# WilliamVenner/squad-mortar-helper

Measured on AMD Instinct MI355X. Metric: map frames/sec (1920x1080 full CV pipeline), whole job, higher is better.
Workload: dtype u8/f32

## Files before the change

include/smh_vision_hip_debug.h:

```cpp
#ifndef SMH_VISION_HIP_DEBUG_H
#define SMH_VISION_HIP_DEBUG_H

#include "smh_vision_hip.h"

#ifdef __cplusplus
extern "C" {
#endif

SMHV_API int smhv_debug_lsd_classic(int on);
SMHV_API int smhv_debug_lsd_tile_cap(uint32_t cap);
SMHV_API int smhv_debug_lsd_threads(uint32_t threads);
SMHV_API int smhv_debug_pattern_copy(smhv_batch *b, const void *d_frames, uint32_t n, uint32_t rows_in_flight, void *stream);
SMHV_API int smhv_debug_heightmap_color_map_device(smhv_heightmap *hm, void *d_rgba, float *ms);
SMHV_API int smhv_debug_skip_line_search(int on);
SMHV_API int smhv_debug_lsd_spin_limit(uint32_t polls);
SMHV_API int smhv_debug_no_host_atomics(int on);
SMHV_API int smhv_debug_side_kernel(smhv_ctx *ctx, uint32_t workgroups, void *stream);

SMHV_API int smhv_debug_pipeline_stats(smhv_pipeline *p, uint64_t out[32]);
SMHV_API int smhv_debug_pipeline_peek(smhv_pipeline *p, uint64_t out[16]);

SMHV_API int smhv_debug_marker_table(smhv_ctx *ctx, uint32_t *bits);

SMHV_API int smhv_debug_crc32_host_level(const void *data, uint64_t nbytes, int level, uint32_t *crc);
SMHV_API int smhv_debug_band_rows(uint32_t frame_w, uint32_t frame_h, uint32_t n, int fused, uint32_t *rows, uint32_t *bands, int *tiles);
SMHV_API int smhv_debug_map_band_rows(uint32_t rows);
SMHV_API int smhv_debug_render_form(uint32_t form);
SMHV_API int smhv_debug_render_rule(uint32_t map_w, uint32_t map_h, float sw, float sh, uint32_t hm_w, uint32_t hm_h, float *ratio, float *switch_ratio,
                                    uint32_t *lds_texels, uint32_t *form);
SMHV_API int smhv_debug_feed_rows(uint32_t rows);
SMHV_API int smhv_debug_feed_gray_form(uint32_t form);
SMHV_API int smhv_debug_batch_mask_state(smhv_batch *b, uint32_t *stale_frames, int *eager);
SMHV_API int smhv_debug_batch_ui_state(smhv_batch *b, uint32_t *stale_frames, int *eager);
SMHV_API int smhv_debug_batch_materialize_ui(smhv_batch *b, void *stream);
SMHV_API int smhv_debug_mask_expand(smhv_batch *b, uint32_t n, void *stream);
SMHV_API int smhv_debug_ingest_feed(smhv_ingest *q, uint32_t n, uint32_t *counter);
SMHV_API int smhv_debug_ingest_feed_pixels(smhv_ingest *q, uint32_t n, uint32_t *counter, uint32_t pixels);

#ifdef __cplusplus
}
#endif

#endif
```

squad-mortar-helper_amd/_lib.py:

```python
import ctypes as C
import os

_HERE = os.path.dirname(os.path.abspath(__file__))
LIB_PATH = os.environ.get("SMH_VISION_HIP_LIB") or os.path.join(_HERE, "libsmh_vision_hip.so")

MAX_LINES = 32
MAX_SCALES = 3

STAGE_MARKERS, STAGE_UI_MAP, STAGE_OCR, STAGE_SCALES, STAGE_ALL = 0x1, 0x2, 0x4, 0x8, 0xF
STAGE_MINIMAP = 0x10
STAGE_EXACT_STATS = 0x20
STAGE_LSD_HELPERS = 0x40
STAGE_FIRING = 0x80
STAGE_HEIGHTMAP_OVERLAY = 0x100
FIRING_BOUNDS_OFFSET = 1
FIRING_NONE, FIRING_SCALES, FIRING_HEIGHTMAP = 0, 1, 2
VIEW_NONE, VIEW_OCR_INPUT, VIEW_FIND_SCALES_INPUT, VIEW_LSD_PREPROCESS, VIEW_LSD_INPUT, VIEW_CROPPED_BRQ = range(6)
IMAGE_UI_MAP = 100
IMAGE_HEIGHTMAP_OVERLAY = 101
RENDER_HEIGHTMAP, RENDER_MARKERS, RENDER_BOUNDS_OFFSET = 1, 2, 4
RENDER_MAX_LINES = 256
PRIM_LINE, PRIM_RECT, PRIM_FOREGROUND, PRIM_SHIFT1 = 0, 1, 0x100, 0x200
RENDER_MAX_PRIMS = 256
LAYER_MINIMAP_BOUNDS = 1
# ... 117 lines not shown

class FeedHeader(C.Structure):
    _fields_ = [("n_entries", C.c_uint32), ("frames_done", C.c_uint32), ("n_maps", C.c_uint32), ("has_last_crc", C.c_uint32),
                ("last_crc", C.c_uint32), ("reserved", C.c_uint32), ("bytes_used", C.c_uint64)]


PIXELS_NV12, PIXELS_I420 = 5, 6
YUV_ROI_ONLY = 1


class YuvLayout(C.Structure):
    _fields_ = [("y_pitch", C.c_uint64), ("uv_pitch", C.c_uint64), ("u_offset", C.c_uint64), ("v_offset", C.c_uint64), ("frame_stride", C.c_uint64)]


LOG_FN = C.CFUNCTYPE(None, C.c_int, C.c_char_p)

SIGNATURES = {
    "smhv_init": (C.c_int, [C.c_int, LOG_FN, C.POINTER(C.c_void_p)]),
    "smhv_shutdown": (None, [C.c_void_p]),
    "smhv_thread_ctx": (C.c_int, [C.c_void_p]),
    "smhv_set_ray_table": (C.c_int, [C.c_void_p, C.POINTER(C.c_float), C.POINTER(C.c_float)]),
    "smhv_last_error": (C.c_char_p, []),
    "smhv_map_bounds": (C.c_int, [C.c_uint32, C.c_uint32, C.POINTER(C.c_uint32)]),
    "smhv_button_bounds": (C.c_int, [C.c_uint32, C.c_uint32, C.POINTER(C.c_uint32)]),
    "smhv_load_frame": (C.c_int, [C.c_void_p, C.c_void_p, C.c_uint32, C.c_uint32]),
    "smhv_load_frame_view": (C.c_int, [C.c_void_p, C.c_void_p] + [C.c_uint32] * 6),
    "smhv_load_frame_device": (C.c_int, [C.c_void_p, C.c_void_p, C.c_uint32, C.c_uint32]),
    "smhv_crop_to_map": (C.c_int, [C.c_void_p, C.c_int, C.POINTER(C.c_int), C.POINTER(C.c_uint32), C.c_void_p]),
    "smhv_red_pixels": (C.c_int, [C.c_void_p, C.POINTER(C.c_uint32)]),
    "smhv_ocr_preprocess": (C.c_int, [C.c_void_p, C.POINTER(C.c_void_p), C.POINTER(C.c_size_t)]),
    "smhv_find_scales_preprocess": (C.c_int, [C.c_void_p, C.c_uint32, C.POINTER(C.c_void_p), C.POINTER(C.c_uint32), C.POINTER(C.c_uint32)]),
    "smhv_isolate_map_markers": (C.c_int, [C.c_void_p]),
    "smhv_mask_marker_lines": (C.c_int, [C.c_void_p]),
    "smhv_get_lsd_image": (C.c_int, [C.c_void_p, C.c_void_p, C.POINTER(C.c_uint32), C.POINTER(C.c_uint32)]),
    "smhv_find_longest_line": (C.c_int, [C.c_void_p, C.c_float, C.c_float, C.c_float, C.POINTER(Line), C.POINTER(C.c_float)]),
    "smhv_find_marker_lines": (C.c_int, [C.c_void_p, C.c_uint32, C.POINTER(Line), C.POINTER(C.c_uint32)]),
    "smhv_lsd_stats": (C.c_int, [C.c_void_p, C.c_uint32, C.c_int, C.POINTER(C.c_uint32), C.POINTER(C.c_uint64)]),
    "smhv_calc_meters_to_px_ratio": (C.c_int, [C.c_void_p, C.POINTER(C.c_uint32), C.c_uint32, C.POINTER(C.c_double), C.POINTER(C.c_int), C.POINTER(C.c_uint32)]),
    "smhv_find_minimap": (C.c_int, [C.c_void_p, C.POINTER(C.c_uint32), C.POINTER(C.c_int)]),
    "smhv_get_debug_view": (C.c_int, [C.c_void_p, C.c_int, C.c_void_p, C.POINTER(C.c_uint32), C.POINTER(C.c_uint32)]),
    "smhv_batch_create": (C.c_int, [C.c_void_p, C.c_uint32, C.c_uint32, C.c_uint32, C.POINTER(C.c_void_p)]),
    "smhv_batch_destroy": (None, [C.c_void_p]),
    "smhv_batch_layout_get": (C.c_int, [C.c_void_p, C.POINTER(BatchLayout)]),
    "smhv_batch_run": (C.c_int, [C.c_void_p, C.c_void_p, C.c_uint32, C.c_uint32, C.c_int, C.c_uint32, C.c_void_p, C.c_void_p]),
    "smhv_batch_device_ptrs": (C.c_int, [C.c_void_p] + [C.POINTER(C.c_void_p)] * 6),
    "smhv_batch_tile_mask": (C.c_int, [C.c_void_p, C.POINTER(C.c_void_p), C.POINTER(C.c_void_p), C.POINTER(C.c_uint32)]),
    "smhv_batch_read_tile_mask": (C.c_int, [C.c_void_p, C.c_uint32, C.c_void_p, C.c_void_p, C.c_void_p, C.POINTER(C.c_int)]),
    "smhv_batch_read_results": (C.c_int, [C.c_void_p, C.c_uint32, C.c_uint32, C.POINTER(FrameResult)]),
    "smhv_batch_read_image": (C.c_int, [C.c_void_p, C.c_int, C.c_uint32, C.c_void_p]),
    "smhv_batch_set_scales_stream": (C.c_int, [C.c_void_p, C.c_void_p]),
    "smhv_batch_wait_map_pass": (C.c_int, [C.c_void_p, C.c_void_p]),
    "smhv_batch_enable_timing": (C.c_int, [C.c_void_p, C.c_int]),
    "smhv_batch_lsd_coop_stats": (C.c_int, [C.c_void_p, C.c_uint32, C.c_uint32, C.POINTER(C.c_uint32)]),
    "smhv_batch_stage_ms": (C.c_int, [C.c_void_p, C.POINTER(C.c_float)]),
    "smhv_pipeline_create": (C.c_int, [C.c_void_p, C.c_uint32, C.c_uint32, C.c_uint32, C.c_uint32, C.POINTER(C.c_void_p)]),
    "smhv_pipeline_create_ex": (C.c_int, [C.c_void_p, C.c_uint32, C.c_uint32, C.c_uint32, C.c_uint32, C.c_void_p, C.POINTER(C.c_void_p)]),
    "smhv_pipeline_hold": (C.c_int, [C.c_void_p, C.c_uint32, C.c_void_p]),
    "smhv_debug_pipeline_stats": (C.c_int, [C.c_void_p, C.POINTER(C.c_uint64)]),
    "smhv_debug_pipeline_peek": (C.c_int, [C.c_void_p, C.POINTER(C.c_uint64)]),
    "smhv_pipeline_destroy": (None, [C.c_void_p]),
    "smhv_pipeline_submit": (C.c_int, [C.c_void_p, C.c_void_p, C.c_uint32, C.c_uint32, C.c_int, C.c_uint32, C.c_void_p, C.c_void_p, C.POINTER(C.c_uint32)]),
    "smhv_pipeline_wait": (C.c_int, [C.c_void_p, C.c_uint32]),
    "smhv_pipeline_wait_all": (C.c_int, [C.c_void_p]),
    "smhv_pipeline_slot": (C.c_int, [C.c_void_p, C.c_uint32, C.POINTER(C.c_void_p), C.POINTER(C.c_void_p)]),
    "smhv_shard_range": (None, [C.c_uint64, C.c_uint32, C.c_uint32, C.POINTER(C.c_uint64), C.POINTER(C.c_uint64)]),
    "smhv_node_create": (C.c_int, [C.POINTER(C.c_int), C.c_uint32, C.c_uint32, C.c_uint32, C.c_uint32, C.c_uint32, LOG_FN, C.POINTER(C.c_void_p)]),
    "smhv_node_destroy": (None, [C.c_void_p]),
    "smhv_node_ctx": (C.c_int, [C.c_void_p, C.c_uint32, C.POINTER(C.c_void_p), C.POINTER(C.c_void_p)]),
    "smhv_node_run": (C.c_int, [C.c_void_p, C.POINTER(C.c_void_p), C.POINTER(C.c_uint32), C.c_uint32, C.c_int, C.c_uint32, C.POINTER(C.c_void_p)]),
    "smhv_node_gather": (C.c_int, [C.c_void_p, C.POINTER(FrameResult), C.POINTER(C.c_uint32)]),
    "smhv_debug_lsd_classic": (C.c_int, [C.c_int]),
    "smhv_debug_lsd_tile_cap": (C.c_int, [C.c_uint32]),
    "smhv_debug_lsd_spin_limit": (C.c_int, [C.c_uint32]),
    "smhv_debug_lsd_threads": (C.c_int, [C.c_uint32]),
    "smhv_debug_skip_line_search": (C.c_int, [C.c_int]),
    "smhv_debug_no_host_atomics": (C.c_int, [C.c_int]),
    "smhv_debug_side_kernel": (C.c_int, [C.c_void_p, C.c_uint32, C.c_void_p]),
    "smhv_trait_times": (C.c_int, [C.c_void_p, C.POINTER(C.c_uint64), C.POINTER(C.c_uint64), C.c_int]),
    "smhv_ui_map": (C.c_int, [C.c_void_p, C.POINTER(C.c_void_p), C.POINTER(C.c_uint32), C.POINTER(C.c_uint32)]),
    "smhv_debug_pattern_copy": (C.c_int, [C.c_void_p, C.c_void_p, C.c_uint32, C.c_uint32, C.c_void_p]),
    "smhv_debug_batch_mask_state": (C.c_int, [C.c_void_p, C.POINTER(C.c_uint32), C.POINTER(C.c_int)]),
    "smhv_debug_batch_ui_state": (C.c_int, [C.c_void_p, C.POINTER(C.c_uint32), C.POINTER(C.c_int)]),
    "smhv_debug_batch_materialize_ui": (C.c_int, [C.c_void_p, C.c_void_p]),
    "smhv_debug_mask_expand": (C.c_int, [C.c_void_p, C.c_uint32, C.c_void_p]),
    "smhv_debug_marker_table": (C.c_int, [C.c_void_p, C.c_void_p]),
    "smhv_ingest_create": (C.c_int, [C.c_void_p, C.c_uint32, C.c_uint32, C.c_uint32, C.c_uint32, C.POINTER(C.c_void_p)]),
    "smhv_ingest_create_ex": (C.c_int, [C.c_void_p, C.c_uint32, C.c_uint32, C.c_uint32, C.c_uint32, C.c_uint32, C.POINTER(C.c_void_p)]),
    "smhv_crc32_host": (C.c_uint32, [C.c_void_p, C.c_uint64]),
    "smhv_debug_map_band_rows": (C.c_int, [C.c_uint32]),
    "smhv_debug_band_rows": (C.c_int, [C.c_uint32, C.c_uint32, C.c_uint32, C.c_int, C.POINTER(C.c_uint32), C.POINTER(C.c_uint32), C.POINTER(C.c_int)]),
    "smhv_debug_ingest_feed": (C.c_int, [C.c_void_p, C.c_uint32, C.POINTER(C.c_uint32)]),
    "smhv_debug_ingest_feed_pixels": (C.c_int, [C.c_void_p, C.c_uint32, C.POINTER(C.c_uint32), C.c_uint32]),
    "smhv_debug_crc32_host_level": (C.c_int, [C.c_void_p, C.c_uint64, C.c_int, C.POINTER(C.c_uint32)]),
    "smhv_ingest_destroy": (None, [C.c_void_p]),
    "smhv_ingest_local_cpus": (C.c_int, [C.c_void_p, C.c_char_p, C.c_size_t]),
    "smhv_ingest_bind_thread": (C.c_int, [C.c_void_p]),
    "smhv_ingest_acquire": (C.c_int, [C.c_void_p, C.POINTER(C.c_void_p)]),
    "smhv_ingest_commit": (C.c_int, [C.c_void_p]),
    "smhv_ingest_push": (C.c_int, [C.c_void_p, C.c_void_p]),
    "smhv_ingest_commit_pixels": (C.c_int, [C.c_void_p, C.c_uint32]),
    "smhv_ingest_push_pixels": (C.c_int, [C.c_void_p, C.c_void_p, C.c_uint32]),
    "smhv_ingest_staging_bytes": (C.c_uint64, [C.c_uint32, C.c_uint32, C.c_uint32]),
    "smhv_yuv_to_bgra_device": (C.c_int, [C.c_void_p, C.c_void_p, C.POINTER(YuvLayout), C.c_uint32, C.c_uint32, C.c_uint32, C.c_uint32, C.c_void_p, C.c_uint64,
                                          C.c_uint32, C.c_void_p]),
    "smhv_ingest_batch": (C.c_int, [C.c_void_p, C.POINTER(C.c_void_p), C.POINTER(C.c_uint32), C.POINTER(C.c_uint32)]),
    "smhv_ingest_reset": (C.c_int, [C.c_void_p]),
    "smhv_ingest_counts": (C.c_int, [C.c_void_p, C.POINTER(C.c_uint64), C.POINTER(C.c_uint64)]),
    "smhv_crc32_device": (C.c_int, [C.c_void_p, C.c_void_p, C.c_uint64, C.POINTER(C.c_uint32)]),
    "smhv_heightmap_create": (C.c_int, [C.c_void_p, C.c_void_p, C.c_uint32, C.c_uint32, C.POINTER(C.c_int32), C.POINTER(C.c_float), C.POINTER(C.c_void_p)]),
    "smhv_heightmap_destroy": (None, [C.c_void_p]),
    "smhv_heightmap_color_map": (C.c_int, [C.c_void_p, C.c_void_p]),
    "smhv_debug_heightmap_color_map_device": (C.c_int, [C.c_void_p, C.c_void_p, C.POINTER(C.c_float)]),
    "smhv_batch_set_firing": (C.c_int, [C.c_void_p, C.c_void_p, C.POINTER(FiringOptions)]),
    "smhv_pipeline_set_firing": (C.c_int, [C.c_void_p, C.c_void_p, C.POINTER(FiringOptions)]),
    "smhv_batch_read_firing": (C.c_int, [C.c_void_p, C.c_uint32, C.c_uint32, C.POINTER(FiringResult)]),
    "smhv_batch_firing_ptr": (C.c_int, [C.c_void_p, C.POINTER(C.c_void_p)]),
    "smhv_firing_solutions": (C.c_int, [C.c_void_p, C.c_void_p, C.c_uint32, C.POINTER(C.c_double), C.POINTER(C.c_uint32), C.c_void_p,
                                        C.POINTER(FiringOptions), C.POINTER(Firing)]),
    "smhv_batch_overlay_ptr": (C.c_int, [C.c_void_p, C.POINTER(C.c_void_p)]),
    "smhv_heightmap_overlay": (C.c_int, [C.c_void_p, C.c_void_p, C.POINTER(FiringOptions), C.c_void_p]),
    "smhv_map_viewport_calc": (C.c_int, [C.c_float, C.c_float, C.c_float, C.c_float, C.c_uint32, C.POINTER(C.c_float), C.POINTER(C.c_float),
                                         C.POINTER(RenderOptions)]),
    "smhv_batch_render": (C.c_int, [C.c_void_p, C.c_uint32, C.c_uint32, C.c_void_p, C.POINTER(RenderOptions), C.c_void_p]),
    "smhv_batch_render_ptr": (C.c_int, [C.c_void_p, C.POINTER(C.c_void_p), C.POINTER(C.c_uint64)]),
    "smhv_batch_render_size": (C.c_int, [C.c_void_p, C.POINTER(C.c_uint32), C.POINTER(C.c_uint32)]),
    "smhv_batch_read_render": (C.c_int, [C.c_void_p, C.c_uint32, C.c_void_p]),
    "smhv_batch_render_layers": (C.c_int, [C.c_void_p, C.c_uint32, C.c_uint32, C.c_void_p, C.POINTER(RenderOptions), C.POINTER(RenderLayersStruct), C.c_void_p]),
    "smhv_render_map_layers": (C.c_int, [C.c_void_p, C.c_void_p, C.POINTER(RenderOptions), C.POINTER(RenderLayersStruct), C.c_void_p, C.c_uint32, C.c_void_p]),
    "smhv_render_map": (C.c_int, [C.c_void_p, C.c_void_p, C.POINTER(RenderOptions), C.c_void_p, C.c_uint32, C.c_void_p]),
    "smhv_label_font": (C.c_int, [C.c_uint8, C.POINTER(C.c_uint8)]),
    "smhv_batch_render_labels": (C.c_int, [C.c_void_p, C.c_uint32, C.c_uint32, C.c_void_p, C.POINTER(RenderOptions), C.POINTER(LabelOptionsStruct), C.c_void_p]),
    "smhv_batch_read_labels": (C.c_int, [C.c_void_p, C.c_uint32, C.c_uint32, C.POINTER(LabelResult)]),
    "smhv_batch_labels_ptr": (C.c_int, [C.c_void_p, C.POINTER(C.c_void_p)]),
    "smhv_render_map_labeled": (C.c_int, [C.c_void_p, C.c_void_p, C.POINTER(RenderOptions), C.POINTER(RenderLayersStruct), C.c_void_p, C.c_uint32,
                                          C.POINTER(LabelOptionsStruct), C.c_void_p, C.POINTER(LabelResult)]),
    "smhv_text_font": (C.c_int, [C.c_uint8, C.POINTER(C.c_uint8)]),
    "smhv_probe_text": (C.c_int, [C.POINTER(Probe), C.c_char_p, C.c_size_t]),
    "smhv_batch_probe": (C.c_int, [C.c_void_p, C.c_uint32, C.c_uint32, C.POINTER(RenderOptions), C.POINTER(ProbePoint), C.c_uint32, C.c_void_p]),
    "smhv_batch_read_probes": (C.c_int, [C.c_void_p, C.c_uint32, C.c_uint32, C.POINTER(Probe)]),
    "smhv_batch_probes_ptr": (C.c_int, [C.c_void_p, C.POINTER(C.c_void_p)]),
    "smhv_batch_render_debug": (C.c_int, [C.c_void_p, C.c_uint32, C.c_uint32, C.POINTER(RenderOptions), C.POINTER(DebugOptionsStruct), C.c_void_p]),
    "smhv_render_map_debug": (C.c_int, [C.c_void_p, C.c_void_p, C.POINTER(RenderOptions), C.POINTER(RenderLayersStruct), C.c_void_p, C.c_uint32,
                                        C.POINTER(LabelOptionsStruct), C.POINTER(DebugOptionsStruct), C.c_void_p, C.POINTER(LabelResult), C.POINTER(Probe)]),
    "smhv_feed_create": (C.c_int, [C.c_void_p, C.c_uint64, C.c_uint32, C.POINTER(C.c_void_p)]),
    "smhv_feed_destroy": (None, [C.c_void_p]),
    "smhv_feed_reset": (C.c_int, [C.c_void_p]),
    "smhv_batch_feed": (C.c_int, [C.c_void_p, C.c_void_p, C.c_uint32, C.c_uint32, C.c_uint32, C.c_void_p]),
    "smhv_feed_read": (C.c_int, [C.c_void_p, C.POINTER(FeedHeader), C.POINTER(FeedEntry), C.c_uint32, C.c_void_p, C.c_uint64]),
    "smhv_feed_ptrs": (C.c_int, [C.c_void_p, C.POINTER(C.c_void_p), C.POINTER(C.c_void_p), C.POINTER(C.c_void_p)]),
    "smhv_feed_frame": (C.c_int, [C.c_void_p, C.c_void_p, C.c_void_p, C.c_uint32, C.POINTER(C.c_double), C.POINTER(C.c_uint32), C.c_uint32]),
    "smhv_web_event_markers": (C.c_int, [C.c_void_p, C.c_uint32, C.c_int, C.c_void_p, C.c_uint64, C.POINTER(C.c_uint64)]),
    "smhv_web_event_heightmap": (C.c_int, [C.c_void_p, C.c_uint32, C.c_uint32, C.POINTER(C.c_int32), C.POINTER(C.c_float), C.c_void_p, C.c_uint64,
                                           C.POINTER(C.c_uint64)]),
    "smhv_web_event_fit": (C.c_int, [C.c_int, C.c_void_p, C.c_uint64, C.POINTER(C.c_uint64)]),
    "smhv_web_interaction_parse": (C.c_int, [C.c_void_p, C.c_uint64, C.POINTER(C.c_uint32), C.POINTER(C.c_float), C.POINTER(C.c_uint32)]),
    "smhv_debug_feed_rows": (C.c_int, [C.c_uint32]),
    "smhv_debug_feed_gray_form": (C.c_int, [C.c_uint32]),
    "smhv_batch_feed_view": (C.c_int, [C.c_void_p, C.c_void_p, C.c_uint32, C.c_uint32, C.c_uint32, C.c_uint32, C.c_void_p]),
    "smhv_feed_frame_view": (C.c_int, [C.c_void_p, C.c_void_p, C.c_void_p, C.c_uint32, C.POINTER(C.c_double), C.POINTER(C.c_uint32), C.c_uint32, C.c_uint32]),
    "smhv_debug_render_form": (C.c_int, [C.c_uint32]),
    "smhv_debug_render_rule": (C.c_int, [C.c_uint32, C.c_uint32, C.c_float, C.c_float, C.c_uint32, C.c_uint32, C.POINTER(C.c_float), C.POINTER(C.c_float),
                                         C.POINTER(C.c_uint32), C.POINTER(C.c_uint32)]),
}


def firing_options(fit_to_minimap=True, viewport=None):
# ... 67 lines not shown
```

squad-mortar-helper_amd/batch.py:

```python
import ctypes as C
from collections.abc import Mapping

import numpy as np

from . import _lib as L

STAGE_NAMES = ("button", "map_pass", "brq_pass", "lsd", "scale_ratio")


def make_anchors(per_frame):
    arr = (L.Anchors * len(per_frame))()
    for i, (start_y, scales) in enumerate(per_frame):
        arr[i].n = min(len(scales), L.MAX_SCALES)
        arr[i].scales_start_y = start_y
        for j, (m, x, y) in enumerate(scales[:L.MAX_SCALES]):
            arr[i].scales[j][0], arr[i].scales[j][1], arr[i].scales[j][2] = m, x, y
    return arr


def results_to_dicts(recs):
    out = []
    for r in recs:
        n = r.n_lines
        out.append(dict(
            map_open=int(r.map_open), n_lines=int(n),
            lines=np.array([[r.lines[i].x0, r.lines[i].y0, r.lines[i].x1, r.lines[i].y1] for i in range(n)], np.float32).reshape(-1, 4),
            mpx=(r.mpx if r.has_mpx else None), n_mask_px=int(r.n_mask_px), red_pixels=int(r.red_pixels),
            rounds=int(r.rounds), ray_steps=int(r.ray_steps),
            length_px=np.array(r.length_px[:n], np.float64), meters=np.array(r.meters[:n], np.float64),
            angle=np.array(r.angle[:n], np.float32),
            minimap=(tuple(r.minimap) if r.has_minimap else None),
            status=int(r.status), error=(None if r.status == L.FRAME_OK else "line search gave the frame up (SMHV_FRAME_LSD_STUCK)" if r.status == L.FRAME_LSD_STUCK
                                         else "status %d" % r.status)))
    return out


_PTR_KEYS = ("results", "ui", "mask", "ocr", "scales", "bits")


class _DevicePtrs(Mapping):

    def __init__(self, batch, ptrs):
        self._batch, self._ptrs = batch, ptrs

    def __getitem__(self, key):
        if key == "mask" and self._ptrs["mask"] is None:
            self._ptrs["mask"] = self._batch._mask_ptr()
        if key == "ui" and self._ptrs["ui"] is None:
            self._ptrs["ui"] = self._batch._ui_ptr()
        return self._ptrs[key]

    def __iter__(self):
        return iter(_PTR_KEYS)

    def __len__(self):
        return len(_PTR_KEYS)


class FrameBatch:

    def __init__(self, vision, frame_w, frame_h, max_frames, _handle=None):
        self._lib = L.load()
        self._vision = vision
        self._owned = _handle is None
        if _handle is None:
            b = C.c_void_p()
            L.check(self._lib.smhv_batch_create(vision._ctx, frame_w, frame_h, max_frames, C.byref(b)))
        else:
            b = _handle
        self._b = b
        self.max_frames = max_frames
        self.frame_w, self.frame_h = frame_w, frame_h
        self.layout = L.BatchLayout()
        L.check(self._lib.smhv_batch_layout_get(self._b, C.byref(self.layout)))

    def close(self):
        if self._b:
            if self._owned:
                self._lib.smhv_batch_destroy(self._b)
            self._b = None

    def __del__(self):
        try:
            self.close()
        except Exception:
            pass

    @property
    def roi(self):
        return tuple(self.layout.roi)

    def enable_timing(self, on=True):
        L.check(self._lib.smhv_batch_enable_timing(self._b, int(on)))

    def run(self, frames_ptr, n, stages=L.STAGE_ALL, grayscale=True, max_gap=15, anchors=None, stream=0):
        if anchors is not None and len(anchors) < n:
            raise ValueError("anchors holds %d entries, the run covers %d frames" % (len(anchors), n))
        a = C.cast(anchors, C.c_void_p) if anchors is not None else None
        L.check(self._lib.smhv_batch_run(self._b, C.c_void_p(frames_ptr), n, stages, int(bool(grayscale)), max_gap, a, C.c_void_p(stream)))

    def set_scales_stream(self, stream=0):
        L.check(self._lib.smhv_batch_set_scales_stream(self._b, C.c_void_p(stream)))

    def wait_map_pass(self, stream=0):
        L.check(self._lib.smhv_batch_wait_map_pass(self._b, C.c_void_p(stream)))

    def stage_ms(self):
        ms = (C.c_float * 5)()
        L.check(self._lib.smhv_batch_stage_ms(self._b, ms))
        return dict(zip(STAGE_NAMES, [float(v) for v in ms]))

    def lsd_coop_stats(self, first=0, n=None):
        n = self.max_frames - first if n is None else n
        out = np.zeros((n, 4), np.uint32)
        L.check(self._lib.smhv_batch_lsd_coop_stats(self._b, first, n, out.ctypes.data_as(C.POINTER(C.c_uint32))))
        return out

    def device_ptrs(self):
        p = [C.c_void_p() for _ in range(6)]
        args = [C.byref(x) for x in p]
        args[1] = args[2] = None
        L.check(self._lib.smhv_batch_device_ptrs(self._b, *args))
        return _DevicePtrs(self, dict(zip(_PTR_KEYS, [x.value for x in p])))

    def _mask_ptr(self):
        m = C.c_void_p()
        L.check(self._lib.smhv_batch_device_ptrs(self._b, None, None, C.byref(m), None, None, None))
        return m.value

    def _ui_ptr(self):
        u = C.c_void_p()
        L.check(self._lib.smhv_batch_device_ptrs(self._b, None, C.byref(u), None, None, None, None))
        return u.value

    def ui_state(self):
        stale, eager = C.c_uint32(0), C.c_int(0)
        L.check(self._lib.smhv_debug_batch_ui_state(self._b, C.byref(stale), C.byref(eager)))
        return int(stale.value), bool(eager.value)

    def materialize_ui(self, stream=0):
        L.check(self._lib.smhv_debug_batch_materialize_ui(self._b, C.c_void_p(stream)))

    def mask_state(self):
        stale, eager = C.c_uint32(0), C.c_int(0)
        L.check(self._lib.smhv_debug_batch_mask_state(self._b, C.byref(stale), C.byref(eager)))
        return int(stale.value), bool(eager.value)

    def tile_mask(self, frame=0):
        geo = (C.c_uint32 * 4)()
        L.check(self._lib.smhv_batch_tile_mask(self._b, None, None, geo))
        trows, wcols, opitch, xoff = [int(v) for v in geo]
        tiled = np.zeros((trows, wcols, 8), np.uint32)
        occ = np.zeros((trows, opitch), np.uint8)
        bits = np.zeros((self.roi[3], wcols), np.uint32)
        written = C.c_int(0)
        L.check(self._lib.smhv_batch_read_tile_mask(self._b, frame, tiled.ctypes.data, occ.ctypes.data, bits.ctypes.data, C.byref(written)))
        return (tiled if written.value else None), (occ if written.value else None), bits, xoff

    def read_results(self, first=0, n=None, check=True):
        n = self.max_frames - first if n is None else n
        recs = (L.FrameResult * n)()
        rc = self._lib.smhv_batch_read_results(self._b, first, n, recs)
        if rc != 0 and not (rc == L.E_STATE and not check):
            try:
                L.check(rc)
            except L.VisionError as e:
                e.records = recs if rc == L.E_STATE else None
                raise
        return recs

    def set_firing(self, heightmap=None, fit_to_minimap=True, viewport=None):
        opt = L.firing_options(fit_to_minimap, viewport)
        L.check(self._lib.smhv_batch_set_firing(self._b, heightmap._hm if heightmap is not None else None, C.byref(opt)))

    def read_firing(self, first=0, n=None):
        n = self.max_frames - first if n is None else n
        out = (L.FiringResult * n)()
        L.check(self._lib.smhv_batch_read_firing(self._b, first, n, out))
        raw = np.frombuffer(out, np.uint8).reshape(n, C.sizeof(L.FiringResult))
        n_lines = raw[:, :4].copy().view(np.uint32).reshape(n)
        lines = raw[:, 8:].copy().view(L.firing_dtype()).reshape(n, L.MAX_LINES)
        return n_lines, lines

    def firing_ptr(self):
        d = C.c_void_p()
        L.check(self._lib.smhv_batch_firing_ptr(self._b, C.byref(d)))
        return d.value or 0

    def read_overlay(self, frame):
        return self.read_image(L.IMAGE_HEIGHTMAP_OVERLAY, frame)

    def overlay_ptr(self):
        d = C.c_void_p()
        L.check(self._lib.smhv_batch_overlay_ptr(self._b, C.byref(d)))
        return d.value or 0

    def render(self, viewport, out_w, out_h, first=0, n=None, heightmap=None, markers=False, fit_to_minimap=True, background=(0, 0, 0, 255),
               stream=None, options=None, layers=None):
        from .render import render_options
        n = self.max_frames - first if n is None else n
        opt = options if options is not None else render_options(viewport, out_w, out_h, heightmap is not None, markers, fit_to_minimap, background)
        if layers is not None:
            ly, keep = layers.struct()
            L.check(self._lib.smhv_batch_render_layers(self._b, first, n, heightmap._hm if heightmap is not None else None, C.byref(opt), C.byref(ly), stream))
            del keep
            return
        L.check(self._lib.smhv_batch_render(self._b, first, n, heightmap._hm if heightmap is not None else None, C.byref(opt), stream))

    def render_size(self):
        w, h = C.c_uint32(), C.c_uint32()
        L.check(self._lib.smhv_batch_render_size(self._b, C.byref(w), C.byref(h)))
        return int(w.value), int(h.value)

    def read_render(self, frame):
        w, h = self.render_size()
        out = np.empty((h, w, 4), np.uint8)
# ... 162 lines not shown
```

squad-mortar-helper_amd/csrc/smh_feed.inc:

```

struct smhv_feed {
	smhv_ctx *ctx = nullptr;
	uint64_t capacity = 0;
	uint32_t max_frames = 0;
	uint8_t *d_bytes = nullptr;
	smhv_feed_header *d_header = nullptr;
	smhv_feed_entry *d_entries = nullptr;
	uint32_t *d_state = nullptr, *d_raw = nullptr, *d_tab = nullptr;
	FeedMap *d_maps = nullptr;
	uint32_t tab_w = 0, tab_h = 0, tab_xoff = 0, tab_ppg = 0;
	uint8_t *d_view = nullptr;
	size_t view_cap = 0;
	hipEvent_t ev_last = nullptr;
	bool used = false;
	smhv_frame_result *d_rec = nullptr, *h_rec = nullptr;
};

extern "C" SMHV_API void smhv_feed_destroy(smhv_feed *f) {
	if (!f) return;
	if (f->ctx) (void)hipSetDevice(f->ctx->device);
	(void)hipDeviceSynchronize();
	void *ptrs[] = {f->d_bytes, f->d_header, f->d_entries, f->d_state, f->d_raw, f->d_tab, f->d_maps, f->d_rec, f->d_view};
	for (void *p : ptrs)
		if (p) (void)hipFree(p);
// ... 81 lines not shown
		f->tab_w = cw; f->tab_h = ch; f->tab_xoff = cxoff; f->tab_ppg = v.ppg;
	}
	FeedRun r;
	memset(&r, 0, sizeof r);
	r.ui = v.base; r.res = res;
	r.ui_stride = v.stride; r.ui_pitch = v.pitch;
	r.w = v.w; r.h = v.h; r.xoff = v.xoff; r.quads = v.quads;
	r.n = n; r.first = first; r.flags = flags;
	r.len_term = crc32_mul(crc32_xpow(32ull * v.w * v.h), 0xFFFFFFFFu) ^ 0xFFFFFFFFu;
	r.rows_per_wave = feed_rows_per_wave(ch, n);
	r.capacity = f->capacity;
	r.raw = f->d_raw; r.tab = f->d_tab; r.state = f->d_state;
	r.header = f->d_header; r.entries = f->d_entries; r.bytes = f->d_bytes; r.maps = f->d_maps;
	if (v.mode == SMH_RND_SRC_UI) HIPCHK(launch_feed(r, s));
	else if (!image) HIPCHK(launch_feed_view(r, v.mode, s));
	else {
		FeedRun c = r;
		c.ui = v.base - 4ull * v.lead; c.ui_pitch = 4ull * SMH_FEED_IMAGE_ROW; c.ui_stride = 0;
		c.w = cw; c.h = ch; c.xoff = 0u; c.quads = cquads;
		HIPCHK(launch_feed_image(c, r, s));
	}
	HIPCHK(hipEventRecord(f->ev_last, s));
	f->used = true;
	return SMHV_OK;
}

static int feed_batch_source(const smhv_batch *b, uint32_t first, uint32_t map_source, bool resolve, FeedSrc *v) {
	const Geom &g = b->g;
	if (map_source > (uint32_t)SMHV_VIEW_CROPPED_BRQ) return fail(SMHV_E_INVALID, "batch_feed_view: unknown map source %u", map_source);
	if (resolve && !b->ui_written) return fail(SMHV_E_STATE, "batch_feed: no run of this batch has produced a ui_map (SMHV_STAGE_UI_MAP)");
	*v = feed_src_ui(g, b->d_ui + (size_t)first * g.ui_stride);
	switch ((int)map_source) {
	case SMHV_VIEW_NONE: break;
	case SMHV_VIEW_OCR_INPUT:
	case SMHV_VIEW_FIND_SCALES_INPUT: {
		const bool ocr = map_source == (uint32_t)SMHV_VIEW_OCR_INPUT;
		if (resolve && !(ocr ? b->ocr_written : b->scales_written))
			return fail(SMHV_E_STATE, "batch_feed_view: no run of this batch has produced the %s image", ocr ? "OCR input (SMHV_STAGE_OCR)" : "scales input (SMHV_STAGE_SCALES with anchors)");
		v->mode = SMH_RND_SRC_GRAY; v->ppg = 16u;
		v->base = (ocr ? b->d_ocr : b->d_scales) + (size_t)first * g.ocr_stride;
		v->pitch = g.ocr_pitch; v->stride = g.ocr_stride; v->xoff = g.q_xoff; v->w = g.qw; v->h = g.qh;
		v->quads = (v->w + v->xoff + 15u) / 16u;
		break;
	}
	case SMHV_VIEW_LSD_INPUT:
		if (resolve && !b->mask_written) return fail(SMHV_E_STATE, "batch_feed_view: no run of this batch has produced the marker mask (SMHV_STAGE_MARKERS)");
		v->mode = SMH_RND_SRC_GRAY; v->ppg = 16u;
		v->base = b->d_mask + (size_t)first * g.mask_stride;
		v->pitch = g.mask_pitch; v->stride = g.mask_stride;
		v->quads = (v->w + v->xoff + 15u) / 16u;
		break;
	default:
		if (resolve && b->ui_gray) return fail(SMHV_E_STATE, "batch_feed_view: the batch's ui_map is grayscale, map source %u needs the colour one", map_source);
		if (map_source == (uint32_t)SMHV_VIEW_CROPPED_BRQ) {
			const uint32_t x0 = g.m_xoff + g.rw / 2u;
			v->mode = SMH_RND_SRC_CROPPED; v->w = g.rw / 2u; v->h = g.rh / 2u;
			if (resolve && (v->w == 0u || v->h == 0u)) return fail(SMHV_E_STATE, "batch_feed_view: the map has no bottom right quarter");
			v->base += (size_t)(g.rh / 2u) * g.ui_pitch + 16ull * (x0 / 4u);
			v->xoff = x0 & 3u; v->quads = (v->w + v->xoff + 3u) / 4u;
		} else v->mode = SMH_RND_SRC_PREPROCESS;
		break;
	}
	return SMHV_OK;
}

extern "C" SMHV_API int smhv_batch_feed_view(smhv_batch *b, smhv_feed *f, uint32_t first, uint32_t n, uint32_t flags, uint32_t map_source, void *stream) {
	if (!b || !f) return fail(SMHV_E_INVALID, "batch_feed: null argument");
	CTX_OPEN(b->ctx);
	CTX_OPEN(f->ctx);
	if (f->ctx->device != b->ctx->device) return fail(SMHV_E_INVALID, "batch_feed: the feed lives on device %d, the batch on %d", f->ctx->device, b->ctx->device);
	if (n == 0u || (uint64_t)first + n > b->max_frames) return fail(SMHV_E_INVALID, "batch_feed: frames [%u, %u + %u) of a batch of %u", first, first, n, b->max_frames);
	FeedSrc v;
	int rc = feed_batch_source(b, first, map_source, false, &v);
	if (rc) return rc;
	rc = feed_check(f, v.w, v.h, n, flags, "batch_feed");
	if (rc) return rc;
	rc = feed_batch_source(b, first, map_source, true, &v);
	if (rc) return rc;
	HIPCHK(hipSetDevice(b->ctx->device));
	if (map_source == (uint32_t)SMHV_VIEW_LSD_INPUT) {
		rc = batch_materialize_mask(b, (hipStream_t)stream);
		if (rc) return rc;
	}
	rc = batch_materialize_ui(b, (hipStream_t)stream);
	if (rc) return rc;
	return feed_enqueue(f, v, b->d_results + first, first, n, flags, (hipStream_t)stream);
}

extern "C" SMHV_API int smhv_batch_feed(smhv_batch *b, smhv_feed *f, uint32_t first, uint32_t n, uint32_t flags, void *stream) {
	return smhv_batch_feed_view(b, f, first, n, flags, (uint32_t)SMHV_VIEW_NONE, stream);
}

extern "C" SMHV_API int smhv_feed_read(smhv_feed *f, smhv_feed_header *header, smhv_feed_entry *entries, uint32_t max_entries, uint8_t *bytes, uint64_t cap) {
	if (!f || !header) return fail(SMHV_E_INVALID, "feed_read: null argument");
	CTX_OPEN(f->ctx);
	HIPCHK(hipSetDevice(f->ctx->device));
	if (f->used) HIPCHK(wait_event(f->ev_last));
	HIPCHK(hipMemcpy(header, f->d_header, sizeof *header, hipMemcpyDeviceToHost));
	if (entries && header->n_entries > max_entries) return fail(SMHV_E_INVALID, "feed_read: %u entries, room for %u", header->n_entries, max_entries);
	if (bytes && header->bytes_used > cap) return fail(SMHV_E_INVALID, "feed_read: %llu bytes, room for %llu", (unsigned long long)header->bytes_used, (unsigned long long)cap);
	if (entries && header->n_entries) HIPCHK(hipMemcpy(entries, f->d_entries, sizeof(smhv_feed_entry) * header->n_entries, hipMemcpyDeviceToHost));
	if (bytes && header->bytes_used) HIPCHK(hipMemcpy(bytes, f->d_bytes, (size_t)header->bytes_used, hipMemcpyDeviceToHost));
	return SMHV_OK;
}

extern "C" SMHV_API int smhv_feed_ptrs(smhv_feed *f, void **d_header, void **d_entries, void **d_bytes) {
	if (!f) return fail(SMHV_E_INVALID, "feed_ptrs: null feed");
	if (d_header) *d_header = f->d_header;
	if (d_entries) *d_entries = f->d_entries;
	if (d_bytes) *d_bytes = f->d_bytes;
	return SMHV_OK;
}

extern "C" SMHV_API int smhv_debug_feed_gray_form(uint32_t form) {
	if (form != 0u && form != 4u) return fail(SMHV_E_INVALID, "feed gray form %u (0 = the rule, 4 = four lookups per message dword)", form);
	feed_set_gray_form(form);
	return SMHV_OK;
}

extern "C" SMHV_API int smhv_debug_feed_rows(uint32_t rows) {
	if (rows > 64u) return fail(SMHV_E_INVALID, "feed rows per wave %u (0 = the rule, 1 .. 64)", rows);
	feed_set_rows(rows);
	return SMHV_OK;
}

extern "C" SMHV_API int smhv_feed_frame_view(smhv_ctx *c, smhv_feed *f, const smhv_line *lines, uint32_t n_lines, const double *mpx, const uint32_t minimap[4],
                                             uint32_t flags, uint32_t map_source) {
	int rc = require_open(c, "feed_frame");
	if (rc) return rc;
	CTX_OPEN(c);
	if (!f || (n_lines && !lines)) return fail(SMHV_E_INVALID, "feed_frame: null argument");
	CTX_OPEN(f->ctx);
	if (f->ctx->device != c->device) return fail(SMHV_E_INVALID, "feed_frame: the feed lives on device %d, the context on %d", f->ctx->device, c->device);
	if (n_lines > SMHV_MAX_LINES) return fail(SMHV_E_INVALID, "feed_frame: %u lines (at most %u)", n_lines, (unsigned)SMHV_MAX_LINES);
	if (map_source > (uint32_t)SMHV_VIEW_CROPPED_BRQ) return fail(SMHV_E_INVALID, "feed_frame_view: unknown map source %u", map_source);
	smhv_batch *b = c->fb;
	const Geom &g = b->g;
	rc = batch_materialize_ui(b, c->s_main);
	if (rc) return rc;
	FeedSrc v = feed_src_ui(g, b->d_ui);
	if (map_source != (uint32_t)SMHV_VIEW_NONE) {
		const int which = (int)map_source;
		const bool brq = which == SMHV_VIEW_OCR_INPUT || which == SMHV_VIEW_FIND_SCALES_INPUT || which == SMHV_VIEW_CROPPED_BRQ;
		v.mode = SMH_RND_SRC_RGBA; v.w = brq ? g.qw : g.rw; v.h = brq ? g.qh : g.rh;
		v.xoff = 0u; v.quads = 0u; v.pitch = 4ull * v.w; v.stride = 0;
	}
	rc = feed_check(f, v.w, v.h, 1, flags, "feed_frame");
	if (rc) return rc;
	HIPCHK(hipSetDevice(c->device));
	if (f->used) HIPCHK(wait_event(f->ev_last));
	if (v.mode == SMH_RND_SRC_RGBA) {
		const uint64_t dw = (uint64_t)v.w * v.h, rows = (dw + SMH_FEED_IMAGE_ROW - 1u) / SMH_FEED_IMAGE_ROW;
		const size_t need = (size_t)rows * SMH_FEED_IMAGE_ROW * 4u;
		if (rows > SMH_FEED_MAX_ROWS) return fail(SMHV_E_INVALID, "feed_frame_view: a view of %u x %u pixels", v.w, v.h);
		if (f->view_cap < need) {
			if (f->d_view) (void)hipFree(f->d_view);
			f->d_view = nullptr; f->view_cap = 0;
			HIPCHK(hipMalloc((void **)&f->d_view, need));
			f->view_cap = need;
		}
		v.lead = (uint32_t)(rows * SMH_FEED_IMAGE_ROW - dw);
		v.base = f->d_view + 4ull * v.lead;
		if (v.lead) HIPCHK(hipMemsetAsync(f->d_view, 0, 4ull * v.lead, c->s_main));
		Buffers bf = make_buffers(b, c->frame_ptr, 0);
		HIPCHK(launch_debug_view(g, bf, 0, (int)map_source, c->isolated ? 1 : 0, f->d_view + 4ull * v.lead, c->s_main));
	}
// ... 87 lines not shown
```

squad-mortar-helper_amd/csrc/smh_kernels.h:

```cpp
#pragma once
#include <hip/hip_runtime.h>
#include <stdint.h>

#include "../../include/smh_vision_hip.h"
#include "../../include/smh_vision_hip_debug.h"

namespace smh {

struct Geom {
	uint32_t W, H;
	uint32_t rx, ry, rw, rh;
	uint32_t bx, by, bw, bh;
	uint32_t qx, qy, qw, qh;
	uint32_t m_ax, m_xoff, m_quads, m_block;
	uint32_t q_ax, q_xoff, q_quads, q_block;
	uint64_t frame_bytes;
	uint64_t ui_pitch, ui_stride;
	uint64_t mask_pitch, mask_stride;
	uint32_t bits_pitch_w; uint64_t bits_stride_w;
	uint64_t ocr_pitch, ocr_stride;
};

struct FrameAux {
	uint32_t open;
// ... 207 lines not shown
#define SMH_CULL_TAB_WORDS (SMH_CULL_CELLS + (SMH_SECTOR_ENTRIES + 3) / 4)

#define SVC_MAX_SLOTS 32u
struct SvcSlot {
	Buffers b;
	uint32_t n;
	uint32_t seq;
	uint32_t done;
	uint32_t pad;
	unsigned long long t_pub;
};
#define SVC_REMOTE_RING 12u
#define SVC_REMOTE_OPEN 0x80000000ull
struct SvcRemoteEntry {
	unsigned long long post;
	unsigned long long claim;
	uint32_t res_a[4];
	uint32_t res_b[4];
	unsigned long long pad[2];
};
struct SvcRemote {
	unsigned long long state;
	unsigned long long info;
	unsigned long long pad[6];
	SvcRemoteEntry ring[SVC_REMOTE_RING];
};
#define SVC_HELP_RING 256u
struct SvcCtl {
	int32_t avail;
	uint32_t closing;
	int32_t help_avail;
	uint32_t help_head, help_reserve;
	uint32_t stat_remote;
	uint32_t head;
	uint32_t reserve;
	uint32_t completed;
	uint32_t busy;
	uint32_t stat_items, stat_waves;
	unsigned long long stat_busy, stat_life;
	unsigned long long stat_phase[4];
	unsigned long long stat_help;
	uint32_t stat_requests, stat_attached;
	unsigned long long stat_t_wait, stat_t_sub, stat_t_last;
	uint32_t stat_h_polls, stat_h_empty, stat_h_lost, stat_h_idle_exit, stat_h_closed_exit, stat_h_pad;
	unsigned long long stat_h_cycles, stat_h_cast_cycles;
	unsigned long long help_ring[SVC_HELP_RING];
};
struct SvcHost {
	unsigned long long state;
	uint32_t launches;
	uint32_t pad0;
	uint32_t done_seq[SVC_MAX_SLOTS];
	uint32_t pad[12];
};
struct SvcParams {
	SvcCtl *ctl;
	unsigned long long *ring;
	SvcSlot *slots;
	SvcHost *host;
	const uint32_t *cull_tab;
	const float *ray_off;
	float max_gap;
	uint32_t tile_cap, list_cap;
	uint32_t part_words;
	uint32_t ring_log2;
	uint32_t epoch;
	uint32_t idle_short, idle_long;
	uint32_t flags;
	SvcRemote *remote;
	uint32_t *remote_store;
	uint32_t remote_store_words;
	uint32_t remote_after;
	uint32_t remote_tickets;
	uint32_t remote_last_div;
	uint32_t compact;
};
uint32_t svc_waves_for(const Geom &g, uint32_t tile_limit, uint32_t *part_words, uint32_t *tile_cap, uint32_t *list_cap, uint32_t *lds_bytes, uint32_t *compact = nullptr);
uint32_t svc_store_words_for(const Geom &g, uint32_t tile_cap, uint32_t compact);
hipError_t svc_probe_host_atomics(SvcHost *h, SvcHost *d_h, bool *ok);
hipError_t launch_svc_publish(SvcCtl *ctl, unsigned long long *ring, SvcSlot *slots, uint32_t slot, const Buffers &b, uint32_t n, uint32_t seq, uint32_t ring_log2, hipStream_t s);
hipError_t launch_lsd_service(const Geom &g, const SvcParams &p, uint32_t workgroups, uint32_t waves, uint32_t lds_bytes, hipStream_t s);

enum : uint32_t { MAP_UI = 1u, MAP_MASK = 2u, MAP_BYTES = 4u, MAP_PRIO = 0x100u, MAP_BAND_MAJOR = 0x200u };
enum : uint32_t { BRQ_OCR = 1u, BRQ_SCALES = 2u };

enum : uint32_t { UI_FORM_RGBA = 0u, UI_FORM_LUMA = 1u, UI_FORM_KEEP = 2u };
hipError_t launch_button(const Geom &g, const Buffers &b, uint32_t n, int force_open, hipStream_t s, uint8_t *ui_form = nullptr, uint32_t ui_luma = UI_FORM_KEEP);
hipError_t launch_ui_expand(const Geom &g, const uint8_t *d_luma, uint8_t *d_ui, uint8_t *ui_form, uint32_t n, hipStream_t s);
hipError_t launch_map_pass(const Geom &g, const Buffers &b, uint32_t n, uint32_t flags, int grayscale, hipStream_t s, bool tiles_wanted = false, bool overlapped = false);
struct LaunchTuning {
	uint32_t map_lds_total;
	uint32_t map_grid_cap;
	uint32_t lsd_tile_limit;
	uint32_t map_prio;
	uint32_t map_deep;
	uint32_t map_overlapped;
};
uint32_t map_brq_lds_bytes(const Geom &g);
uint32_t lsd_tile_lds_bytes(const Geom &g, uint32_t tile_limit);
hipError_t launch_map_brq_pass(const Geom &g, const Buffers &b, uint32_t n, uint32_t flags, uint32_t qflags, int grayscale, uint32_t fixed_start_y, int use_anchor_start, hipStream_t s,
                               const LaunchTuning *tune = nullptr);
hipError_t launch_pattern_copy(const Geom &g, const Buffers &b, uint32_t n, uint32_t rows_in_flight, hipStream_t s);
void map_band_rows(uint32_t rh, uint32_t n, int fused, uint32_t *rows, int *tiles);
hipError_t launch_brq_pass(const Geom &g, const Buffers &b, uint32_t n, uint32_t flags, uint32_t fixed_start_y, int use_anchor_start, hipStream_t s);
struct LsdFork { hipStream_t s1, s2; hipEvent_t fork, join1, join2; };
bool lsd_rows_only(const Geom &g);
hipError_t launch_lsd(const Geom &g, const Buffers &b, uint32_t n, float max_gap, int mode, float px, float py, hipStream_t s, const LsdFork *fk, uint32_t tile_bs = 0,
                      bool prefer_classic = false, uint32_t tile_limit = 0, bool *record_fused = nullptr);
size_t lsd_coop_ctl_bytes(uint32_t n);
hipError_t launch_scale_ratio(const Geom &g, const Buffers &b, uint32_t n, uint32_t *d_bars, hipStream_t s);
hipError_t launch_find_minimap(const Geom &g, const Buffers &b, uint32_t n, hipStream_t s);
hipError_t launch_finalize(const Geom &g, const Buffers &b, uint32_t n, uint32_t stages, hipStream_t s);
hipError_t launch_scales_finalize(const Geom &g, const Buffers &b, uint32_t n, uint32_t stages, uint32_t *d_bars, hipStream_t s);
hipError_t launch_firing_lines(const FiringRun &r, const smhv_line *lines, uint32_t n, uint32_t has_mpx, double mpx, uint32_t has_minimap,
                               const uint32_t minimap[4], smhv_firing *out, hipStream_t s);
hipError_t launch_heightmap_color_map(const uint16_t *hm, uint64_t n, uint32_t *mm, uint32_t *rgba, hipStream_t s);
#define SMH_HM_LUT_ENTRIES 65536u
hipError_t launch_heightmap_lut(const uint16_t *hm, uint64_t n, uint32_t *mm, uint32_t *lut, hipStream_t s);
hipError_t launch_hm_overlay(const Geom &g, const OverlayRun &r, uint32_t n, hipStream_t s);
hipError_t launch_render_map(const Geom &g, const RenderRun &r, uint32_t n, hipStream_t s);
hipError_t launch_render_map_layers(const Geom &g, const RenderRun &r, const RenderLayersRun &y, uint32_t n, hipStream_t s);
hipError_t launch_heightmap_lut16(const uint32_t *lut, uint16_t *lut16, uint32_t *vr, hipStream_t s);
#define SMH_HM_LUT_WORDS (SMH_HM_LUT_ENTRIES + 4u + SMH_HM_LUT_ENTRIES / 2u)
hipError_t launch_labels(const LabelRun &r, uint32_t n, hipStream_t s);
hipError_t launch_debug_text(const Geom &g, const DebugRun &r, uint32_t n, hipStream_t s);
void render_set_form(uint32_t form);
uint32_t render_rule(const Geom &g, const RenderRun &r, uint32_t *texels, float *ratio);
float render_switch_ratio();
hipError_t launch_debug_view(const Geom &g, const Buffers &b, uint32_t frame, int which, int isolated, uint8_t *d_rgba, hipStream_t s);
hipError_t launch_marker_table(uint32_t *d_bits, hipStream_t s);
hipError_t launch_mask_expand(const Geom &g, const uint32_t *d_bits, uint8_t *d_mask, uint32_t n, hipStream_t s);
hipError_t launch_pack_rows(const void *d_src, uint32_t src_pitch_bytes, void *d_dst, uint32_t row_bytes, uint32_t rows, hipStream_t s);
hipError_t launch_side_probe(uint32_t *d_out, uint32_t workgroups, uint32_t spin, hipStream_t s);
hipError_t launch_build_sector_table(unsigned long long *d_tab, uint32_t T, hipStream_t s);
hipError_t launch_build_ray_offsets(float *d_off, hipStream_t s);
size_t lsd_lds_bytes();
void lsd_set_classic(bool on);
void lsd_set_tile_cap(uint32_t cap);
void lsd_set_threads(uint32_t threads);
void lsd_set_spin_limit(uint32_t polls);
hipError_t set_ray_table(const float *dx, const float *dy);
#define SMH_CRC_BS 1024
hipError_t launch_to_bgra(const void *d_src, void *d_bgra, uint64_t n_px, uint32_t layout, hipStream_t s);
#define SMH_YUV_NV12 5
#define SMH_YUV_I420 6
#define SMH_YUV_BAND_PAIRS 4u
struct YuvCoef { int cy, yoff, rv, gu, gv, bu; };
struct YuvRect {
	uint32_t x0, y0, w, h;
	uint64_t y_off, u_off, v_off;
	uint32_t y_pitch, uv_pitch, y_x0, y_y0, c_x0, c_y0;
};
struct YuvRun {
	const uint8_t *src; uint8_t *dst;
	uint64_t src_stride, dst_stride;
	uint32_t W, H, n;
	uint32_t bands0, bands_total;
	YuvCoef k;
	YuvRect r[2];
};
hipError_t launch_yuv_to_bgra(YuvRun run, uint32_t n_rects, uint32_t layout, uint32_t bilinear, hipStream_t s);
hipError_t launch_unpack_rows(const void *d_pack, void *d_frame, uint32_t pitch_px, uint32_t roi_x, uint32_t roi_y, uint32_t roi_w, uint32_t roi_h, uint32_t btn_x,
                              uint32_t btn_y, uint32_t btn_w, uint32_t btn_h, hipStream_t s);
hipError_t launch_crc32(const void *d_msg, uint64_t n_dwords, uint32_t wgs, uint32_t rounds, uint32_t x_skip, const uint32_t *d_x_local,
                        const uint32_t *d_x_wg, uint32_t *d_acc, hipStream_t s);
uint32_t crc32_xpow(uint64_t n);
uint32_t crc32_mul(uint32_t a, uint32_t b);

struct FeedMap { uint64_t dst; uint32_t frame, pad; };
struct FeedRun {
	const uint8_t *ui;
	const smhv_frame_result *res;
	uint64_t ui_stride, ui_pitch;
	uint32_t w, h, xoff, quads;
	uint32_t n, first, flags;
	uint32_t len_term;
	uint32_t rows_per_wave;
	uint64_t capacity;
	uint32_t *raw;
	const uint32_t *tab;
	uint32_t *state;
	smhv_feed_header *header;
// ... 17 lines not shown
```

squad-mortar-helper_amd/csrc/smh_misc.hip:

```cpp
#include "smh_device.h"
#include "smh_record.inc"

namespace smh {

__global__ void __launch_bounds__(64 * SMHV_MAX_SCALES) k_scale_ratio(Geom g, Buffers b, uint32_t *bars) { scale_ratio_body(g, b, blockIdx.x, bars); }

__device__ __forceinline__ bool flat_pixel(const uint8_t *roi0, uint32_t W, uint32_t x, uint32_t y) {
	const uint32_t *p = (const uint32_t *)(roi0 + ((size_t)y * W + x) * 4);
	const int Wi = (int)W;
	const uint32_t c = p[0] & 0x00FFFFFFu;
	uint32_t mx = 0;
#pragma unroll
	for (int dy = -1; dy <= 1; ++dy)
#pragma unroll
		for (int dx = -1; dx <= 1; ++dx)
			if (dx != 0 || dy != 0) mx = max(mx, (uint32_t)__builtin_amdgcn_sad_u8(c, p[dy * Wi + dx] & 0x00FFFFFFu, 0u));
	return (float)mx / 765.0f <= 0.01f;
}

__device__ uint32_t find_edge(const uint8_t *roi0, uint32_t W, uint32_t w, uint32_t h, uint32_t x0, uint32_t y0, int dir) {
	const uint32_t lane = threadIdx.x & 63u;
	const bool vertical = dir < 2;
	uint32_t c_max = vertical ? h : w, oc_max = vertical ? w : h;
	const int cod = (dir == 0 || dir == 2) ? -1 : 1;
// ... 302 lines not shown
hipError_t launch_scale_ratio(const Geom &g, const Buffers &b, uint32_t n, uint32_t *d_bars, hipStream_t s) {
	hipLaunchKernelGGL(k_scale_ratio, dim3(n), dim3(64 * SMHV_MAX_SCALES), 0, s, g, b, d_bars);
	return hipGetLastError();
}

hipError_t launch_find_minimap(const Geom &g, const Buffers &b, uint32_t n, hipStream_t s) {
	hipLaunchKernelGGL(k_find_minimap, dim3(n), dim3(256), 0, s, g, b);
	return hipGetLastError();
}

hipError_t launch_finalize(const Geom &g, const Buffers &b, uint32_t n, uint32_t stages, hipStream_t s) {
	if (stages & SMHV_STAGE_FIRING) hipLaunchKernelGGL(k_finalize_firing, dim3(n), dim3(64), 0, s, g, b, stages);
	else hipLaunchKernelGGL(k_finalize, dim3(n), dim3(64), 0, s, g, b, stages);
	return hipGetLastError();
}

hipError_t launch_scales_finalize(const Geom &g, const Buffers &b, uint32_t n, uint32_t stages, uint32_t *d_bars, hipStream_t s) {
	if (stages & SMHV_STAGE_FIRING) hipLaunchKernelGGL(k_scales_finalize_firing, dim3(n), dim3(64 * SMHV_MAX_SCALES), 0, s, g, b, stages, d_bars);
	else hipLaunchKernelGGL(k_scales_finalize, dim3(n), dim3(64 * SMHV_MAX_SCALES), 0, s, g, b, stages, d_bars);
	return hipGetLastError();
}

__global__ void __launch_bounds__(256) k_pack_rows(const uint32_t *__restrict__ src, uint32_t src_pitch_w, uint32_t *__restrict__ dst, uint32_t row_w, uint32_t rows) {
	const uint32_t r = blockIdx.y;
	const uint32_t *s = src + (size_t)r * src_pitch_w;
	uint32_t *d = dst + (size_t)r * row_w;
	for (uint32_t x = blockIdx.x * blockDim.x + threadIdx.x; x < row_w; x += gridDim.x * blockDim.x) d[x] = s[x];
}
hipError_t launch_pack_rows(const void *d_src, uint32_t src_pitch_bytes, void *d_dst, uint32_t row_bytes, uint32_t rows, hipStream_t s) {
	if ((src_pitch_bytes | row_bytes) & 3u) return hipErrorInvalidValue;
	const uint32_t row_w = row_bytes / 4u;
	hipLaunchKernelGGL(k_pack_rows, dim3((row_w + 255u) / 256u, rows), dim3(256), 0, s, (const uint32_t *)d_src, src_pitch_bytes / 4u, (uint32_t *)d_dst, row_w, rows);
	return hipGetLastError();
}

__global__ void __launch_bounds__(256) k_mask_expand(const uint16_t *__restrict__ bits, uint4 *__restrict__ mask, uint64_t groups) {
	const uint64_t i = (uint64_t)blockIdx.x * 256u + threadIdx.x;
	if (i >= groups) return;
	const uint32_t v = bits[i];
	uint4 o;
	o.x = (((v & 15u) * 0x00204081u) & 0x01010101u) * 0xFFu;
	o.y = ((((v >> 4) & 15u) * 0x00204081u) & 0x01010101u) * 0xFFu;
	o.z = ((((v >> 8) & 15u) * 0x00204081u) & 0x01010101u) * 0xFFu;
	o.w = ((((v >> 12) & 15u) * 0x00204081u) & 0x01010101u) * 0xFFu;
	mask[i] = o;
}
hipError_t launch_mask_expand(const Geom &g, const uint32_t *d_bits, uint8_t *d_mask, uint32_t n, hipStream_t s) {
	if (g.mask_pitch != (uint64_t)g.bits_pitch_w * 32u || (g.mask_stride & 15u)) return hipErrorInvalidValue;
	const uint64_t groups = g.mask_stride / 16u * n, blocks = (groups + 255u) / 256u;
	if (blocks == 0 || blocks > 0x7FFFFFFFull) return hipErrorInvalidValue;
	hipLaunchKernelGGL(k_mask_expand, dim3((uint32_t)blocks), dim3(256), 0, s, (const uint16_t *)d_bits, (uint4 *)d_mask, groups);
	return hipGetLastError();
}

__global__ void __launch_bounds__(256) k_ui_expand(const uint32_t *__restrict__ luma, uint4 *__restrict__ ui, const uint8_t *__restrict__ form, uint32_t groups,
                                                   uint32_t pitch_q, uint32_t quads) {
	const uint32_t f = blockIdx.y;
	if (form[f] != UI_FORM_LUMA) return;
	const uint32_t i = blockIdx.x * 256u + threadIdx.x;
	if (i >= groups || i % pitch_q >= quads) return;
	const size_t j = (size_t)f * groups + i;
	const uint32_t v = luma[j];
	uint4 o;
	o.x = __builtin_amdgcn_perm(0u, v, 0x0D000000u);
	o.y = __builtin_amdgcn_perm(0u, v, 0x0D010101u);
	o.z = __builtin_amdgcn_perm(0u, v, 0x0D020202u);
	o.w = __builtin_amdgcn_perm(0u, v, 0x0D030303u);
	ui[j] = o;
}
hipError_t launch_ui_expand(const Geom &g, const uint8_t *d_luma, uint8_t *d_ui, uint8_t *ui_form, uint32_t n, hipStream_t s) {
	if ((g.ui_stride & 15u) || g.ui_stride / 16u > 0xFFFFFF00ull || n == 0) return hipErrorInvalidValue;
	const uint32_t groups = (uint32_t)(g.ui_stride / 16u);
	hipError_t e = hipSuccess;
	for (uint32_t done = 0; done < n && e == hipSuccess; done += 65535u) {
		const uint32_t k = std::min(n - done, 65535u);
		hipLaunchKernelGGL(k_ui_expand, dim3((groups + 255u) / 256u, k), dim3(256), 0, s, (const uint32_t *)d_luma + (size_t)done * groups, (uint4 *)d_ui + (size_t)done * groups,
		                   (const uint8_t *)ui_form + done, groups, (uint32_t)(g.ui_pitch / 16u), g.m_quads);
		e = hipGetLastError();
	}
	if (e == hipSuccess) e = hipMemsetAsync(ui_form, 0, n, s);
	return e;
}

hipError_t launch_debug_view(const Geom &g, const Buffers &b, uint32_t frame, int which, int isolated, uint8_t *d_rgba, hipStream_t s) {
	const bool brq = which == SMHV_VIEW_OCR_INPUT || which == SMHV_VIEW_FIND_SCALES_INPUT || which == SMHV_VIEW_CROPPED_BRQ;
	const uint32_t npx = brq ? g.qw * g.qh : g.rw * g.rh;
	hipLaunchKernelGGL(k_debug_view, dim3((npx + 255) / 256), dim3(256), 0, s, g, b, frame, which, isolated, d_rgba);
	return hipGetLastError();
}

hipError_t launch_marker_table(uint32_t *d_bits, hipStream_t s) {
	hipLaunchKernelGGL(k_marker_table, dim3(((1u << 24) / 32u + 255) / 256), dim3(256), 0, s, d_bits);
	return hipGetLastError();
}

#define CRC_POLY SMH_CRC_POLY
#define CRC_BS 1024

__global__ void __launch_bounds__(CRC_BS) k_crc32(const uint32_t *msg, uint64_t n_dwords, uint32_t rounds, uint32_t x_skip,
                                                 const uint32_t *x_local, const uint32_t *x_wg, uint32_t *acc) {
	__shared__ uint32_t tab[4][256];
	__shared__ uint32_t wsum[CRC_BS / 64];
	const uint32_t tid = threadIdx.x;
	if (tid < 256u) {
		uint32_t c = tid;
		for (int k = 0; k < 8; ++k) c = (c >> 1) ^ ((c & 1u) ? CRC_POLY : 0u);
		tab[0][tid] = c;
	}
	__syncthreads();
	if (tid < 256u) {
		uint32_t c = tab[0][tid];
		for (int k = 1; k < 4; ++k) { c = (c >> 8) ^ tab[0][c & 255u]; tab[k][tid] = c; }
	}
	__syncthreads();
	const uint64_t G = (uint64_t)gridDim.x * CRC_BS, T = (uint64_t)blockIdx.x * CRC_BS + tid;
	const uint64_t pad = (uint64_t)rounds * G * 4u - n_dwords;
	uint32_t v = 0;
	for (uint32_t r = 0; r < rounds; ++r) {
		const uint64_t vi = ((uint64_t)r * G + T) * 4u;
		uint32_t d[4] = {0u, 0u, 0u, 0u};
		if (vi >= pad && ((vi - pad) & 3u) == 0u && (((uintptr_t)msg) & 15u) == 0u) {
			const uint4 q = *(const uint4 *)(msg + (vi - pad));
			d[0] = q.x; d[1] = q.y; d[2] = q.z; d[3] = q.w;
		} else {
#pragma unroll
			for (int j = 0; j < 4; ++j) if (vi + j >= pad) d[j] = msg[vi + j - pad];
		}
		if (r) v = gf2_mulmod(v, x_skip);
#pragma unroll
		for (int j = 0; j < 4; ++j) {
			const uint32_t c = v ^ d[j];
			v = tab[3][c & 255u] ^ tab[2][(c >> 8) & 255u] ^ tab[1][(c >> 16) & 255u] ^ tab[0][c >> 24];
		}
	}
	v = gf2_mulmod(v, x_local[tid]);
	v = wave_xor32_dpp(v);
	if ((tid & 63u) == 0u) wsum[tid >> 6] = v;
	__syncthreads();
	if (tid == 0) {
		uint32_t w = 0;
		for (int k = 0; k < CRC_BS / 64; ++k) w ^= wsum[k];
		atomicXor(acc, gf2_mulmod(w, x_wg[blockIdx.x]));
	}
}

uint32_t crc32_xpow(uint64_t n) {
	uint32_t r = 0x80000000u, b = 0x40000000u;
	for (; n; n >>= 1) { if (n & 1u) r = gf2_mulmod(r, b); b = gf2_mulmod(b, b); }
	return r;
}
uint32_t crc32_mul(uint32_t a, uint32_t b) { return gf2_mulmod(a, b); }

hipError_t launch_crc32(const void *d_msg, uint64_t n_dwords, uint32_t wgs, uint32_t rounds, uint32_t x_skip, const uint32_t *d_x_local,
                        const uint32_t *d_x_wg, uint32_t *d_acc, hipStream_t s) {
	hipLaunchKernelGGL(k_crc32, dim3(wgs), dim3(CRC_BS), 0, s, (const uint32_t *)d_msg, n_dwords, rounds, x_skip, d_x_local, d_x_wg, d_acc);
	return hipGetLastError();
}

template <int BPP>
__global__ void __launch_bounds__(256) k_to_bgra(const uint32_t *__restrict__ src, uint4 *__restrict__ dst, uint64_t n_groups, uint64_t n_px) {
	for (uint64_t gidx = (uint64_t)blockIdx.x * 256u + threadIdx.x; gidx < n_groups; gidx += (uint64_t)gridDim.x * 256u) {
		uint32_t w[4] = {0u, 0u, 0u, 0u}, px[4];
		const uint64_t n_src_dwords = (n_px * BPP + 3u) / 4u;
#pragma unroll
		for (int k = 0; k < BPP; ++k) { const uint64_t i = gidx * BPP + k; if (i < n_src_dwords) w[k] = src[i]; }
		if (BPP == 4) {
// ... 60 lines not shown
```

squad-mortar-helper_amd/csrc/smh_runtime.cpp:

```cpp
#include <hip/hip_runtime.h>

#include <atomic>
#include <condition_variable>
#include <deque>
#include <thread>
#include <cmath>
#include <cstdarg>
#include <cstdio>
#include <cstdlib>
#include <cstring>
#include <ctime>
#include <sched.h>
#include <pthread.h>
#include <cctype>
#include <mutex>
#include <vector>
#include <new>
#include <string>

#include "smh_consts.h"
#include "smh_kernels.h"

using namespace smh;

// ... 99 lines not shown
	if (rc) return rc;
	rc = smhv_button_bounds(W, H, bt);
	if (rc) return rc;
	memset(g, 0, sizeof *g);
	g->W = W; g->H = H;
	g->rx = m[0]; g->ry = m[1]; g->rw = m[2]; g->rh = m[3];
	g->bx = bt[0]; g->by = bt[1]; g->bw = bt[2]; g->bh = bt[3];
	g->qw = g->rw / 2; g->qh = g->rh / 2;
	g->qx = g->rx + g->qw; g->qy = g->ry + g->qh;
	if (g->qw < SMH_OCR_DILATE_RADIUS || g->qh < SMH_OCR_DILATE_RADIUS) return fail(SMHV_E_GEOMETRY, "frame %ux%u too small", W, H);
	g->m_ax = g->rx & ~3u; g->m_xoff = g->rx - g->m_ax;
	g->m_quads = (g->rw + g->m_xoff + 3u) / 4u;
	g->m_block = (g->m_quads + 63u) & ~63u;
	g->q_ax = g->qx & ~3u; g->q_xoff = g->qx - g->q_ax;
	g->q_quads = (g->qw + g->q_xoff + 3u) / 4u;
	g->q_block = (g->q_quads + 63u) & ~63u;
	if (g->m_block > 1024u) return fail(SMHV_E_GEOMETRY, "frame %ux%u: map ROI wider than 4096 px is not supported", W, H);
	const uint32_t mq = (g->m_quads + 15u) & ~15u, qq = (g->q_quads + 15u) & ~15u;
	g->frame_bytes = (uint64_t)W * H * 4;
	g->ui_pitch = (uint64_t)mq * 16; g->ui_stride = g->ui_pitch * g->rh;
	g->mask_pitch = (uint64_t)mq * 4; g->mask_stride = g->mask_pitch * g->rh;
	g->bits_pitch_w = mq / 8; g->bits_stride_w = (uint64_t)g->bits_pitch_w * g->rh;
	g->ocr_pitch = (uint64_t)qq * 4; g->ocr_stride = g->ocr_pitch * g->qh;
	return SMHV_OK;
}

struct smhv_batch {
	smhv_ctx *ctx = nullptr;
	Geom g{};
	uint32_t max_frames = 0;
	uint8_t *d_ui = nullptr, *d_mask = nullptr, *d_ocr = nullptr, *d_scales = nullptr;
	uint32_t *d_bits = nullptr, *d_bars = nullptr, *d_tiled = nullptr;
	uint8_t *d_occ = nullptr;
	FrameAux *d_aux = nullptr;
	smhv_frame_result *d_results = nullptr;
	smhv_anchors *d_anchors = nullptr;
	BatchError *h_err = nullptr, *d_err = nullptr;
	FarmFrame *d_farm = nullptr;
	uint8_t *d_lsd_ctl = nullptr;
	uint32_t *d_lsd_req = nullptr;
	LsdCacheEntry *d_lsd_cache = nullptr;
	uint32_t lsd_epoch = 0;
	struct AnchorStage { smhv_anchors *h = nullptr; hipEvent_t done = nullptr; };
	std::vector<AnchorStage> anchor_stage;
	static constexpr int TIMING_RING = 64;
	static constexpr int TIMING_EVENTS = 10;
	bool timing = false;
	hipEvent_t (*ev)[TIMING_EVENTS] = nullptr;
	uint64_t timed_runs = 0;
	hipStream_t s_scales = nullptr;
	hipStream_t s_scales_ext = nullptr;
	hipEvent_t ev_map_done = nullptr;
	hipEvent_t ev_fork = nullptr, ev_join = nullptr;
	LsdFork lsd_fork{};
	uint32_t lsd_late_kc = 0;
	uint32_t lsd_bs = 1024;
	bool lsd_prefer_classic = false;
	LaunchTuning tune{0u, 0u, 0u, 0u};
	hipEvent_t ev_probe[3] = {nullptr, nullptr, nullptr};
	bool probe = false, probe_valid = false;
	smhv_heightmap *fire_hm = nullptr;
	smhv_firing_options fire_opt{};
	smhv_firing_result *d_firing = nullptr;
	FiringRun *d_fire_run = nullptr;
	struct FireStage { FiringRun *h = nullptr; hipEvent_t done = nullptr; };
	std::vector<FireStage> fire_stage;
	uint8_t *d_overlay = nullptr;
	uint8_t *d_render = nullptr;
	size_t render_cap = 0;
	uint32_t render_w = 0, render_h = 0;
	smhv_heightmap *render_hm = nullptr;
	hipEvent_t ev_render = nullptr;
	bool ui_written = false;
	bool ui_gray = false, mask_written = false, ocr_written = false, scales_written = false;
	std::mutex mask_mu;
	uint32_t mask_stale = 0;
	bool mask_eager = false;
	hipEvent_t ev_mask = nullptr;
	uint8_t *d_ui_luma = nullptr, *d_ui_form = nullptr;
	std::mutex ui_mu;
	uint32_t ui_stale = 0;
	bool ui_eager = false;
	hipEvent_t ev_ui = nullptr;
	smhv_render_prim *h_prims = nullptr, *d_prims = nullptr;
	hipEvent_t ev_prims = nullptr;
	smhv_label_result *d_labels = nullptr;
	LabelCull *d_label_cull = nullptr;
	smhv_label_line *h_label_extra = nullptr, *d_label_extra = nullptr;
	hipEvent_t ev_label_extra = nullptr;
	smhv_heightmap *label_hm = nullptr;
	smhv_probe *d_probes = nullptr;
	DebugItem *d_dbg_items = nullptr;
	uint8_t *d_dbg_pool = nullptr, *h_dbg_stage = nullptr, *d_dbg_stage = nullptr;
	hipEvent_t ev_dbg_stage = nullptr, ev_dbg = nullptr;
	bool probed = false;
};

struct smhv_heightmap {
	smhv_ctx *ctx = nullptr;
	uint16_t *d = nullptr;
	uint32_t w = 0, h = 0;
	int32_t bounds[4] = {0, 0, 0, 0};
	float scale[3] = {0.0f, 0.0f, 0.0f};
	std::atomic<int> refs{1};
	mutable std::mutex lut_mu;
	mutable std::atomic<uint32_t *> d_lut{nullptr};
};
static void hm_retain(smhv_heightmap *hm) { if (hm) hm->refs.fetch_add(1, std::memory_order_relaxed); }
static void hm_release(smhv_heightmap *hm);

struct smhv_ctx {
	int device = 0;
	smhv_log_fn log = nullptr;
	hipStream_t s_main = nullptr, s_markers = nullptr, s_scales = nullptr;
	hipStream_t s_ui = nullptr;
	hipEvent_t ev_map = nullptr, ev_ui[2] = {nullptr, nullptr};
	hipEvent_t ev_ui_part[3] = {nullptr, nullptr, nullptr};
	uint8_t *h_ui[2] = {nullptr, nullptr};
	size_t h_ui_cap[2] = {0, 0};
	uint8_t *d_ui_tight = nullptr;
	size_t d_ui_tight_cap = 0;
	uint8_t *d_fire = nullptr, *h_fire = nullptr;
	size_t fire_cap = 0;
	std::mutex fire_mu;
	uint32_t ui_turn = 0;
	bool ui_pending = false, minimap_cached = false;
	uint32_t W = 0, H = 0;
	bool have_frame = false;
	uint8_t *d_frame = nullptr;
	size_t d_frame_cap = 0;
	const uint8_t *frame_ptr = nullptr;
	smhv_batch *fb = nullptr;
	uint8_t *h_ocr = nullptr, *h_scales = nullptr;
	uint8_t *h_stage[3] = {nullptr, nullptr, nullptr};
	size_t h_stage_cap[3] = {0, 0, 0};
	smhv_frame_result *h_res = nullptr;
	FrameAux *h_aux = nullptr;
	uint32_t *h_bars = nullptr;
	bool cropped = false, map_open = false, isolated = false, mask_valid = false, scales_valid = false;
	static constexpr int SECTOR_CACHE = 8;
	uint32_t sector_T[SECTOR_CACHE] = {};
	uint32_t *sector_tab[SECTOR_CACHE] = {};
	int sector_n = 0;
	float *d_ray_off = nullptr;
	uint32_t *d_side = nullptr;
	std::atomic<uint64_t> tt_ns[SMHV_TRAIT_CALLS] = {}, tt_calls[SMHV_TRAIT_CALLS] = {};
	std::mutex mu;
	std::atomic<int> refs{1};
	std::atomic<bool> closed{false};
};

static std::mutex g_ctx_mu;
static std::vector<smhv_ctx *> g_ctx_open;

static void ctx_release(smhv_ctx *c) {
	if (c && c->refs.fetch_sub(1, std::memory_order_acq_rel) == 1) delete c;
}
#define CTX_OPEN(c)                                                                                          \
	do {                                                                                                     \
		if (!(c) || (c)->closed.load(std::memory_order_acquire)) return fail(SMHV_E_INVALID, "the context was shut down"); \
	} while (0)

static void logf(smhv_ctx *c, int lvl, const char *fmt, ...) {
	if (!c || !c->log) return;
	char buf[512];
	va_list ap;
// ... 169 lines not shown
extern "C" SMHV_API int smhv_debug_lsd_tile_cap(uint32_t cap) {
	lsd_set_tile_cap(cap);
	return SMHV_OK;
}

extern "C" SMHV_API int smhv_debug_skip_line_search(int on) {
	g_skip_lsd.store(on != 0, std::memory_order_relaxed);
	return SMHV_OK;
}

static std::atomic<bool> g_no_host_atomics{false};
extern "C" SMHV_API int smhv_debug_no_host_atomics(int on) {
	g_no_host_atomics.store(on != 0, std::memory_order_relaxed);
	return SMHV_OK;
}
extern "C" SMHV_API int smhv_debug_side_kernel(smhv_ctx *c, uint32_t workgroups, void *stream) {
	if (!c || workgroups == 0 || workgroups > 1024u) return fail(SMHV_E_INVALID, "side_kernel: 1..1024 workgroups");
	CTX_OPEN(c);
	HIPCHK(hipSetDevice(c->device));
	if (!c->d_side) HIPCHK(hipMalloc((void **)&c->d_side, 1024u * sizeof(uint32_t)));
	HIPCHK(launch_side_probe(c->d_side, workgroups, 64u, (hipStream_t)stream));
	return SMHV_OK;
}
extern "C" SMHV_API int smhv_debug_lsd_threads(uint32_t threads) {
	if (threads != 0 && (threads < 128 || threads > 1024 || threads % 64)) return fail(SMHV_E_INVALID, "lsd_threads: 0 or a multiple of 64 from 128 to 1024");
	lsd_set_threads(threads);
	return SMHV_OK;
}

extern "C" SMHV_API int smhv_debug_lsd_spin_limit(uint32_t polls) {
	lsd_set_spin_limit(polls);
	return SMHV_OK;
}

extern "C" SMHV_API int smhv_set_ray_table(smhv_ctx *c, const float *dx, const float *dy) {
	if (!c || !dx || !dy) return fail(SMHV_E_INVALID, "bad arguments");
	CTX_OPEN(c);
	for (int i = 0; i < SMH_LSD_RAYS; ++i) {
		const double a = (double)i / 10.0 * 3.14159265358979323846 / 180.0;
		if (!(std::fabs((double)dx[i] - std::cos(a)) < 1e-5 && std::fabs((double)dy[i] - std::sin(a)) < 1e-5))
			return fail(SMHV_E_INVALID, "ray table entry %d is not (cos, sin) of %.1f degrees", i, i / 10.0);
	}
	std::lock_guard<std::mutex> lk(g_ctx_mu);
	HIPCHK(hipSetDevice(c->device));
	HIPCHK(hipDeviceSynchronize());
	HIPCHK(set_ray_table(dx, dy));
	for (smhv_ctx *o : g_ctx_open)
		if (o->device == c->device && o->d_ray_off) HIPCHK(launch_build_ray_offsets(o->d_ray_off, c->s_main));
	HIPCHK(hipStreamSynchronize(c->s_main));
	return SMHV_OK;
}

static hipError_t create_stream(hipStream_t *st, const uint32_t *cu_mask) {
	return cu_mask ? hipExtStreamCreateWithCUMask(st, 8, cu_mask) : hipStreamCreateWithFlags(st, hipStreamNonBlocking);
}

extern "C" SMHV_API int smhv_batch_create(smhv_ctx *c, uint32_t W, uint32_t H, uint32_t max_frames, smhv_batch **out) {
	if (!c || !out || max_frames == 0) return fail(SMHV_E_INVALID, "bad arguments");
	*out = nullptr;
	CTX_OPEN(c);
	Geom g;
	int rc = compute_geom(W, H, &g);
	if (rc) return rc;
	HIPCHK(hipSetDevice(c->device));
	smhv_batch *b = new (std::nothrow) smhv_batch();
	if (!b) return fail(SMHV_E_INVALID, "out of host memory");
	c->refs.fetch_add(1, std::memory_order_relaxed);
	b->ctx = c; b->g = g; b->max_frames = max_frames;
	const size_t n = max_frames;
#define ALLOC0(ptr, bytes)                                          \
	do {                                                            \
		hipError_t _e = hipMalloc((void **)&(ptr), (bytes));        \
		if (_e == hipSuccess) _e = hipMemset((ptr), 0, (bytes));    \
		if (_e != hipSuccess) { smhv_batch_destroy(b); return fail(SMHV_E_HIP, "allocating %zu bytes: %s", (size_t)(bytes), hipGetErrorString(_e)); } \
	} while (0)
	ALLOC0(b->d_ui, g.ui_stride * n);
	ALLOC0(b->d_ui_luma, g.ui_stride / 4 * n);
	ALLOC0(b->d_ui_form, n);
	ALLOC0(b->d_mask, g.mask_stride * n);
	ALLOC0(b->d_bits, g.bits_stride_w * 4 * n);
	ALLOC0(b->d_tiled, tiled_stride_w(g) * 4 * n);
	ALLOC0(b->d_occ, occ_stride(g) * n);
	ALLOC0(b->d_ocr, g.ocr_stride * n);
	ALLOC0(b->d_scales, g.ocr_stride * n);
	ALLOC0(b->d_aux, sizeof(FrameAux) * n);
	ALLOC0(b->d_results, sizeof(smhv_frame_result) * (n + 3));
	ALLOC0(b->d_anchors, sizeof(smhv_anchors) * n);
	ALLOC0(b->d_bars, sizeof(uint32_t) * SMHV_MAX_SCALES * 4 * n);
	ALLOC0(b->d_lsd_ctl, lsd_coop_ctl_bytes(max_frames));
	ALLOC0(b->d_lsd_req, sizeof(uint32_t) * SMH_LSD_REQ_CAP * n);
	ALLOC0(b->d_farm, sizeof(FarmFrame) * n);
	ALLOC0(b->d_lsd_cache, sizeof(LsdCacheEntry) * SMH_LSD_CACHE_SLOTS * n);
#undef ALLOC0
	{
		hipError_t e = hipHostMalloc((void **)&b->h_err, sizeof(BatchError), hipHostMallocMapped | hipHostMallocCoherent);
		if (e == hipSuccess) { memset(b->h_err, 0, sizeof(BatchError)); e = hipHostGetDevicePointer((void **)&b->d_err, b->h_err, 0); }
		if (e == hipSuccess) e = hipEventCreateWithFlags(&b->ev_map_done, hipEventDisableTiming);
		if (e == hipSuccess) e = hipEventCreateWithFlags(&b->ev_mask, hipEventDisableTiming);
		if (e == hipSuccess) e = hipEventCreateWithFlags(&b->ev_ui, hipEventDisableTiming);
		if (max_frames > 1 && !lsd_rows_only(b->g)) {
			if (e == hipSuccess) e = create_stream(&b->lsd_fork.s1, nullptr);
			if (e == hipSuccess) e = create_stream(&b->lsd_fork.s2, nullptr);
			if (e == hipSuccess) e = hipEventCreateWithFlags(&b->lsd_fork.fork, hipEventDisableTiming);
			if (e == hipSuccess) e = hipEventCreateWithFlags(&b->lsd_fork.join1, hipEventDisableTiming);
			if (e == hipSuccess) e = hipEventCreateWithFlags(&b->lsd_fork.join2, hipEventDisableTiming);
		}
		if (e != hipSuccess) { smhv_batch_destroy(b); return fail(SMHV_E_HIP, "branch streams: %s", hipGetErrorString(e)); }
	}
	*out = b;
	return SMHV_OK;
}

extern "C" SMHV_API void smhv_batch_destroy(smhv_batch *b) {
	if (!b) return;
	if (b->ctx) (void)hipSetDevice(b->ctx->device);
	(void)hipDeviceSynchronize();
	void *ptrs[] = {b->d_ui, b->d_ui_luma, b->d_ui_form, b->d_mask, b->d_bits, b->d_tiled, b->d_occ, b->d_ocr, b->d_scales, b->d_aux, b->d_results, b->d_anchors, b->d_bars, b->d_farm,
	                b->d_lsd_ctl, b->d_lsd_req, b->d_lsd_cache, b->d_firing, b->d_fire_run, b->d_overlay, b->d_render, b->d_prims, b->d_labels,
	                b->d_label_cull, b->d_label_extra, b->d_probes, b->d_dbg_items, b->d_dbg_pool, b->d_dbg_stage};
	for (void *p : ptrs)
		if (p) (void)hipFree(p);
	if (b->h_prims) (void)hipHostFree(b->h_prims);
	if (b->ev_prims) (void)hipEventDestroy(b->ev_prims);
	if (b->h_label_extra) (void)hipHostFree(b->h_label_extra);
	if (b->ev_label_extra) (void)hipEventDestroy(b->ev_label_extra);
	if (b->h_dbg_stage) (void)hipHostFree(b->h_dbg_stage);
	if (b->ev_dbg_stage) (void)hipEventDestroy(b->ev_dbg_stage);
	if (b->ev_dbg) (void)hipEventDestroy(b->ev_dbg);
	if (b->h_err) (void)hipHostFree(b->h_err);
	for (auto &a : b->anchor_stage) {
		if (a.h) (void)hipHostFree(a.h);
		if (a.done) (void)hipEventDestroy(a.done);
	}
	for (auto &a : b->fire_stage) {
		if (a.h) (void)hipHostFree(a.h);
		if (a.done) (void)hipEventDestroy(a.done);
	}
	hm_release(b->fire_hm);
	hm_release(b->render_hm);
	hm_release(b->label_hm);
	if (b->ev_render) (void)hipEventDestroy(b->ev_render);
	if (b->ev) {
		for (int r = 0; r < smhv_batch::TIMING_RING; ++r)
			for (int i = 0; i < smhv_batch::TIMING_EVENTS; ++i) if (b->ev[r][i]) (void)hipEventDestroy(b->ev[r][i]);
		delete[] b->ev;
	}
	if (b->s_scales) (void)hipStreamDestroy(b->s_scales);
	if (b->ev_fork) (void)hipEventDestroy(b->ev_fork);
	if (b->ev_join) (void)hipEventDestroy(b->ev_join);
	if (b->ev_map_done) (void)hipEventDestroy(b->ev_map_done);
	if (b->ev_mask) (void)hipEventDestroy(b->ev_mask);
	if (b->ev_ui) (void)hipEventDestroy(b->ev_ui);
	for (auto e : b->ev_probe) if (e) (void)hipEventDestroy(e);
	if (b->lsd_fork.s1) (void)hipStreamDestroy(b->lsd_fork.s1);
	if (b->lsd_fork.s2) (void)hipStreamDestroy(b->lsd_fork.s2);
	if (b->lsd_fork.fork) (void)hipEventDestroy(b->lsd_fork.fork);
	if (b->lsd_fork.join1) (void)hipEventDestroy(b->lsd_fork.join1);
	if (b->lsd_fork.join2) (void)hipEventDestroy(b->lsd_fork.join2);
	ctx_release(b->ctx);
	delete b;
}

static int batch_check_errors(smhv_batch *b, const char *what) {
	BatchError *e = b->h_err;
	if (!e) return SMHV_OK;
	const uint32_t count = __atomic_load_n(&e->count, __ATOMIC_ACQUIRE);
	if (count == 0) return SMHV_OK;
	const BatchError snap = *e;
	memset(e, 0, sizeof *e);
	logf(b->ctx, 1, "%s: %u frame(s) failed, first: frame %u status %u", what, count, snap.frame, snap.status);
	if (snap.status == SMHV_FRAME_LSD_STUCK)
		return fail(SMHV_E_STATE, "%s: %u frame(s) without marker lines (status != 0 in their records); first: frame %u, line search gave up "
		            "(SMHV_FRAME_LSD_STUCK: head %u tail %u list %u/%u lines %u rounds %u spec %u head-state %u)", what, count, snap.frame,
		            snap.info[0], snap.info[1], snap.info[2], snap.info[3], snap.info[4], snap.info[5], snap.info[6], snap.info[7]);
	return fail(SMHV_E_STATE, "%s: %u frame(s) failed; first: frame %u, status %u", what, count, snap.frame, snap.status);
}
extern "C" int smhv_internal_batch_check(smhv_batch *b, const char *what) { return b ? batch_check_errors(b, what) : SMHV_OK; }

extern "C" SMHV_API int smhv_batch_layout_get(smhv_batch *b, smhv_batch_layout *o) {
	if (!b || !o) return fail(SMHV_E_INVALID, "bad arguments");
	const Geom &g = b->g;
	memset(o, 0, sizeof *o);
	o->frame_w = g.W; o->frame_h = g.H;
	o->roi[0] = g.rx; o->roi[1] = g.ry; o->roi[2] = g.rw; o->roi[3] = g.rh;
	o->button[0] = g.bx; o->button[1] = g.by; o->button[2] = g.bw; o->button[3] = g.bh;
	o->brq_w = g.qw; o->brq_h = g.qh;
	o->ui_pitch = g.ui_pitch; o->ui_stride = g.ui_stride; o->ui_offset = (uint64_t)g.m_xoff * 4;
	o->mask_pitch = g.mask_pitch; o->mask_stride = g.mask_stride; o->mask_offset = g.m_xoff;
	o->ocr_pitch = g.ocr_pitch; o->ocr_stride = g.ocr_stride; o->ocr_offset = g.q_xoff;
	o->scales_pitch = g.ocr_pitch; o->scales_stride = g.ocr_stride; o->scales_offset = g.q_xoff;
	o->bits_pitch_words = g.bits_pitch_w; o->bits_stride = g.bits_stride_w * 4; o->bits_xoff = g.m_xoff;
	return SMHV_OK;
}

extern "C" SMHV_API int smhv_batch_enable_timing(smhv_batch *b, int enable) {
	if (!b) return fail(SMHV_E_INVALID, "null batch");
	if (enable && !b->ev) {
		HIPCHK(hipSetDevice(b->ctx->device));
		b->ev = new hipEvent_t[smhv_batch::TIMING_RING][smhv_batch::TIMING_EVENTS]();
		for (int r = 0; r < smhv_batch::TIMING_RING; ++r)
			for (int i = 0; i < smhv_batch::TIMING_EVENTS; ++i) HIPCHK(hipEventCreate(&b->ev[r][i]));
	}
	b->timing = enable != 0;
	b->timed_runs = 0;
	return SMHV_OK;
}

static void hm_release(smhv_heightmap *hm) {
	if (!hm || hm->refs.fetch_sub(1, std::memory_order_acq_rel) != 1) return;
	(void)hipSetDevice(hm->ctx->device);
	(void)hipDeviceSynchronize();
	if (hm->d) (void)hipFree(hm->d);
	if (uint32_t *l = hm->d_lut.load(std::memory_order_acquire)) (void)hipFree(l);
	ctx_release(hm->ctx);
	delete hm;
}

static smhv_firing_options firing_opts(const smhv_firing_options *opt) {
	smhv_firing_options o{};
	o.size = sizeof o;
	if (opt) { o.flags = opt->flags; o.viewport_scale[0] = opt->viewport_scale[0]; o.viewport_scale[1] = opt->viewport_scale[1];
	           o.viewport_top_left[0] = opt->viewport_top_left[0]; o.viewport_top_left[1] = opt->viewport_top_left[1]; }
	if (o.viewport_scale[0] == 0.0f) o.viewport_scale[0] = 1.0f;
	if (o.viewport_scale[1] == 0.0f) o.viewport_scale[1] = 1.0f;
	return o;
}

static void firing_run_params(const smhv_heightmap *hm, const smhv_firing_options *o, FiringRun *r) {
	memset(r, 0, sizeof *r);
	if (hm) {
		r->hm = hm->d; r->hm_w = hm->w; r->hm_h = hm->h;
		r->b0x = (float)hm->bounds[0]; r->b0y = (float)hm->bounds[1];
		r->zscale = (double)hm->scale[2] / 0.1953125;
	}
	r->flags = o->flags;
// ... 42 lines not shown
	}
	firing_run_params(b->fire_hm, &b->fire_opt, st->h);
	st->h->out = b->d_firing;
	HIPCHK(hipMemcpyAsync(b->d_fire_run, st->h, sizeof(FiringRun), hipMemcpyHostToDevice, sb));
	HIPCHK(hipEventRecord(st->done, sb));
	return SMHV_OK;
}

static int hm_lut(const smhv_heightmap *hm, const uint32_t **lut) {
	uint32_t *l = hm->d_lut.load(std::memory_order_acquire);
	if (!l) {
		std::lock_guard<std::mutex> lk(hm->lut_mu);
		l = hm->d_lut.load(std::memory_order_relaxed);
		if (!l) {
			HIPCHK(hipSetDevice(hm->ctx->device));
			hipStream_t s = nullptr;
			hipError_t e = hipMalloc((void **)&l, sizeof(uint32_t) * SMH_HM_LUT_WORDS);
			if (e == hipSuccess) e = hipStreamCreateWithFlags(&s, hipStreamNonBlocking);
			if (e == hipSuccess) e = launch_heightmap_lut(hm->d, (uint64_t)hm->w * hm->h, l + SMH_HM_LUT_ENTRIES, l, s);
			if (e == hipSuccess) e = launch_heightmap_lut16(l, (uint16_t *)(l + SMH_HM_LUT_ENTRIES + 4u), l + SMH_HM_LUT_ENTRIES + 2u, s);
			if (e == hipSuccess) e = hipStreamSynchronize(s);
			if (s) (void)hipStreamDestroy(s);
			if (e != hipSuccess) {
				if (l) (void)hipFree(l);
				return fail(SMHV_E_HIP, "heightmap overlay colour table: %s", hipGetErrorString(e));
			}
			hm->d_lut.store(l, std::memory_order_release);
		}
	}
	*lut = l;
	return SMHV_OK;
}

static int overlay_prepare(smhv_batch *b, const smhv_heightmap *hm, uint32_t flags, const smhv_frame_result *res, hipStream_t s, OverlayRun *r) {
	const uint32_t *lut = nullptr;
	int rc = hm_lut(hm, &lut);
	if (rc) return rc;
	if (!b->d_overlay) {
		const size_t bytes = b->g.ui_stride * (size_t)b->max_frames;
		hipError_t e = hipMalloc((void **)&b->d_overlay, bytes);
		if (e == hipSuccess) e = hipMemsetAsync(b->d_overlay, 0, bytes, s);
		if (e != hipSuccess) {
			if (b->d_overlay) (void)hipFree(b->d_overlay);
			b->d_overlay = nullptr;
			return fail(SMHV_E_HIP, "overlay slab: %s", hipGetErrorString(e));
		}
	}
	memset(r, 0, sizeof *r);
	r->ui = b->d_ui; r->out = b->d_overlay; r->aux = b->d_aux; r->res = res;
	r->hm = hm->d; r->lut = lut; r->hm_w = hm->w; r->hm_h = hm->h;
	r->b0x = (float)hm->bounds[0]; r->b0y = (float)hm->bounds[1];
	r->flags = flags;
	return SMHV_OK;
}

static int check_overlay_stages(uint32_t stages, const smhv_heightmap *hm) {
	if (!(stages & SMHV_STAGE_HEIGHTMAP_OVERLAY)) return SMHV_OK;
	if ((stages & (SMHV_STAGE_UI_MAP | SMHV_STAGE_MINIMAP)) != (SMHV_STAGE_UI_MAP | SMHV_STAGE_MINIMAP))
		return fail(SMHV_E_INVALID, "SMHV_STAGE_HEIGHTMAP_OVERLAY needs SMHV_STAGE_UI_MAP and SMHV_STAGE_MINIMAP");
	if (!hm) return fail(SMHV_E_INVALID, "SMHV_STAGE_HEIGHTMAP_OVERLAY needs a heightmap (smhv_batch_set_firing / smhv_pipeline_set_firing)");
	return SMHV_OK;
}

static int batch_materialize_mask(smhv_batch *b, hipStream_t stream) {
	std::lock_guard<std::mutex> lk(b->mask_mu);
	if (b->mask_stale) {
		HIPCHK(launch_mask_expand(b->g, b->d_bits, b->d_mask, std::min(b->mask_stale, b->max_frames), stream));
		HIPCHK(hipEventRecord(b->ev_mask, stream));
		b->mask_stale = 0;
	} else HIPCHK(hipStreamWaitEvent(stream, b->ev_mask, 0));
	return SMHV_OK;
}

static int batch_materialize_ui(smhv_batch *b, hipStream_t stream) {
	std::lock_guard<std::mutex> lk(b->ui_mu);
	if (b->ui_stale) {
		HIPCHK(launch_ui_expand(b->g, b->d_ui_luma, b->d_ui, b->d_ui_form, std::min(b->ui_stale, b->max_frames), stream));
		HIPCHK(hipEventRecord(b->ev_ui, stream));
		b->ui_stale = 0;
	} else HIPCHK(hipStreamWaitEvent(stream, b->ev_ui, 0));
	return SMHV_OK;
}

struct SvcPublish { SvcCtl *ctl; unsigned long long *ring; SvcSlot *slots; uint32_t slot, seq, ring_log2; const uint32_t *cull_tab; bool have_cull; hipStream_t s_pro; hipEvent_t ev_pro;
                    bool *published; };
static int batch_run_impl(smhv_batch *b, const void *d_frames, uint32_t n, uint32_t stages, int grayscale, uint32_t max_gap,
                          const smhv_anchors *anchors, hipStream_t s, hipStream_t sl, const SvcPublish *svc = nullptr) {
	if (!b || !d_frames || n == 0 || n > b->max_frames) return fail(SMHV_E_INVALID, "bad arguments (n=%u, capacity %u)", n, b ? b->max_frames : 0);
	if ((uintptr_t)d_frames & 3u) return fail(SMHV_E_INVALID, "d_frames is not aligned to a pixel (4 bytes)");
	CTX_OPEN(b->ctx);
	if ((stages & (SMHV_STAGE_ALL | SMHV_STAGE_MINIMAP)) == 0) return fail(SMHV_E_INVALID, "no stage selected");
	if ((stages & SMHV_STAGE_FIRING) && !(stages & SMHV_STAGE_MARKERS)) return fail(SMHV_E_INVALID, "SMHV_STAGE_FIRING needs SMHV_STAGE_MARKERS");
	{ int rc = check_overlay_stages(stages, b->fire_hm); if (rc) return rc; }
	stages &= SMHV_STAGE_ALL | SMHV_STAGE_MINIMAP | SMHV_STAGE_EXACT_STATS | SMHV_STAGE_LSD_HELPERS | SMHV_STAGE_FIRING | SMHV_STAGE_HEIGHTMAP_OVERLAY;
	HIPCHK(hipSetDevice(b->ctx->device));
	const Geom &g = b->g;
	Buffers bf = make_buffers(b, (const uint8_t *)d_frames, 0);
	OverlayRun orun{};
	if (stages & SMHV_STAGE_HEIGHTMAP_OVERLAY) {
		int rc = batch_materialize_ui(b, s);
		if (rc) return rc;
		rc = overlay_prepare(b, b->fire_hm, b->fire_opt.flags, bf.results, s, &orun);
		if (rc) return rc;
	}
	if ((bf.co.epoch & 0xFFFFu) == 0u && b->d_farm) HIPCHK(hipMemsetAsync(b->d_farm, 0, sizeof(FarmFrame) * (size_t)b->max_frames, s));
	if (stages & SMHV_STAGE_LSD_HELPERS) bf.co.ctl = (LsdCtl *)b->d_lsd_ctl;
	if (svc && svc->have_cull) bf.cull_tab = svc->cull_tab;
	else if ((stages & SMHV_STAGE_MARKERS) && !(stages & SMHV_STAGE_EXACT_STATS)) {
		int rc = sector_table_for(b->ctx, max_gap, s, &bf);
		if (rc) return rc;
	}
	const bool scales = (stages & SMHV_STAGE_SCALES) && anchors;
	const hipStream_t sb = (svc && svc->s_pro) ? svc->s_pro : s;
	if (scales) {
		smhv_batch::AnchorStage *st = nullptr;
		for (auto &a : b->anchor_stage)
			if (hipEventQuery(a.done) == hipSuccess) { st = &a; break; }
		if (!st) {
			smhv_batch::AnchorStage a;
			hipError_t e = hipHostMalloc((void **)&a.h, sizeof(smhv_anchors) * b->max_frames);
			if (e == hipSuccess) e = hipEventCreateWithFlags(&a.done, hipEventDisableTiming);
			if (e != hipSuccess) { if (a.h) (void)hipHostFree(a.h); return fail(SMHV_E_HIP, "anchor staging: %s", hipGetErrorString(e)); }
			b->anchor_stage.push_back(a);
			st = &b->anchor_stage.back();
		}
		memcpy(st->h, anchors, sizeof(smhv_anchors) * n);
		HIPCHK(hipMemcpyAsync(b->d_anchors, st->h, sizeof(smhv_anchors) * n, hipMemcpyHostToDevice, sb));
		HIPCHK(hipEventRecord(st->done, sb));
	}
	if (stages & SMHV_STAGE_FIRING) {
		int rc = firing_upload(b, sb);
		if (rc) return rc;
		bf.firing = b->d_fire_run;
	}
	const bool t = b->timing;
	hipEvent_t *ev = t ? b->ev[b->timed_runs % smhv_batch::TIMING_RING] : nullptr;
#define STAGE_BEGIN(i, st) do { if (t) HIPCHK(hipEventRecord(ev[2 * (i)], (st))); } while (0)
#define STAGE_END(i, st) do { if (t) HIPCHK(hipEventRecord(ev[2 * (i) + 1], (st))); } while (0)
	const bool ui_stage = (stages & SMHV_STAGE_UI_MAP) != 0u;
	bool ui_lazy = false;
	if (ui_stage) {
		std::lock_guard<std::mutex> lk(b->ui_mu);
		ui_lazy = grayscale && !(stages & SMHV_STAGE_HEIGHTMAP_OVERLAY) && !b->ui_eager;
		if (ui_lazy) { b->ui_stale = std::max(b->ui_stale, n); bf.ui = b->d_ui_luma; }
	}
	const int pass_gray = ui_lazy ? 2 : (grayscale ? 1 : 0);
	STAGE_BEGIN(0, sb);
	HIPCHK(launch_button(g, bf, n, 0, sb, b->d_ui_form, ui_stage ? (ui_lazy ? UI_FORM_LUMA : UI_FORM_RGBA) : UI_FORM_KEEP));
	STAGE_END(0, sb);
	if (sb != s) {
		HIPCHK(hipEventRecord(svc->ev_pro, sb));
		HIPCHK(hipStreamWaitEvent(s, svc->ev_pro, 0));
	}
	uint32_t mflags = 0, qflags = 0;
	if (stages & SMHV_STAGE_MARKERS) mflags |= MAP_MASK;
	if (stages & SMHV_STAGE_UI_MAP) mflags |= MAP_UI;
	if (stages & SMHV_STAGE_OCR) qflags |= BRQ_OCR;
	if (scales) qflags |= BRQ_SCALES;
	if (b->probe) HIPCHK(hipEventRecord(b->ev_probe[0], s));
	STAGE_BEGIN(1, s);
	if (mflags && qflags) HIPCHK(launch_map_brq_pass(g, bf, n, mflags, qflags, pass_gray, 0, 1, s, &b->tune));
	else if (mflags) HIPCHK(launch_map_pass(g, bf, n, mflags, pass_gray, s, true, b->tune.map_overlapped != 0u));
	if (mflags & MAP_MASK) {
		std::lock_guard<std::mutex> lk(b->mask_mu);
		if (b->mask_eager) HIPCHK(launch_mask_expand(g, b->d_bits, b->d_mask, n, s));
		else b->mask_stale = std::max(b->mask_stale, n);
	}
	STAGE_END(1, s);
	if (mflags & MAP_UI) { b->ui_written = true; b->ui_gray = grayscale != 0; }
	if (mflags & MAP_MASK) b->mask_written = true;
	if (qflags & BRQ_OCR) b->ocr_written = true;
	if (qflags & BRQ_SCALES) b->scales_written = true;
	STAGE_BEGIN(2, s);
	if (qflags && !mflags) HIPCHK(launch_brq_pass(g, bf, n, qflags, 0, 1, s));
	STAGE_END(2, s);
	if (!svc) HIPCHK(hipEventRecord(b->ev_map_done, s));
	if (b->probe) HIPCHK(hipEventRecord(b->ev_probe[1], s));
	if (sl != s) HIPCHK(hipStreamWaitEvent(sl, b->ev_map_done, 0));
	const bool skip_lsd = g_skip_lsd.load(std::memory_order_relaxed);
	if (svc) {
		if (stages & SMHV_STAGE_MINIMAP) HIPCHK(launch_find_minimap(g, bf, n, s));
		if (stages & SMHV_STAGE_HEIGHTMAP_OVERLAY) HIPCHK(launch_hm_overlay(g, orun, n, s));
		bf.rec_stages = SMH_REC_ON | (scales ? stages : (stages & ~SMHV_STAGE_SCALES));
		bf.rec_bars = b->d_bars;
		STAGE_BEGIN(3, s);
		HIPCHK(launch_svc_publish(svc->ctl, svc->ring, svc->slots, svc->slot, bf, n, svc->seq, svc->ring_log2, s));
		if (svc->published) *svc->published = true;
		STAGE_END(3, s);
		STAGE_BEGIN(4, s);
		STAGE_END(4, s);
		if (t) b->timed_runs++;
		return SMHV_OK;
	}
	STAGE_BEGIN(3, sl);
	const uint32_t late_kc = b->lsd_late_kc;
	if (late_kc > 0u) { bf.lsd_flags |= SMH_LSD_LATE_HELP; bf.lsd_late_kc = late_kc; }
	bool record_fused = false;
	if (!(stages & SMHV_STAGE_MINIMAP)) {
		bf.rec_stages = SMH_REC_ON | (scales ? stages : (stages & ~SMHV_STAGE_SCALES));
		bf.rec_bars = b->d_bars;
	}
	if ((stages & SMHV_STAGE_MARKERS) && !skip_lsd) HIPCHK(launch_lsd(g, bf, n, (float)max_gap, 0, 0.0f, 0.0f, sl, b->lsd_fork.s1 ? &b->lsd_fork : nullptr, b->lsd_bs, b->lsd_prefer_classic,
	                                                      (mflags && qflags) ? b->tune.lsd_tile_limit : 0u,
	                                                      &record_fused));
	STAGE_END(3, sl);
	if (b->probe) { HIPCHK(hipEventRecord(b->ev_probe[2], sl)); b->probe_valid = (stages & SMHV_STAGE_MARKERS) && mflags; }
	if (stages & SMHV_STAGE_MINIMAP) HIPCHK(launch_find_minimap(g, bf, n, sl));
	if (stages & SMHV_STAGE_HEIGHTMAP_OVERLAY) HIPCHK(launch_hm_overlay(g, orun, n, sl));
	STAGE_BEGIN(4, sl);
	if (record_fused) {  }
	else if (scales) HIPCHK(launch_scales_finalize(g, bf, n, stages, b->d_bars, sl));
	else HIPCHK(launch_finalize(g, bf, n, stages & ~SMHV_STAGE_SCALES, sl));
	STAGE_END(4, sl);
#undef STAGE_BEGIN
#undef STAGE_END
	if (t) b->timed_runs++;
	return SMHV_OK;
}

extern "C" SMHV_API int smhv_batch_run(smhv_batch *b, const void *d_frames, uint32_t n, uint32_t stages, int grayscale, uint32_t max_gap,
                                       const smhv_anchors *anchors, void *stream) {
	return batch_run_impl(b, d_frames, n, stages, grayscale, max_gap, anchors, (hipStream_t)stream, (hipStream_t)stream);
}

extern "C" SMHV_API int smhv_debug_pattern_copy(smhv_batch *b, const void *d_frames, uint32_t n, uint32_t rows_in_flight, void *stream) {
	if (!b || !d_frames || n == 0 || n > b->max_frames || (rows_in_flight != 0u && rows_in_flight != 4u && rows_in_flight != 8u && rows_in_flight != 12u))
		return fail(SMHV_E_INVALID, "bad arguments (rows in flight: 0 = 4, 4, 8, 12)");
	CTX_OPEN(b->ctx);
	HIPCHK(hipSetDevice(b->ctx->device));
	const Buffers bf = make_buffers(b, (const uint8_t *)d_frames, 0);
	HIPCHK(launch_pattern_copy(b->g, bf, n, rows_in_flight, (hipStream_t)stream));
	return SMHV_OK;
}

extern "C" SMHV_API int smhv_batch_wait_map_pass(smhv_batch *b, void *stream) {
	if (!b) return fail(SMHV_E_INVALID, "null batch");
	HIPCHK(hipSetDevice(b->ctx->device));
	HIPCHK(hipStreamWaitEvent((hipStream_t)stream, b->ev_map_done, 0));
	return SMHV_OK;
}

extern "C" SMHV_API int smhv_batch_set_scales_stream(smhv_batch *b, void *stream) {
	if (!b) return fail(SMHV_E_INVALID, "null batch");
	(void)stream;
	return SMHV_OK;
}

extern "C" SMHV_API int smhv_batch_stage_ms(smhv_batch *b, float ms[5]) {
	if (!b || !ms) return fail(SMHV_E_INVALID, "bad arguments");
	if (!b->ev || b->timed_runs == 0) return fail(SMHV_E_STATE, "no timed smhv_batch_run since timing was enabled");
	const uint64_t runs = b->timed_runs < (uint64_t)smhv_batch::TIMING_RING ? b->timed_runs : (uint64_t)smhv_batch::TIMING_RING;
	double acc[5] = {0, 0, 0, 0, 0};
	for (uint64_t r = 0; r < runs; ++r) {
		hipEvent_t *ev = b->ev[(b->timed_runs - 1 - r) % smhv_batch::TIMING_RING];
		for (int i = 0; i < 5; ++i) {
			float m = 0;
			HIPCHK(hipEventSynchronize(ev[2 * i + 1]));
			HIPCHK(hipEventElapsedTime(&m, ev[2 * i], ev[2 * i + 1]));
			acc[i] += m;
		}
	}
	for (int i = 0; i < 5; ++i) ms[i] = (float)(acc[i] / (double)runs);
	b->timed_runs = 0;
	return SMHV_OK;
}

extern "C" SMHV_API int smhv_batch_lsd_coop_stats(smhv_batch *b, uint32_t first, uint32_t n, uint32_t *out) {
	if (!b || !out || (uint64_t)first + n > b->max_frames) return fail(SMHV_E_INVALID, "bad arguments");
	HIPCHK(hipSetDevice(b->ctx->device));
	HIPCHK(hipDeviceSynchronize());
	std::vector<LsdCoop> h(n);
	HIPCHK(hipMemcpy(h.data(), b->d_lsd_ctl + sizeof(LsdCtl) + sizeof(LsdCoop) * (size_t)first, sizeof(LsdCoop) * n, hipMemcpyDeviceToHost));
	for (uint32_t i = 0; i < n; ++i) { out[4 * i] = h[i].stat_groups; out[4 * i + 1] = h[i].stat_hits; out[4 * i + 2] = h[i].stat_casts; out[4 * i + 3] = h[i].req_tail; }
	return SMHV_OK;
}

extern "C" SMHV_API int smhv_batch_device_ptrs(smhv_batch *b, void **r, void **ui, void **mask, void **ocr, void **scales, void **bits) {
	if (!b) return fail(SMHV_E_INVALID, "null batch");
	if (r) *r = b->d_results;
	if (ui) {
		CTX_OPEN(b->ctx);
		HIPCHK(hipSetDevice(b->ctx->device));
		{ std::lock_guard<std::mutex> lk(b->ui_mu); b->ui_eager = true; }
		HIPCHK(hipDeviceSynchronize());
		int rc = batch_materialize_ui(b, b->ctx->s_main);
		if (rc) return rc;
		HIPCHK(wait_stream(b->ctx->s_main));
		*ui = b->d_ui;
	}
	if (mask) {
		CTX_OPEN(b->ctx);
		HIPCHK(hipSetDevice(b->ctx->device));
		{ std::lock_guard<std::mutex> lk(b->mask_mu); b->mask_eager = true; }
		HIPCHK(hipDeviceSynchronize());
		int rc = batch_materialize_mask(b, b->ctx->s_main);
		if (rc) return rc;
		HIPCHK(wait_stream(b->ctx->s_main));
		*mask = b->d_mask;
	}
	if (ocr) *ocr = b->d_ocr;
	if (scales) *scales = b->d_scales;
	if (bits) *bits = b->d_bits;
	return SMHV_OK;
}

extern "C" SMHV_API int smhv_batch_tile_mask(smhv_batch *b, void **d_tiled, void **d_occ, uint32_t geometry[4]) {
	if (!b) return fail(SMHV_E_INVALID, "null batch");
	if (d_tiled) *d_tiled = b->d_tiled;
	if (d_occ) *d_occ = b->d_occ;
	if (geometry) { geometry[0] = tiled_rows(b->g); geometry[1] = b->g.bits_pitch_w; geometry[2] = occ_pitch(b->g); geometry[3] = b->g.m_xoff; }
	return SMHV_OK;
}

extern "C" SMHV_API int smhv_batch_read_tile_mask(smhv_batch *b, uint32_t frame, uint32_t *tiled, uint8_t *occ, uint32_t *bits, int *written) {
	if (!b || frame >= b->max_frames) return fail(SMHV_E_INVALID, "bad arguments");
	HIPCHK(hipSetDevice(b->ctx->device));
	HIPCHK(hipDeviceSynchronize());
	const Geom &g = b->g;
	if (tiled) HIPCHK(hipMemcpy(tiled, b->d_tiled + (size_t)frame * tiled_stride_w(g), tiled_stride_w(g) * 4, hipMemcpyDeviceToHost));
	if (occ) HIPCHK(hipMemcpy(occ, b->d_occ + (size_t)frame * occ_stride(g), occ_stride(g), hipMemcpyDeviceToHost));
	if (bits) HIPCHK(hipMemcpy(bits, b->d_bits + (size_t)frame * g.bits_stride_w, g.bits_stride_w * 4, hipMemcpyDeviceToHost));
	if (written) {
		FrameAux a;
		HIPCHK(hipMemcpy(&a, b->d_aux + frame, sizeof a, hipMemcpyDeviceToHost));
		*written = a.tiles ? 1 : 0;
	}
	return SMHV_OK;
}

extern "C" SMHV_API int smhv_batch_read_results(smhv_batch *b, uint32_t first, uint32_t n, smhv_frame_result *out) {
	if (!b || !out || (uint64_t)first + n > b->max_frames) return fail(SMHV_E_INVALID, "bad arguments");
	HIPCHK(hipSetDevice(b->ctx->device));
	HIPCHK(hipDeviceSynchronize());
	HIPCHK(hipMemcpy(out, b->d_results + first, sizeof(smhv_frame_result) * n, hipMemcpyDeviceToHost));
	return batch_check_errors(b, "batch_read_results");
}

static int copy_image_d2h(smhv_ctx *c, int slot, uint8_t *dst, const uint8_t *d_rows, size_t pitch, size_t xoff, size_t width, size_t rows, hipStream_t s) {
	const size_t bytes = pitch * rows;
	if (c->h_stage_cap[slot] < bytes) {
		if (c->h_stage[slot]) { (void)hipHostFree(c->h_stage[slot]); c->h_stage[slot] = nullptr; c->h_stage_cap[slot] = 0; }
		HIPCHK(hipHostMalloc((void **)&c->h_stage[slot], bytes, hipHostMallocDefault));
		c->h_stage_cap[slot] = bytes;
	}
	HIPCHK(hipMemcpyAsync(c->h_stage[slot], d_rows, bytes, hipMemcpyDeviceToHost, s));
	HIPCHK(wait_stream(s));
	for (size_t r = 0; r < rows; ++r) memcpy(dst + r * width, c->h_stage[slot] + r * pitch + xoff, width);
	return SMHV_OK;
}

extern "C" SMHV_API int smhv_batch_read_image(smhv_batch *b, int which, uint32_t frame, uint8_t *out) {
	if (!b || !out || frame >= b->max_frames) return fail(SMHV_E_INVALID, "bad arguments");
	CTX_OPEN(b->ctx);
	const Geom &g = b->g;
	HIPCHK(hipSetDevice(b->ctx->device));
	HIPCHK(hipDeviceSynchronize());
	if (which == SMHV_IMAGE_HEIGHTMAP_OVERLAY && !b->d_overlay) return fail(SMHV_E_STATE, "batch_read_image: no run of this batch had SMHV_STAGE_HEIGHTMAP_OVERLAY");
	switch (which) {
	case 100:
	case SMHV_IMAGE_HEIGHTMAP_OVERLAY:
		{
			int rc = batch_materialize_ui(b, b->ctx->s_main);
			if (rc) return rc;
			HIPCHK(wait_stream(b->ctx->s_main));
		}
		HIPCHK(hipMemcpy2D(out, (size_t)g.rw * 4, (which == 100 ? b->d_ui : b->d_overlay) + frame * g.ui_stride + (size_t)g.m_xoff * 4, g.ui_pitch, (size_t)g.rw * 4,
		                   g.rh, hipMemcpyDeviceToHost));
		break;
	case SMHV_VIEW_LSD_INPUT: {
		std::lock_guard<std::mutex> lk(b->ctx->mu);
		int rc = batch_materialize_mask(b, b->ctx->s_main);
		if (rc) return rc;
		return copy_image_d2h(b->ctx, 2, out, b->d_mask + frame * g.mask_stride, g.mask_pitch, g.m_xoff, g.rw, g.rh, b->ctx->s_main);
	}
	case SMHV_VIEW_OCR_INPUT: {
		std::lock_guard<std::mutex> lk(b->ctx->mu);
		return copy_image_d2h(b->ctx, 2, out, b->d_ocr + frame * g.ocr_stride, g.ocr_pitch, g.q_xoff, g.qw, g.qh, b->ctx->s_main);
	}
	case SMHV_VIEW_FIND_SCALES_INPUT: {
		std::lock_guard<std::mutex> lk(b->ctx->mu);
		return copy_image_d2h(b->ctx, 2, out, b->d_scales + frame * g.ocr_stride, g.ocr_pitch, g.q_xoff, g.qw, g.qh, b->ctx->s_main);
	}
	default:
		return fail(SMHV_E_INVALID, "unsupported image id %d", which);
	}
	return SMHV_OK;
}

static std::atomic<int> g_own_queues[64];
struct smhv_pipeline {
	smhv_ctx *ctx = nullptr;
	uint32_t depth = 0;
	smhv_pipeline_options opt{};
	std::vector<smhv_batch *> batch;
	std::vector<hipStream_t> stream;
	std::vector<hipEvent_t> done;
	std::vector<hipEvent_t> hold;
	std::vector<char> held;
	std::vector<hipStream_t> last_sl;
	hipEvent_t ev_after = nullptr;
	LaunchTuning tuning{0u, 0u, 0u, 0u};
	bool adapt = false, tune_on = true;
	float ratio_ema = 0.0f;
	uint64_t submitted = 0;
	uint64_t round_start = 0;
	bool svc = false;
	uint32_t svc_compact = 0;
	uint32_t svc_streams = 0, svc_waves = 0, svc_part_words = 0, svc_tile_cap = 0, svc_list_cap = 0, svc_lds = 0, svc_wgs = 0, svc_ring_log2 = 0;
	SvcCtl *d_svc_ctl = nullptr;
	unsigned long long *d_svc_ring = nullptr;
	SvcSlot *d_svc_slots = nullptr;
	SvcHost *h_svc = nullptr, *d_svc_host = nullptr;
	SvcRemote *d_svc_remote = nullptr;
	uint32_t *d_svc_store = nullptr;
	uint32_t svc_store_words = 0;
	hipStream_t s_search = nullptr, s_pro = nullptr;
	std::mutex peek_mu;
	hipStream_t s_peek = nullptr;
	SvcCtl *h_peek = nullptr;
	smhv_heightmap *fire_hm = nullptr;
	smhv_firing_options fire_opt{};
	std::vector<hipEvent_t> ev_pub;
	std::vector<hipEvent_t> ev_pro;
	std::vector<uint32_t> seq;
	std::vector<hipStream_t> slot_st;
	uint32_t seq_counter = 0, svc_epoch = 0;
	bool svc_key_valid = false;
	const uint32_t *svc_cull = nullptr;
	uint32_t svc_max_gap = 0;
	std::vector<hipStream_t> svc_stream;
	std::vector<uint8_t> slot_frame;
	bool adaptive = false, mode_frame = false;
	uint32_t own_queues = 0;
	struct ModeCtl {
		uint32_t phase = 0, count = 0, settle = 0, key_n = 0, key_stages = 0, key_gap = 0, decisions = 0;
		uint32_t cand_n = 0, cand_stages = 0, cand_gap = 0, cand_count = 0;
		uint32_t remeasured = 0;
		bool window_mixed = false;
		uint64_t frames = 0;
		struct timespec t0{};
		double rate[2] = {0.0, 0.0};
	} mc;
};
static int svc_wait_slot(smhv_pipeline *p, uint32_t slot);
static int slot_wait(smhv_pipeline *p, uint32_t slot) {
	if (p->svc && p->slot_frame[slot]) return svc_wait_slot(p, slot);
	HIPCHK(wait_event(p->done[slot]));
	return SMHV_OK;
}
static int svc_launch(smhv_pipeline *p, uint32_t slot);
static int svc_submit(smhv_pipeline *p, uint32_t slot, const void *d_frames, uint32_t n, uint32_t stages, int grayscale, uint32_t max_gap,
                      const smhv_anchors *anchors, void *after_stream, uint32_t *slot_out);

extern "C" SMHV_API void smhv_pipeline_destroy(smhv_pipeline *p) {
	if (!p) return;
	if (p->ctx) (void)hipSetDevice(p->ctx->device);
	if (p->svc) for (uint32_t i = 0; i < p->depth && i < p->slot_frame.size(); ++i) if (p->slot_frame[i]) (void)svc_wait_slot(p, i);
	(void)hipDeviceSynchronize();
	for (auto b : p->batch) if (b) smhv_batch_destroy(b);
// ... 1370 lines not shown
			q->slot_pixels[slot] = layout;
			q->crc_state[slot] = 1;
			q->jobs.push_back(slot);
		}
		q->cv_job.notify_one();
		q->head++;
		q->acquired = false;
		return SMHV_OK;
	}
	if (layout == SMHV_PIXELS_BGRA8) {
		HIPCHK(hipMemcpyAsync(q->d_stage[slot], q->h_stage[slot], q->frame_bytes, hipMemcpyHostToDevice, q->s));
	} else if (yuv) {
		if (!q->d_raw[slot]) HIPCHK(hipMalloc((void **)&q->d_raw[slot], q->frame_bytes));
		HIPCHK(hipMemcpyAsync(q->d_raw[slot], q->h_stage[slot], yuv_tight_bytes(q->W, q->H), hipMemcpyHostToDevice, q->s));
		YuvRun run{};
		run.src = q->d_raw[slot]; run.dst = q->d_stage[slot]; run.W = q->W; run.H = q->H; run.n = 1; run.k = yuv_coef(yd);
		run.r[0] = yuv_tight_rect(q->W, q->H, yd.layout);
		HIPCHK(launch_yuv_to_bgra(run, 1, yd.layout, yd.bilinear, q->s));
	} else {
		if (!q->d_raw[slot]) HIPCHK(hipMalloc((void **)&q->d_raw[slot], q->frame_bytes));
		HIPCHK(hipMemcpyAsync(q->d_raw[slot], q->h_stage[slot], q->frame_bytes / 4 * bpp, hipMemcpyHostToDevice, q->s));
		HIPCHK(launch_to_bgra(q->d_raw[slot], q->d_stage[slot], (uint64_t)q->W * q->H, layout, q->s));
	}
	HIPCHK(hipMemsetAsync(q->d_acc + slot, 0, sizeof(uint32_t), q->s));
	HIPCHK(launch_crc32(q->d_stage[slot], q->frame_bytes / 4, q->wgs, q->rounds, q->x_skip, q->d_x_local, q->d_x_wg, q->d_acc + slot, q->s));
	HIPCHK(hipMemcpyAsync(q->h_acc + slot, q->d_acc + slot, sizeof(uint32_t), hipMemcpyDeviceToHost, q->s));
	HIPCHK(hipEventRecord(q->done[slot], q->s));
	q->head++;
	q->acquired = false;
	return SMHV_OK;
}

extern "C" SMHV_API int smhv_ingest_commit(smhv_ingest *q) { return smhv_ingest_commit_pixels(q, SMHV_PIXELS_BGRA8); }

extern "C" SMHV_API int smhv_ingest_push_pixels(smhv_ingest *q, const uint8_t *pixels, uint32_t layout) {
	if (!q || !pixels) return fail(SMHV_E_INVALID, "ingest_push: null argument");
	const uint32_t bpp = pixel_layout_bytes(layout);
	YuvDesc yd;
	if (!bpp && !yuv_decode(layout, &yd)) return fail(SMHV_E_INVALID, "ingest_push_pixels: unknown pixel layout 0x%x", layout);
	if (q->roi && bpp && layout != SMHV_PIXELS_BGRA8) return fail(SMHV_E_INVALID, "ingest_push_pixels: a queue created with SMHV_INGEST_ROI_UPLOAD takes BGRA8, NV12 and I420 frames only");
	uint8_t *dst = nullptr;
	int rc = smhv_ingest_acquire(q, &dst);
	if (rc) return rc;
	memcpy(dst, pixels, bpp ? q->frame_bytes / 4 * bpp : (size_t)yuv_tight_bytes(q->W, q->H));
	return smhv_ingest_commit_pixels(q, layout);
}

namespace smh { extern std::atomic<uint32_t> g_map_band_rows, g_map_band_major; }
extern "C" SMHV_API int smhv_debug_map_band_rows(uint32_t rows) {
	g_map_band_major.store((rows >> 31) ? 1u : ((rows >> 30) & 1u) ? 2u : 0u, std::memory_order_relaxed);
	rows &= 0x3FFFFFFFu;
	if (rows & 7u) return fail(SMHV_E_INVALID, "debug_map_band_rows: a multiple of 8 (0: the library's rule)");
	g_map_band_rows.store(rows, std::memory_order_relaxed);
	return SMHV_OK;
}

extern "C" SMHV_API int smhv_debug_band_rows(uint32_t frame_w, uint32_t frame_h, uint32_t n, int fused, uint32_t *rows, uint32_t *bands, int *tiles) {
	Geom g;
	int rc = compute_geom(frame_w, frame_h, &g);
	if (rc) return rc;
	uint32_t rb = 0;
	map_band_rows(g.rh, n ? n : 1u, fused, &rb, tiles);
	if (rows) *rows = rb;
	if (bands) *bands = (g.rh + rb - 1) / rb;
	return SMHV_OK;
}

extern "C" SMHV_API int smhv_debug_batch_mask_state(smhv_batch *b, uint32_t *stale_frames, int *eager) {
	if (!b) return fail(SMHV_E_INVALID, "null batch");
	std::lock_guard<std::mutex> lk(b->mask_mu);
	if (stale_frames) *stale_frames = b->mask_stale;
	if (eager) *eager = b->mask_eager ? 1 : 0;
	return SMHV_OK;
}

extern "C" SMHV_API int smhv_debug_batch_ui_state(smhv_batch *b, uint32_t *stale_frames, int *eager) {
	if (!b) return fail(SMHV_E_INVALID, "null batch");
	std::lock_guard<std::mutex> lk(b->ui_mu);
	if (stale_frames) *stale_frames = b->ui_stale;
	if (eager) *eager = b->ui_eager ? 1 : 0;
	return SMHV_OK;
}

extern "C" SMHV_API int smhv_debug_batch_materialize_ui(smhv_batch *b, void *stream) {
	if (!b) return fail(SMHV_E_INVALID, "null batch");
	CTX_OPEN(b->ctx);
	HIPCHK(hipSetDevice(b->ctx->device));
	return batch_materialize_ui(b, (hipStream_t)stream);
}

extern "C" SMHV_API int smhv_debug_mask_expand(smhv_batch *b, uint32_t n, void *stream) {
	if (!b || n == 0 || n > b->max_frames) return fail(SMHV_E_INVALID, "debug_mask_expand: bad arguments");
	CTX_OPEN(b->ctx);
	HIPCHK(hipSetDevice(b->ctx->device));
	HIPCHK(launch_mask_expand(b->g, b->d_bits, b->d_mask, n, (hipStream_t)stream));
	return SMHV_OK;
}

extern "C" SMHV_API int smhv_debug_ingest_feed(smhv_ingest *q, uint32_t n, uint32_t *counter) { return smhv_debug_ingest_feed_pixels(q, n, counter, SMHV_PIXELS_BGRA8); }

extern "C" SMHV_API int smhv_debug_ingest_feed_pixels(smhv_ingest *q, uint32_t n, uint32_t *counter, uint32_t pixels) {
	if (!q || !counter) return fail(SMHV_E_INVALID, "ingest_feed: null argument");
	for (uint32_t i = 0; i < n; ++i) {
		uint8_t *buf = nullptr;
		int rc = smhv_ingest_acquire(q, &buf);
		if (rc) return rc;
		const uint32_t c = (*counter)++;
		buf[0] = (uint8_t)c; buf[1] = (uint8_t)(c >> 8); buf[2] = (uint8_t)(c >> 16); buf[3] = 255;
		rc = smhv_ingest_commit_pixels(q, pixels);
		if (rc) return rc;
	}
	return SMHV_OK;
}

extern "C" SMHV_API int smhv_ingest_push(smhv_ingest *q, const uint8_t *bgra) { return smhv_ingest_push_pixels(q, bgra, SMHV_PIXELS_BGRA8); }

extern "C" SMHV_API int smhv_ingest_batch(smhv_ingest *q, const void **d_frames, uint32_t *n, uint32_t *last_crc) {
	if (!q || !d_frames || !n) return fail(SMHV_E_INVALID, "ingest_batch: null argument");
	if (q->acquired) return fail(SMHV_E_INVALID, "ingest_batch: a staging buffer is acquired but not committed");
	HIPCHK(hipSetDevice(q->ctx->device));
	while (q->tail < q->head) {
		int rc = ingest_resolve_one(q);
		if (rc == INGEST_FULL) break;
		if (rc) return rc;
	}
	HIPCHK(wait_stream(q->s));
	if (q->roi) HIPCHK(wait_stream(q->s_alt));
	*d_frames = q->d_slab; *n = q->count;
	if (last_crc) *last_crc = q->last_crc;
	return SMHV_OK;
}

extern "C" SMHV_API int smhv_ingest_reset(smhv_ingest *q) {
	if (!q) return fail(SMHV_E_INVALID, "ingest_reset: null argument");
	if (q->acquired) return fail(SMHV_E_INVALID, "ingest_reset: a staging buffer is acquired but not committed");
	q->count = 0;
	return SMHV_OK;
}

extern "C" SMHV_API int smhv_ingest_counts(smhv_ingest *q, uint64_t *n_new, uint64_t *n_dup) {
	if (!q) return fail(SMHV_E_INVALID, "ingest_counts: null argument");
	if (n_new) *n_new = q->n_new;
	if (n_dup) *n_dup = q->n_dup;
	return SMHV_OK;
}

extern "C" SMHV_API int smhv_heightmap_create(smhv_ctx *c, const uint16_t *data, uint32_t w, uint32_t h, const int32_t bounds[4], const float scale[3],
                                              smhv_heightmap **out) {
	if (!c || !data || !bounds || !scale || !out) return fail(SMHV_E_INVALID, "heightmap_create: null argument");
	*out = nullptr;
	CTX_OPEN(c);
	if (w == 0 || h == 0 || (uint64_t)w * h > (1ull << 28)) return fail(SMHV_E_INVALID, "heightmap_create: %u x %u texels (1 .. 2^28)", w, h);
	HIPCHK(hipSetDevice(c->device));
	smhv_heightmap *hm = new (std::nothrow) smhv_heightmap();
	if (!hm) return fail(SMHV_E_INVALID, "out of host memory");
	hm->w = w; hm->h = h;
	memcpy(hm->bounds, bounds, sizeof hm->bounds);
	memcpy(hm->scale, scale, sizeof hm->scale);
	const size_t bytes = (size_t)w * h * sizeof(uint16_t);
	hipError_t e = hipMalloc((void **)&hm->d, bytes);
	if (e == hipSuccess) e = hipMemcpy(hm->d, data, bytes, hipMemcpyHostToDevice);
	if (e != hipSuccess) {
		if (hm->d) (void)hipFree(hm->d);
		delete hm;
		return fail(SMHV_E_HIP, "heightmap_create: %s", hipGetErrorString(e));
	}
// ... 338 lines not shown

static int check_render_layers(const smhv_render_layers *ly, const char *what) {
	if (!ly) return fail(SMHV_E_INVALID, "%s: null layers", what);
	if (ly->size != sizeof(smhv_render_layers)) return fail(SMHV_E_INVALID, "%s: smhv_render_layers.size %u != %zu", what, ly->size, sizeof(smhv_render_layers));
	if (ly->flags & ~SMHV_LAYER_MINIMAP_BOUNDS) return fail(SMHV_E_INVALID, "%s: unknown layer flags 0x%x", what, ly->flags);
	if (ly->map_source > (uint32_t)SMHV_VIEW_CROPPED_BRQ) return fail(SMHV_E_INVALID, "%s: unknown map source %u", what, ly->map_source);
	if (ly->n_prims > SMHV_RENDER_MAX_PRIMS) return fail(SMHV_E_INVALID, "%s: %u prims (at most %u)", what, ly->n_prims, SMHV_RENDER_MAX_PRIMS);
	if (ly->n_prims && !ly->prims) return fail(SMHV_E_INVALID, "%s: %u prims and a null pointer", what, ly->n_prims);
	for (uint32_t i = 0; i < ly->n_prims; ++i) {
		const smhv_render_prim &p = ly->prims[i];
		if ((p.kind & ~(0xFFu | SMHV_PRIM_FOREGROUND | SMHV_PRIM_SHIFT1)) || (p.kind & 0xFFu) > SMHV_PRIM_RECT)
			return fail(SMHV_E_INVALID, "%s: prim %u has the unknown kind 0x%x", what, i, p.kind);
		if (p.rgba[3] != 255u) return fail(SMHV_E_INVALID, "%s: prim %u has alpha %u (255 only)", what, i, p.rgba[3]);
	}
	return SMHV_OK;
}

static int render_upload_prims(smhv_batch *b, const smhv_render_layers *ly, RenderLayersRun *y, hipStream_t s) {
	if (ly->n_prims == 0u) return SMHV_OK;
	const size_t cap = sizeof(smhv_render_prim) * (size_t)SMHV_RENDER_MAX_PRIMS;
	if (!b->h_prims) HIPCHK(hipHostMalloc((void **)&b->h_prims, cap));
	if (!b->d_prims) HIPCHK(hipMalloc((void **)&b->d_prims, cap));
	if (!b->ev_prims) HIPCHK(hipEventCreateWithFlags(&b->ev_prims, hipEventDisableTiming));
	else HIPCHK(wait_event(b->ev_prims));
	uint32_t k = 0;
	for (uint32_t pass = 0; pass < 2u; ++pass) {
		for (uint32_t i = 0; i < ly->n_prims; ++i)
			if (((ly->prims[i].kind & SMHV_PRIM_FOREGROUND) != 0u) == (pass == 1u)) b->h_prims[k++] = ly->prims[i];
		if (pass == 0u) y->n_below = k;
	}
	y->n_fg = k - y->n_below;
	y->prims = b->d_prims;
	HIPCHK(hipMemcpyAsync(b->d_prims, b->h_prims, sizeof(smhv_render_prim) * (size_t)k, hipMemcpyHostToDevice, s));
	HIPCHK(hipEventRecord(b->ev_prims, s));
	return SMHV_OK;
}

extern "C" SMHV_API int smhv_batch_render_layers(smhv_batch *b, uint32_t first, uint32_t n, const smhv_heightmap *hm, const smhv_render_options *opt,
                                                 const smhv_render_layers *layers, void *stream) {
	if (!b) return fail(SMHV_E_INVALID, "batch_render_layers: null batch");
	CTX_OPEN(b->ctx);
	int rc = check_render_options(opt, hm, "batch_render_layers");
	if (rc) return rc;
	rc = check_render_layers(layers, "batch_render_layers");
	if (rc) return rc;
	if (n == 0u || (uint64_t)first + n > b->max_frames) return fail(SMHV_E_INVALID, "batch_render_layers: frames [%u, %u + %u) of a batch of %u", first, first, n, b->max_frames);
	if (!b->ui_written) return fail(SMHV_E_STATE, "batch_render_layers: no run of this batch has produced a ui_map (SMHV_STAGE_UI_MAP)");
	const Geom &g = b->g;
	RenderLayersRun y{};
	y.flags = layers->flags;
	y.src_mode = SMH_RND_SRC_UI; y.src_w = g.rw; y.src_h = g.rh;
	switch ((int)layers->map_source) {
	case SMHV_VIEW_NONE: break;
	case SMHV_VIEW_OCR_INPUT:
	case SMHV_VIEW_FIND_SCALES_INPUT: {
		const bool ocr = layers->map_source == (uint32_t)SMHV_VIEW_OCR_INPUT;
		if (!(ocr ? b->ocr_written : b->scales_written))
			return fail(SMHV_E_STATE, "batch_render_layers: no run of this batch has produced the %s image", ocr ? "OCR input (SMHV_STAGE_OCR)" : "scales input (SMHV_STAGE_SCALES with anchors)");
		y.src_mode = SMH_RND_SRC_GRAY; y.src = (ocr ? b->d_ocr : b->d_scales) + (size_t)first * g.ocr_stride;
		y.src_pitch = g.ocr_pitch; y.src_stride = g.ocr_stride; y.src_xoff = g.q_xoff; y.src_w = g.qw; y.src_h = g.qh;
		break;
	}
	case SMHV_VIEW_LSD_INPUT:
		if (!b->mask_written) return fail(SMHV_E_STATE, "batch_render_layers: no run of this batch has produced the marker mask (SMHV_STAGE_MARKERS)");
		y.src_mode = SMH_RND_SRC_GRAY; y.src = b->d_mask + (size_t)first * g.mask_stride;
		y.src_pitch = g.mask_pitch; y.src_stride = g.mask_stride; y.src_xoff = g.m_xoff;
		break;
	default:
		if (b->ui_gray) return fail(SMHV_E_STATE, "batch_render_layers: the batch's ui_map is grayscale, map source %u needs the colour one", layers->map_source);
		if (layers->map_source == (uint32_t)SMHV_VIEW_CROPPED_BRQ) {
			y.src_mode = SMH_RND_SRC_CROPPED; y.src_w = g.rw / 2u; y.src_h = g.rh / 2u;
			if (y.src_w == 0u || y.src_h == 0u) return fail(SMHV_E_STATE, "batch_render_layers: the map has no bottom right quarter");
		} else y.src_mode = SMH_RND_SRC_PREPROCESS;
		break;
	}
	HIPCHK(hipSetDevice(b->ctx->device));
	const bool use_hm = (opt->flags & SMHV_RENDER_HEIGHTMAP) != 0u;
	RenderRun r;
	rc = render_prepare(b, first, n, b->d_results + first, use_hm ? hm : nullptr, opt, &r);
	if (rc) return rc;
	hipStream_t s = (hipStream_t)stream;
	if (layers->map_source == (uint32_t)SMHV_VIEW_LSD_INPUT) {
		rc = batch_materialize_mask(b, s);
		if (rc) return rc;
	}
	rc = batch_materialize_ui(b, s);
	if (rc) return rc;
	rc = render_upload_prims(b, layers, &y, s);
	if (rc) return rc;
	render_bind(b, use_hm ? hm : nullptr);
	for (uint32_t done = 0; done < n;) {
		const uint32_t k = std::min(n - done, 65535u);
		RenderRun part = r;
		part.ui += (size_t)done * g.ui_stride; part.out += (size_t)done * r.out_stride; part.aux += done; part.res += done;
		RenderLayersRun yp = y;
		if (yp.src) yp.src += (size_t)done * y.src_stride;
		HIPCHK(launch_render_map_layers(g, part, yp, k, s));
		done += k;
	}
	HIPCHK(hipEventRecord(b->ev_render, s));
	return SMHV_OK;
}

extern "C" SMHV_API int smhv_render_map_layers(smhv_ctx *c, const smhv_heightmap *hm, const smhv_render_options *opt, const smhv_render_layers *layers,
                                               const smhv_line *lines, uint32_t n_lines, uint8_t *rgba) {
	int rc = require_open(c, "render_map_layers");
	if (rc) return rc;
	CTX_OPEN(c);
	if (!rgba || (n_lines && !lines)) return fail(SMHV_E_INVALID, "render_map_layers: null argument");
	if (n_lines > SMHV_RENDER_MAX_LINES) return fail(SMHV_E_INVALID, "render_map_layers: %u lines (at most %u)", n_lines, SMHV_RENDER_MAX_LINES);
	rc = check_render_options(opt, hm, "render_map_layers");
	if (rc) return rc;
	rc = check_render_layers(layers, "render_map_layers");
	if (rc) return rc;
	HIPCHK(hipSetDevice(c->device));
	smhv_batch *b = c->fb;
	const Geom &g = b->g;
	const bool use_hm = (opt->flags & SMHV_RENDER_HEIGHTMAP) != 0u;
	std::lock_guard<std::mutex> lk(c->fire_mu);
	RenderRun r;
	rc = render_prepare(b, 0, 1, b->d_results + 3, use_hm ? hm : nullptr, opt, &r);
	if (rc) return rc;
	RenderLayersRun y{};
	y.flags = layers->flags;
	y.src_mode = SMH_RND_SRC_UI; y.src_w = g.rw; y.src_h = g.rh;
	uint8_t *d_view = nullptr;
	if (layers->map_source != (uint32_t)SMHV_VIEW_NONE) {
		const int which = (int)layers->map_source;
		const bool brq = which == SMHV_VIEW_OCR_INPUT || which == SMHV_VIEW_FIND_SCALES_INPUT || which == SMHV_VIEW_CROPPED_BRQ;
		y.src_w = brq ? g.qw : g.rw; y.src_h = brq ? g.qh : g.rh;
		HIPCHK(hipMalloc((void **)&d_view, (size_t)y.src_w * y.src_h * 4u));
		Buffers bf = make_buffers(b, c->frame_ptr, 0);
		hipError_t e = launch_debug_view(g, bf, 0, which, c->isolated ? 1 : 0, d_view, c->s_main);
		if (e != hipSuccess) { (void)hipFree(d_view); return fail(SMHV_E_HIP, "render_map_layers: debug view: %s", hipGetErrorString(e)); }
		y.src_mode = SMH_RND_SRC_RGBA; y.src = d_view; y.src_pitch = (uint64_t)y.src_w * 4u;
	}
	const auto run = [&]() -> int {
		const size_t line_bytes = sizeof(smhv_line) * (size_t)SMHV_RENDER_MAX_LINES;
		if (c->fire_cap < line_bytes) {
			if (c->d_fire) (void)hipFree(c->d_fire);
			if (c->h_fire) (void)hipHostFree(c->h_fire);
			c->d_fire = c->h_fire = nullptr; c->fire_cap = 0;
			HIPCHK(hipMalloc((void **)&c->d_fire, line_bytes));
			HIPCHK(hipHostMalloc((void **)&c->h_fire, line_bytes));
			c->fire_cap = line_bytes;
		}
		if (n_lines && (opt->flags & SMHV_RENDER_MARKERS)) {
			memcpy(c->h_fire, lines, sizeof(smhv_line) * (size_t)n_lines);
			HIPCHK(hipMemcpyAsync(c->d_fire, c->h_fire, sizeof(smhv_line) * (size_t)n_lines, hipMemcpyHostToDevice, c->s_main));
			r.lines = (const smhv_line *)c->d_fire; r.n_lines = n_lines;
		} else
			r.flags &= ~SMHV_RENDER_MARKERS;
		int rc2 = render_upload_prims(b, layers, &y, c->s_main);
		if (rc2) return rc2;
		HIPCHK(launch_render_map_layers(g, r, y, 1, c->s_main));
		HIPCHK(hipEventRecord(b->ev_render, c->s_main));
		std::lock_guard<std::mutex> lk2(c->mu);
		return copy_image_d2h(c, 2, rgba, b->d_render, (size_t)r.out_stride / opt->out_h, 0, (size_t)opt->out_w * 4, opt->out_h, c->s_main);
	};
	rc = run();
	if (d_view) {
		if (rc) (void)hipStreamSynchronize(c->s_main);
		(void)hipFree(d_view);
	}
	return rc;
}
// ... 28 lines not shown
```

squad-mortar-helper_amd/csrc/smh_stream.hip:

```cpp
#include <algorithm>
#include <atomic>
#include <cstdlib>

#include "smh_device.h"

namespace smh {

__device__ __forceinline__ uint32_t tile_occupancy(uint64_t rows_any, uint32_t lane, uint32_t ntr, uint8_t *occp, uint32_t pitch) {
	uint32_t alo = (uint32_t)rows_any, ahi = (uint32_t)(rows_any >> 32);
	alo |= SMH_DPP(alo, 0x101); ahi |= SMH_DPP(ahi, 0x101);
	alo |= SMH_DPP(alo, 0x102); ahi |= SMH_DPP(ahi, 0x102);
	alo |= SMH_DPP(alo, 0x104); ahi |= SMH_DPP(ahi, 0x104);
	uint32_t occ = 0;
#pragma unroll
	for (int t = 0; t < 4; ++t) occ |= (((alo >> (8 * t)) & 255u) ? 1u : 0u) << t;
#pragma unroll
	for (int t = 0; t < 3; ++t) occ |= (((ahi >> (8 * t)) & 255u) ? 1u : 0u) << (4 + t);
	if (lane & 7u) occ = 0u;
	uint32_t mine = 0;
#pragma unroll
	for (int t = 0; t < 7; ++t) {
		const uint64_t bal = __ballot((occ >> t) & 1u) & 0x0101010101010101ull;
		const uint32_t byte = (uint32_t)((bal * 0x0102040810204080ull) >> 56);
		if (lane == (uint32_t)t) mine = byte;
	}
	if (lane < ntr) occp[(size_t)lane * pitch] = (uint8_t)mine;
	return occ;
}

__global__ void __launch_bounds__(256) k_button(Geom g, Buffers b, int force_open, uint8_t *ui_form, uint32_t ui_luma) {
	const uint32_t f = blockIdx.x;
	const uint8_t *fp = b.frames + (size_t)f * g.frame_bytes;
	__shared__ uint32_t s_cnt;
	if (threadIdx.x == 0) s_cnt = 0;
	__syncthreads();
	uint32_t cnt = 0;
	const uint32_t npx = g.bw * g.bh;
	constexpr uint32_t U = 8;
	for (uint32_t i0 = threadIdx.x; i0 < npx; i0 += blockDim.x * U) {
		uint32_t p[U];
#pragma unroll
		for (uint32_t k = 0; k < U; ++k) {
			const uint32_t i = min(i0 + k * blockDim.x, npx - 1u);
			const uint32_t y = i / g.bw, x = i - y * g.bw;
			p[k] = *(const uint32_t *)(fp + ((size_t)(g.by + y) * g.W + g.bx + x) * 4);
		}
#pragma unroll
		for (uint32_t k = 0; k < U; ++k) {
			const uint32_t bb = p[k] & 255u, gg = (p[k] >> 8) & 255u, rr = (p[k] >> 16) & 255u;
			const bool red = absdiff(SMH_BUTTON_R, rr) <= SMH_BUTTON_TOLERANCE && absdiff(SMH_BUTTON_G, gg) <= SMH_BUTTON_TOLERANCE &&
			                 absdiff(SMH_BUTTON_B, bb) <= SMH_BUTTON_TOLERANCE;
			cnt += (red && i0 + k * blockDim.x < npx) ? 1u : 0u;
		}
	}
	cnt = wave_sum32(cnt);
	if ((threadIdx.x & 63) == 0) atomicAdd(&s_cnt, cnt);
	__syncthreads();
	if (threadIdx.x == 0) {
		const uint32_t red = s_cnt;
		const float ratio = (float)red / (float)npx;
		FrameAux a;
		a.open = (force_open || !(ratio < SMH_BUTTON_RED_PIXEL_THRESHOLD)) ? 1u : 0u;
		a.red = red; a.n_mask_px = 0;
		a.y_min = 0xFFFFFFFFu; a.y_max = 0; a.w_min = 0xFFFFFFFFu; a.w_max = 0; a.tiles = 0;
		b.aux[f] = a;
		if (ui_form && ui_luma != UI_FORM_KEEP && a.open) ui_form[f] = (uint8_t)ui_luma;
	}
}

#define MAP_RB_MAX 62

template <bool GRAY, bool TILES>
__global__ void __launch_bounds__(1024) k_map_pass(Geom g, Buffers b, uint32_t flags, uint32_t RB) {
	constexpr int GRAYF = GRAY ? 1 : 0;
#include "smh_map_pass.inc"
}
template <bool TILES>
__global__ void __launch_bounds__(1024) k_map_pass_luma(Geom g, Buffers b, uint32_t flags, uint32_t RB) {
	constexpr int GRAYF = 2;
#include "smh_map_pass.inc"
}

#define BRQ_RB 58

__global__ void __launch_bounds__(1024) k_brq_pass(Geom g, Buffers b, uint32_t flags, uint32_t fixed_start_y, int use_anchor_start) {
	const uint32_t f = blockIdx.y;
	if (!b.aux[f].open) return;
	uint32_t start_y = fixed_start_y;
	bool do_scales = (flags & BRQ_SCALES) != 0;
	if (use_anchor_start) {
		const smhv_anchors an = b.anchors[f];
		start_y = an.scales_start_y;
		if (an.n == 0 || start_y > g.qh) do_scales = false;
	}
	const bool do_ocr = (flags & BRQ_OCR) != 0;
	const uint32_t q = threadIdx.x, lane = q & 63u, wave = q >> 6, nwave = blockDim.x >> 6;
	const int r0 = (int)(blockIdx.x * BRQ_RB);
	const int r1 = min(r0 + BRQ_RB, (int)g.qh);
	const bool qact = q < g.q_quads;
	uint32_t vmask = 0, wmask = 0;
#pragma unroll
	for (int c = 0; c < 4; ++c) {
		const uint32_t x = 4 * q + c - g.q_xoff;
		if (x < g.qw) vmask |= 1u << c;
		if (x + SMH_OCR_DILATE_RADIUS <= g.qw) wmask |= 1u << c;
	}
	if (!qact) { vmask = 0; wmask = 0; }
	wmask &= vmask;

	const uint8_t *fp = b.frames + (size_t)f * g.frame_bytes + ((size_t)g.qy * g.W + g.q_ax + 4 * q) * 4;
	const size_t row_bytes = (size_t)g.W * 4;
	uint8_t *op = b.ocr + (size_t)f * g.ocr_stride + (size_t)q * 4;
	uint8_t *sp = b.scales + (size_t)f * g.ocr_stride + (size_t)q * 4;

	uint64_t Wb[4] = {0, 0, 0, 0}, Eb[4] = {0, 0, 0, 0};
	const int rs = max(r0 - 3, 0), re = min(r1 + 2, (int)g.qh - 1);
	const uint8_t *lp = qact ? fp : fp - (size_t)q * 16;
	uint4 nx[4];
#pragma unroll
	for (int k = 0; k < 4; ++k) nx[k] = *(const uint4 *)(lp + (size_t)min(rs + k, re) * row_bytes);
	for (int r = rs; r <= re; r += 4) {
		uint4 px[4];
#pragma unroll
		for (int k = 0; k < 4; ++k) px[k] = nx[k];
		if (r + 4 <= re) {
#pragma unroll
			for (int k = 0; k < 4; ++k) nx[k] = *(const uint4 *)(lp + (size_t)min(r + 4 + k, re) * row_bytes);
		}
#pragma unroll
		for (int k = 0; k < 4; ++k) {
			const int row = r + k;
			if (row > re) break;
			const int bit = row - (r0 - 3);
			const uint32_t pv[4] = {px[k].x, px[k].y, px[k].z, px[k].w};
			const bool out_row = row >= r0 && row < r1;
			const bool nb_row = (uint32_t)row + SMH_OCR_DILATE_RADIUS <= g.qh;
			uint32_t ocr_w = 0, sc_w = 0;
#pragma unroll
			for (int c = 0; c < 4; ++c) {
				const uint32_t p = pv[c], bb = p & 255u, gg = (p >> 8) & 255u, rr8 = (p >> 16) & 255u;
				const uint32_t mx = max(rr8, max(gg, bb)), mn = min(rr8, min(gg, bb));
				const bool w = (mx == mn) && mn >= SMH_OCR_BRIGHTNESS_THRESHOLD;
				const bool e = (4u * (mx - mn) <= SMH_OCR_SIMILARITY_EDGE_THRESHOLD) && mn >= SMH_OCR_BRIGHTNESS_EDGE_THRESHOLD && !w;
				const bool valid = (vmask >> c) & 1u;
				Wb[c] |= (uint64_t)((w && nb_row && ((wmask >> c) & 1u)) ? 1u : 0u) << bit;
				Eb[c] |= (uint64_t)((e && valid && out_row) ? 1u : 0u) << bit;
				const uint32_t l = luma8(rr8, gg, bb);
				ocr_w |= ((w && valid) ? (255u - l) : 255u) << (8 * c);
				sc_w |= (l != 0u ? 255u : 0u) << (8 * c);
// ... 43 lines not shown
				k &= k - 1;
				const int row = r0 - 3 + bit;
				const uint32_t p = *(const uint32_t *)(fp + (size_t)row * row_bytes + 4 * c);
				const uint32_t l = luma8((p >> 16) & 255u, (p >> 8) & 255u, p & 255u);
				op[(size_t)row * g.ocr_pitch + c] = (uint8_t)(255u - l);
			}
		}
	}
}

#define MAPQ_RB_MAX 58
std::atomic<uint32_t> g_map_band_major{0};
std::atomic<uint32_t> g_map_band_rows{0};
static inline uint32_t band_rows_for(uint32_t rh, uint32_t n, uint32_t rb_cap, bool tiles_wanted = true, bool beside_service = false) {
	const uint32_t rb8 = rb_cap & ~7u, forced = g_map_band_rows.load(std::memory_order_relaxed);
	uint32_t RB = rb_cap;
	if (tiles_wanted && forced) RB = std::min(rb8, forced);
	else if (tiles_wanted && rh <= 900u) RB = beside_service ? rb8 : 24u;
	else if (tiles_wanted && (rh + rb8 - 1) / rb8 == (rh + rb_cap - 1) / rb_cap) RB = rb8;
	const uint64_t fill = RB == 24u ? 768u : 512u;
	while (RB > 8 && (uint64_t)((rh + RB - 1) / RB) * n < fill) RB = (RB & 7u) ? (RB + 1) / 2 : (RB > 32 ? 32 : RB > 16 ? 16 : 8);
	return RB;
}

typedef uint32_t u32x4 __attribute__((ext_vector_type(4)));
#ifdef SMH_TRACKED_LOADS
#define SMH_LD128(dst, voff, sbase) (dst) = *(const u32x4 *)((sbase) + (voff))
#else
#define SMH_LD128(dst, voff, sbase) asm volatile("global_load_dwordx4 %0, %1, %2 ; smh-load" : "=v"(dst) : "v"(voff), "s"(sbase) : "memory")
#endif
#define SMH_ST128(voff, data, sbase) asm volatile("global_store_dwordx4 %0, %1, %2" : : "v"(voff), "v"(data), "s"(sbase) : "memory")
#define SMH_ST32(voff, data, sbase) asm volatile("global_store_dword %0, %1, %2" : : "v"(voff), "v"(data), "s"(sbase) : "memory")
#ifdef SMH_TRACKED_LOADS
#define SMH_WAIT_SET(n, X) ((void)0)
#else
#define SMH_WAIT_SET(n, X) asm volatile("s_waitcnt vmcnt(" #n ") ; smh-release" : "+v"((X)[0]), "+v"((X)[1]), "+v"((X)[2]), "+v"((X)[3]) : : "memory")
#endif
__device__ __forceinline__ uint32_t luma_bgra(uint32_t p) {
	const float l = SMH_LUMA_R * (float)((p >> 16) & 255u) + SMH_LUMA_G * (float)((p >> 8) & 255u) + SMH_LUMA_B * (float)(p & 255u);
	return (uint32_t)l;
}
__device__ __forceinline__ uint32_t bright4(const uint32_t pv[4]) {
	uint32_t acc = 0;
#pragma unroll
	for (int c = 0; c < 4; ++c) acc |= ((pv[c] & 0x007F7F7Fu) + 0x004E4E4Eu) & pv[c];
	return acc & 0x00808080u;
}
__device__ __forceinline__ uint32_t ones_to_bytes(uint32_t ones) { return __builtin_amdgcn_perm(0u, 0u, ones + 0x0C0C0C0Cu); }
__device__ __forceinline__ uint32_t nib_to_bytes(uint32_t nib) {
	return ones_to_bytes((nib * 0x00204081u) & 0x01010101u);
}
__device__ __forceinline__ uint32_t rows_of_col(uint32_t nibbles, int c) {
	const uint32_t y = (nibbles >> c) & 0x1111u;
	return (y | (y >> 3) | (y >> 6) | (y >> 9)) & 0xFu;
}

#ifndef SMH_MAP_ITEM_INLINE
#define SMH_MAP_ITEM_INLINE __forceinline__
#endif
struct MapKernelArgs { Geom g; Buffers b; uint32_t flags, qflags, RB, fixed_start_y; int use_anchor_start; uint32_t nbands, items; };
#ifdef __HIP_DEVICE_COMPILE__
typedef const __attribute__((address_space(4))) MapKernelArgs *MapKernelArgsPtr;
#else
typedef const MapKernelArgs *MapKernelArgsPtr;
#endif
template <int GRAY, int SETS, bool TILES>
__device__ SMH_MAP_ITEM_INLINE void map_brq_item(MapKernelArgsPtr ka, uint32_t f, uint32_t band0) {
	constexpr int GR = 4;
	const Geom g = ka->g;
	const Buffers b = ka->b;
	const uint32_t flags = ka->flags, qflags = ka->qflags, RB = ka->RB, fixed_start_y = ka->fixed_start_y;
	const int use_anchor_start = ka->use_anchor_start;
	if (!b.aux[f].open) return;
	const uint32_t band = band0;
	constexpr bool live = true;
	uint32_t start_y = fixed_start_y;
	bool do_scales = (qflags & BRQ_SCALES) != 0;
	if (use_anchor_start && do_scales) {
		const smhv_anchors an = b.anchors[f];
		start_y = an.scales_start_y;
		if (an.n == 0 || start_y > g.qh) do_scales = false;
	}
	const bool do_ocr = (qflags & BRQ_OCR) != 0;
	const uint32_t q = threadIdx.x, lane = q & 63u, wave = q >> 6;
	const uint32_t nwave = blockDim.x >> 6, gwave = wave;
	const int r0 = live ? (int)(band * RB) : 0;
	const int r1 = live ? min(r0 + (int)RB, (int)g.rh) : 0;
	const bool qact = q < g.m_quads && live;
	uint32_t vmask = 0;
#pragma unroll
	for (int c = 0; c < 4; ++c)
		if ((uint32_t)(4 * q + c - g.m_xoff) < g.rw) vmask |= 1u << c;
	if (!qact) vmask = 0;
	const int qy0 = (int)(g.qy - g.ry);
	const int qq = (int)q - (int)((g.q_ax - g.m_ax) >> 2);
	const bool in_q = qq >= 0 && (uint32_t)qq < g.q_quads && qact;
	uint32_t qv = 0, qw_ = 0;
#pragma unroll
	for (int c = 0; c < 4; ++c) {
		const uint32_t x = (uint32_t)(4 * qq + c) - g.q_xoff;
		if (in_q && x < g.qw) qv |= 1u << c;
		if (in_q && x + SMH_OCR_DILATE_RADIUS <= g.qw) qw_ |= 1u << c;
	}
	qw_ &= qv;
	const int qr0 = max(r0 - qy0, 0), qr1 = min(r1 - qy0, (int)g.qh);
	const bool band_q = qr1 > qr0 && (do_ocr || do_scales);

	const uint8_t *fbase = b.frames + (size_t)f * g.frame_bytes + ((size_t)g.ry * g.W + g.m_ax) * 4;
	const uint32_t loff = qact ? q * 16u : 0u;
	const uint8_t *fp = fbase + (size_t)q * 16;
	uint8_t *uibase = b.ui + (size_t)f * (GRAY == 2 ? g.ui_stride >> 2 : g.ui_stride);
	uint8_t *op = b.ocr + (size_t)f * g.ocr_stride;
	uint8_t *sp = b.scales + (size_t)f * g.ocr_stride;
	const uint32_t qoff = (uint32_t)(in_q ? qq : 0) * 4u;
	const size_t row_bytes = (size_t)g.W * 4;

	uint64_t P[4] = {0, 0, 0, 0}, Wb[4] = {0, 0, 0, 0}, Eb[4] = {0, 0, 0, 0};
	extern __shared__ __attribute__((aligned(16))) uint32_t s_dyn[];
	auto or_w = [&](int c, uint64_t v) { Wb[c] |= v; };
	auto or_e = [&](int c, uint64_t v) { Eb[c] |= v; };
	auto get_w = [&](int c) -> uint64_t { return Wb[c]; };
	auto get_e = [&](int c) -> uint64_t { return Eb[c]; };
	const int rs = max(r0 - 1, 0), re = min(r1, (int)g.rh - 1);
	const bool do_ui = (flags & MAP_UI) != 0, do_mask = (flags & MAP_MASK) != 0;
	const int base = r0 - 3;
	const bool my_q = band_q && in_q;
	const bool wave_q = band_q && __any(in_q);

	if (my_q && do_ocr && live) {
#pragma unroll
		for (int k = 0; k < 4; ++k) {
			const int row = k < 2 ? r0 - 3 + k : r1 + k - 1;
			const int qrow = row - qy0;
			if (qrow < 0 || qrow >= (int)g.qh || row < 0 || row >= (int)g.rh) continue;
			if ((uint32_t)qrow + SMH_OCR_DILATE_RADIUS > g.qh) continue;
			const uint4 v = *(const uint4 *)(fp + (size_t)row * row_bytes);
			const uint32_t pv[4] = {v.x, v.y, v.z, v.w};
#pragma unroll
			for (int c = 0; c < 4; ++c) {
				const uint32_t p = pv[c], bb = p & 255u, gg = (p >> 8) & 255u, rr8 = (p >> 16) & 255u;
				const uint32_t mx = max(rr8, max(gg, bb)), mn = min(rr8, min(gg, bb));
				const bool w = (mx == mn) && mn >= SMH_OCR_BRIGHTNESS_THRESHOLD && ((qw_ >> c) & 1u);
				or_w(c, (uint64_t)(w ? 1u : 0u) << (row - base));
			}
		}
	}

	uint32_t *s_hits = s_dyn;
	auto rare = [](bool c) -> bool { if constexpr (TILES) return __builtin_expect(c, 0); else return c; };
	auto group = [&](const u32x4 (&px)[GR], int r) {
		uint32_t prehits = 0, wrows = 0, erows = 0;
#pragma unroll
		for (int k = 0; k < GR; ++k) {
			const int row = r + k;
			if (row > re) break;
			const uint32_t pv[4] = {px[k].x, px[k].y, px[k].z, px[k].w};
			const bool out_row = row >= r0 && row < r1;
			const int qrow = row - qy0;
			const bool q_row = wave_q && qrow >= 0 && qrow < (int)g.qh;
			uint32_t wnib = 0, enib = 0;
			if (q_row) {
#pragma unroll
				for (int c = 0; c < 4; ++c) {
					const uint32_t p = pv[c], bb = p & 255u, gg = (p >> 8) & 255u, rr8 = (p >> 16) & 255u;
					const uint32_t mx = max(rr8, max(gg, bb)), mn = min(rr8, min(gg, bb));
					const bool w = (mx == mn) && mn >= SMH_OCR_BRIGHTNESS_THRESHOLD;
					const bool e = (4u * (mx - mn) <= SMH_OCR_SIMILARITY_EDGE_THRESHOLD) && mn >= SMH_OCR_BRIGHTNESS_EDGE_THRESHOLD && !w;
					wnib |= (w ? 1u : 0u) << c;
					enib |= (e ? 1u : 0u) << c;
				}
				const bool nb_row = (uint32_t)qrow + SMH_OCR_DILATE_RADIUS <= g.qh;
				if (nb_row) wrows |= (wnib & qw_) << (4 * k);
				if (out_row) erows |= (enib & qv) << (4 * k);
			}
			if (out_row) {
				uint32_t lum[4] = {0, 0, 0, 0};
				if (GRAY || q_row) {
#pragma unroll
					for (int c = 0; c < 4; ++c) lum[c] = luma_bgra(pv[c]);
				}
				if constexpr (GRAY == 2) {
					if (do_ui && qact) SMH_ST32(loff >> 2, lum[0] | (lum[1] << 8) | (lum[2] << 16) | (lum[3] << 24), uibase + (size_t)row * (g.ui_pitch >> 2));
				} else if (do_ui && qact) {
					u32x4 o;
					uint32_t ov[4];
#pragma unroll
					for (int c = 0; c < 4; ++c) {
						const uint32_t p = pv[c], bb = p & 255u, gg = (p >> 8) & 255u, rr8 = (p >> 16) & 255u;
						if (GRAY) ov[c] = __builtin_amdgcn_perm(0u, lum[c], 0x0D000000u);
						else ov[c] = rr8 | (gg << 8) | (bb << 16) | 0xFF000000u;
					}
					o.x = ov[0]; o.y = ov[1]; o.z = ov[2]; o.w = ov[3];
					SMH_ST128(loff, o, uibase + (size_t)row * g.ui_pitch);
				}
				if (q_row && in_q) {
					const uint32_t l4 = lum[0] | (lum[1] << 8) | (lum[2] << 16) | (lum[3] << 24);
					if (do_ocr) SMH_ST32(qoff, ~(l4 & nib_to_bytes(wnib & qv)), op + (size_t)qrow * g.ocr_pitch);
					if (do_scales && (uint32_t)qrow >= start_y) {
						const uint32_t nz = ((((l4 & 0x7F7F7F7Fu) + 0x7F7F7F7Fu) | l4) >> 7) & 0x01010101u;
						SMH_ST32(qoff, ones_to_bytes(nz), sp + (size_t)qrow * g.ocr_pitch);
					}
				}
			}
			if (rare(do_mask && __any(bright4(pv) != 0u))) {
				uint32_t pre = 0;
#pragma unroll
				for (int c = 0; c < 4; ++c) pre |= marker_prefilter(pv[c]) ? (1u << c) : 0u;
				prehits |= (pre & vmask) << (4 * k);
			}
		}
		if (rare(wave_q && __any((wrows | erows) != 0u))) {
			const int sh = r - base;
#pragma unroll
			for (int c = 0; c < 4; ++c) { or_w(c, (uint64_t)rows_of_col(wrows, c) << sh); or_e(c, (uint64_t)rows_of_col(erows, c) << sh); }
		}
		if (rare(do_mask && __any(prehits != 0u))) {
			uint32_t *hpx = s_hits + gwave * 160u;
			uint32_t *hres = hpx + 64;
			unsigned short *hid = (unsigned short *)(hres + 64);
			const uint32_t cnt = (uint32_t)__popc(prehits);
			uint32_t incl = cnt;
			for (int o = 1; o < 64; o <<= 1) { const uint32_t t = __shfl_up(incl, o); if (lane >= (uint32_t)o) incl += t; }
			const uint32_t total = __shfl(incl, 63);
			const uint32_t off = incl - cnt;
			hres[lane] = 0u;
			for (uint32_t hb = 0; hb < total; hb += 64u) {
				uint32_t o = off - hb;
#pragma unroll
				for (int k = 0; k < GR; ++k) {
					const uint32_t pk[4] = {px[k].x, px[k].y, px[k].z, px[k].w};
#pragma unroll
					for (int c = 0; c < 4; ++c)
						if ((prehits >> (4 * k + c)) & 1u) {
							if (o < 64u) { hpx[o] = pk[c]; hid[o] = (unsigned short)((lane << 4) | (uint32_t)(4 * k + c)); }
							++o;
						}
				}
				__builtin_amdgcn_wave_barrier();
				const uint32_t e = hb + lane;
				if (e < total) {
					const uint32_t p = hpx[lane];
					if (marker_exact((p >> 16) & 255u, (p >> 8) & 255u, p & 255u)) {
						const uint32_t id = hid[lane];
						atomicOr(&hres[id >> 4], 1u << (id & 15u));
					}
				}
				__builtin_amdgcn_wave_barrier();
			}
			const uint32_t res = hres[lane];
			if (res) {
				const int sh = r - base;
#pragma unroll
				for (int c = 0; c < 4; ++c) P[c] |= (uint64_t)rows_of_col(res, c) << sh;
			}
		}
	};

	{
		const uint8_t *dummy = (const uint8_t *)&b.aux[f];
		auto load4 = [&](u32x4 (&dst)[GR], int r) {
#pragma unroll
			for (int k = 0; k < GR; ++k) {
				const bool inside = r + k <= re;
				const uint8_t *rowp = inside ? fbase + (size_t)(r + k) * row_bytes : dummy;
				SMH_LD128(dst[k], inside ? loff : 0u, rowp);
			}
		};
		if constexpr (SETS == 2) {
			u32x4 S0[GR], S1[GR];
			load4(S0, rs);
			for (int r = rs; ; r += 8) {
				load4(S1, r + 4);
				SMH_WAIT_SET(4, S0);
				group(S0, r);
				if (r + 4 > re) break;
				load4(S0, r + 8);
				SMH_WAIT_SET(4, S1);
				group(S1, r + 4);
				if (r + 8 > re) break;
			}
			asm volatile("s_waitcnt vmcnt(0) ; smh-drain" : "+v"(S0[0]), "+v"(S0[1]), "+v"(S0[2]), "+v"(S0[3]), "+v"(S1[0]), "+v"(S1[1]), "+v"(S1[2]), "+v"(S1[3]) : : "memory");
		} else {
			u32x4 S0[GR], S1[GR], S2[GR];
			load4(S0, rs);
			load4(S1, rs + 4);
			for (int r = rs; ; r += 12) {
				load4(S2, r + 8);
				SMH_WAIT_SET(8, S0);
				group(S0, r);
				if (r + 4 > re) break;
				load4(S0, r + 12);
				SMH_WAIT_SET(8, S1);
				group(S1, r + 4);
				if (r + 8 > re) break;
				load4(S1, r + 16);
				SMH_WAIT_SET(8, S2);
				group(S2, r + 8);
				if (r + 12 > re) break;
			}
			asm volatile("s_waitcnt vmcnt(0) ; smh-drain" : "+v"(S0[0]), "+v"(S0[1]), "+v"(S0[2]), "+v"(S0[3]), "+v"(S1[0]), "+v"(S1[1]), "+v"(S1[2]), "+v"(S1[3]),
			             "+v"(S2[0]), "+v"(S2[1]), "+v"(S2[2]), "+v"(S2[3]) : : "memory");
		}
	}

	uint64_t V[4];
#pragma unroll
	for (int c = 0; c < 4; ++c) {
		const uint64_t w = get_w(c);
		V[c] = w | (w << 1) | (w << 2) | (w << 3) | (w >> 1) | (w >> 2) | (w >> 3);
	}
	__shared__ uint64_t s_edge_first[16], s_edge_last[16], s_first[16][4], s_last[16][4];
	if (lane == 0) { s_edge_first[gwave] = P[0]; s_first[gwave][0] = V[0]; s_first[gwave][1] = V[1]; s_first[gwave][2] = V[2]; s_first[gwave][3] = V[3]; }
	if (lane == 63) { s_edge_last[gwave] = P[3]; s_last[gwave][0] = V[0]; s_last[gwave][1] = V[1]; s_last[gwave][2] = V[2]; s_last[gwave][3] = V[3]; }
	__syncthreads();
	if (do_mask) {
		uint64_t left = __shfl_up(P[3], 1), right = __shfl_down(P[0], 1);
		if (lane == 0) left = wave > 0 ? s_edge_last[gwave - 1] : 0ull;
		if (lane == 63) right = wave + 1 < nwave ? s_edge_first[gwave + 1] : 0ull;
		const int nrows = r1 - r0;
		const uint64_t rowmask = ((nrows >= 61 ? ~0ull : ((1ull << nrows) - 1ull)) << 3);
		uint64_t D[4];
#define SMH_VERT(p) ((p) | ((p) << 1) | ((p) >> 1))
		D[0] = SMH_VERT(P[0]) | left | P[1];
		D[1] = SMH_VERT(P[1]) | P[0] | P[2];
		D[2] = SMH_VERT(P[2]) | P[1] | P[3];
		D[3] = SMH_VERT(P[3]) | P[2] | right;
#undef SMH_VERT
#pragma unroll
		for (int c = 0; c < 4; ++c) D[c] = ((vmask >> c) & 1u) ? (D[c] & rowmask) : 0ull;
		const uint32_t quads_padded = (g.m_quads + 15u) & ~15u;
		const uint64_t any = D[0] | D[1] | D[2] | D[3];
		const uint64_t lanes_set = __ballot(any != 0ull);
		uint32_t occ7 = 0;
		uint32_t *tiled_out = nullptr;
		if constexpr (TILES) {
			MapKernelArgsPtr kb = ka;
			asm volatile("" : "+s"(kb));
			tiled_out = kb->b.tiled;
			uint8_t *const occ_out = kb->b.occ;
			const uint32_t ntr = ((uint32_t)nrows + 7u) >> 3, opitch = occ_pitch(g);
			uint8_t *occp = occ_out + (size_t)f * occ_stride(g) + (size_t)((uint32_t)r0 >> 3) * opitch + wave;
			if (lanes_set) occ7 = tile_occupancy(any >> 3, lane, ntr, occp, opitch);
			else if (lane < ntr) occp[(size_t)lane * opitch] = 0;
			if (band == 0u && q == 0u) b.aux[f].tiles = 1u;
		}
		if (q < quads_padded && !lanes_set) {
			uint32_t *bbase = b.bits + (size_t)f * g.bits_stride_w;
			const uint32_t boff = (q >> 3) * 4u;
			const bool bit_lane = (lane & 7u) == 0;
			if (bit_lane)
				for (int row = r0; row < r1; ++row) *(uint32_t *)((uint8_t *)bbase + (size_t)row * g.bits_pitch_w * 4u + boff) = 0u;
		} else if (q < quads_padded) {
			uint32_t *bbase = b.bits + (size_t)f * g.bits_stride_w;
			const uint32_t boff = (q >> 3) * 4u;
			const bool bit_lane = (lane & 7u) == 0;
			uint32_t *tp = nullptr;
			uint32_t tpitch = 0;
			if constexpr (TILES) { tp = tiled_out + (size_t)f * tiled_stride_w(g) + ((size_t)((uint32_t)r0 >> 3) * g.bits_pitch_w + (q >> 3)) * 8u; tpitch = g.bits_pitch_w * 8u; }
#pragma unroll
			for (int half = 0; half < 2; ++half) {
				const uint32_t d0 = (uint32_t)(D[0] >> (32 * half)), d1 = (uint32_t)(D[1] >> (32 * half)), d2 = (uint32_t)(D[2] >> (32 * half)), d3 = (uint32_t)(D[3] >> (32 * half));
				const int row_lo = max(r0, base + 32 * half), row_hi = min(r1, base + 32 * half + 32);
				for (int row = row_lo; row < row_hi; ++row) {
					const uint32_t bit = (uint32_t)(row - base) & 31u;
					const uint32_t nib = ((d0 >> bit) & 1u) | (((d1 >> bit) & 1u) << 1) | (((d2 >> bit) & 1u) << 2) | (((d3 >> bit) & 1u) << 3);
					uint32_t v = nib;
					v |= SMH_DPP(v, 0x101) << 4;
					v |= SMH_DPP(v, 0x102) << 8;
					v |= SMH_DPP(v, 0x104) << 16;
					if (bit_lane) *(uint32_t *)((uint8_t *)bbase + (size_t)row * g.bits_pitch_w * 4u + boff) = v;
					if constexpr (TILES) {
						const uint32_t i = (uint32_t)(row - r0);
						if ((occ7 >> (i >> 3)) & 1u) tp[(size_t)(i >> 3) * tpitch + (i & 7u)] = v;
					}
				}
			}
		}
		if (lanes_set) {
			const uint64_t rows_set = wave_or64(any);
			const uint32_t cnt = wave_sum32(__popcll(D[0]) + __popcll(D[1]) + __popcll(D[2]) + __popcll(D[3]));
			if (lane == 0) {
				FrameAux *a = &b.aux[f];
				atomicMin(&a->y_min, (uint32_t)(base + __builtin_ctzll(rows_set)));
				atomicMax(&a->y_max, (uint32_t)(base + 63 - __builtin_clzll(rows_set)));
				atomicMin(&a->w_min, (wave * 64u + (uint32_t)__builtin_ctzll(lanes_set)) >> 3);
				atomicMax(&a->w_max, (wave * 64u + 63u - (uint32_t)__builtin_clzll(lanes_set)) >> 3);
				atomicAdd(&a->n_mask_px, cnt);
			}
		}
	}
	if (!(wave_q && do_ocr)) return;
	uint64_t X[12];
#pragma unroll
	for (int c = 0; c < 4; ++c) {
		uint64_t l = __shfl_up(V[c], 1), r = __shfl_down(V[c], 1);
		if (lane == 0) l = wave > 0 ? s_last[gwave - 1][c] : 0ull;
		if (lane == 63) r = wave + 1 < nwave ? s_first[gwave + 1][c] : 0ull;
		X[c] = l; X[4 + c] = V[c]; X[8 + c] = r;
	}
#pragma unroll
	for (int c = 0; c < 4; ++c) {
		uint64_t d = 0;
#pragma unroll
		for (int k = -3; k <= 3; ++k) d |= X[4 + c + k];
		uint64_t kk = get_e(c) & d;
		while (kk) {
			const int bit = __builtin_ctzll(kk);
			kk &= kk - 1;
			const int row = base + bit;
			const uint32_t p = *(const uint32_t *)(fp + (size_t)row * row_bytes + 4 * c);
			const uint32_t l = luma_bgra(p);
			op[(size_t)(row - qy0) * g.ocr_pitch + qoff + c] = (uint8_t)(255u - l);
		}
	}
}

template <bool GRAY, bool LOOP, int SETS, bool TILES>
__global__ void __launch_bounds__(1024) k_map_brq_pass(Geom g, Buffers b, uint32_t flags, uint32_t qflags, uint32_t RB, uint32_t fixed_start_y, int use_anchor_start,
                                                       uint32_t nbands, uint32_t items) {
#ifdef SMH_MAP_FAT
	asm volatile("; register footprint experiment" ::: SMH_MAP_FAT);
#endif
	static_assert(sizeof(MapKernelArgs) == sizeof(Geom) + sizeof(Buffers) + 7 * 4 + 4 || sizeof(MapKernelArgs) == sizeof(Geom) + sizeof(Buffers) + 7 * 4, "the kernel's parameter list");
	MapKernelArgsPtr ka = (MapKernelArgsPtr)__builtin_amdgcn_kernarg_segment_ptr();
	if (flags & MAP_PRIO) __builtin_amdgcn_s_setprio(3);
	if (LOOP) {
		for (uint32_t item = blockIdx.x; item < items; item += gridDim.x) {
			const uint32_t f = item / nbands, band = item - f * nbands;
			map_brq_item<GRAY ? 1 : 0, SETS, TILES>(ka, f, band);
			__syncthreads();
		}
	} else {
		uint32_t f = blockIdx.y, band = blockIdx.x;
		if (flags & MAP_BAND_MAJOR) {
			const uint32_t id = blockIdx.y * gridDim.x + blockIdx.x;
			band = id / gridDim.y; f = id - band * gridDim.y;
		}
		map_brq_item<GRAY ? 1 : 0, SETS, TILES>(ka, f, band);
	}
}

template <bool LOOP, int SETS, bool TILES>
__global__ void __launch_bounds__(1024) k_map_brq_pass_luma(Geom g, Buffers b, uint32_t flags, uint32_t qflags, uint32_t RB, uint32_t fixed_start_y, int use_anchor_start,
                                                            uint32_t nbands, uint32_t items) {
#ifdef SMH_MAP_FAT
	asm volatile("; register footprint experiment" ::: SMH_MAP_FAT);
#endif
	MapKernelArgsPtr ka = (MapKernelArgsPtr)__builtin_amdgcn_kernarg_segment_ptr();
	if (flags & MAP_PRIO) __builtin_amdgcn_s_setprio(3);
	if (LOOP) {
		for (uint32_t item = blockIdx.x; item < items; item += gridDim.x) {
			const uint32_t f = item / nbands, band = item - f * nbands;
			map_brq_item<2, SETS, TILES>(ka, f, band);
			__syncthreads();
		}
	} else {
		uint32_t f = blockIdx.y, band = blockIdx.x;
		if (flags & MAP_BAND_MAJOR) {
			const uint32_t id = blockIdx.y * gridDim.x + blockIdx.x;
			band = id / gridDim.y; f = id - band * gridDim.y;
		}
		map_brq_item<2, SETS, TILES>(ka, f, band);
	}
}

hipError_t launch_button(const Geom &g, const Buffers &b, uint32_t n, int force_open, hipStream_t s, uint8_t *ui_form, uint32_t ui_luma) {
	hipLaunchKernelGGL(k_button, dim3(n), dim3(256), 0, s, g, b, force_open, ui_form, ui_luma);
	return hipGetLastError();
}

static uint32_t work_item_order(bool overlapped) {
	const uint32_t forced = g_map_band_major.load(std::memory_order_relaxed);
	return (forced == 1u || (forced == 0u && !overlapped)) ? (uint32_t)MAP_BAND_MAJOR : 0u;
}

hipError_t launch_map_pass(const Geom &g, const Buffers &b, uint32_t n, uint32_t flags, int grayscale, hipStream_t s, bool tiles_wanted, bool overlapped) {
	const uint32_t RB = band_rows_for(g.rh, n, MAP_RB_MAX, tiles_wanted && b.tiled != nullptr, overlapped);
	const dim3 grid((g.rh + RB - 1) / RB, n);
	const unsigned lds = (g.m_block / 64u) * 640u;
	const bool tiles = tiles_wanted && b.tiled != nullptr && (RB & 7u) == 0u;
	if (grayscale == 2) {
		if (flags & MAP_BYTES) return hipErrorInvalidValue;
		if (tiles) hipLaunchKernelGGL((k_map_pass_luma<true>), grid, dim3(g.m_block), lds, s, g, b, flags, RB);
		else hipLaunchKernelGGL((k_map_pass_luma<false>), grid, dim3(g.m_block), lds, s, g, b, flags, RB);
	} else if (tiles) {
		if (grayscale) hipLaunchKernelGGL((k_map_pass<true, true>), grid, dim3(g.m_block), lds, s, g, b, flags, RB);
		else hipLaunchKernelGGL((k_map_pass<false, true>), grid, dim3(g.m_block), lds, s, g, b, flags, RB);
	} else {
		if (grayscale) hipLaunchKernelGGL((k_map_pass<true, false>), grid, dim3(g.m_block), lds, s, g, b, flags, RB);
		else hipLaunchKernelGGL((k_map_pass<false, false>), grid, dim3(g.m_block), lds, s, g, b, flags, RB);
	}
	return hipGetLastError();
}

static uint32_t map_brq_static_lds() {
	static const uint32_t v = [] { hipFuncAttributes a; return hipFuncGetAttributes(&a, (const void *)k_map_brq_pass<true, true, 2, false>) == hipSuccess ? (uint32_t)a.sharedSizeBytes : 2048u; }();
	return v;
}
uint32_t map_brq_lds_bytes(const Geom &g) { return map_brq_static_lds() + (g.m_block / 64u) * 640u; }

hipError_t launch_map_brq_pass(const Geom &g, const Buffers &b, uint32_t n, uint32_t flags, uint32_t qflags, int grayscale, uint32_t fixed_start_y, int use_anchor_start, hipStream_t s,
                               const LaunchTuning *tune) {
	const uint32_t cap0 = tune ? tune->map_grid_cap : 0u;
	const uint32_t RB0 = band_rows_for(g.rh, n, MAPQ_RB_MAX, false);
	bool no_tiles = b.tiled == nullptr || (tune && tune->map_deep) || (cap0 && cap0 < ((g.rh + RB0 - 1) / RB0) * n);
	uint32_t RB = no_tiles ? RB0 : band_rows_for(g.rh, n, MAPQ_RB_MAX, true, tune && tune->map_overlapped);
	uint32_t nbands = (g.rh + RB - 1) / RB, items = nbands * n;
	if (!no_tiles && cap0 && cap0 < items) { no_tiles = true; RB = RB0; nbands = (g.rh + RB - 1) / RB; items = nbands * n; }
	unsigned lds = (g.m_block / 64u) * 640u;
	if (tune && tune->map_lds_total > map_brq_lds_bytes(g)) lds = tune->map_lds_total - map_brq_static_lds();
	if (lds > 65536u) {
		static std::atomic<uint64_t> attr_devices{0};
		int dev = 0;
		hipError_t e = hipGetDevice(&dev);
		if (e != hipSuccess) return e;
		if (dev >= 64 || !((attr_devices.load(std::memory_order_acquire) >> dev) & 1ull)) {
			const void *fns[] = {(const void *)k_map_brq_pass<true, true, 2, false>, (const void *)k_map_brq_pass<false, true, 2, false>, (const void *)k_map_brq_pass<true, false, 2, false>,
			                     (const void *)k_map_brq_pass<false, false, 2, false>, (const void *)k_map_brq_pass<true, false, 2, true>, (const void *)k_map_brq_pass<false, false, 2, true>,
			                     (const void *)k_map_brq_pass<true, false, 3, false>, (const void *)k_map_brq_pass<false, false, 3, false>,
			                     (const void *)k_map_brq_pass_luma<true, 2, false>, (const void *)k_map_brq_pass_luma<false, 2, false>, (const void *)k_map_brq_pass_luma<false, 2, true>,
			                     (const void *)k_map_brq_pass_luma<false, 3, false>};
			for (const void *fn : fns) if (e == hipSuccess) e = hipFuncSetAttribute(fn, hipFuncAttributeMaxDynamicSharedMemorySize, 160 * 1024 - 2048);
			if (e != hipSuccess) return e;
			if (dev < 64) attr_devices.fetch_or(1ull << dev, std::memory_order_release);
		}
	}
	if (tune && tune->map_prio) flags |= MAP_PRIO;
	flags |= work_item_order(tune && tune->map_overlapped);
	const uint32_t cap = tune ? tune->map_grid_cap : 0u;
	const bool deep = tune && tune->map_deep && !(cap && cap < items);
	const bool tiles = !no_tiles && (RB & 7u) == 0u && !(cap && cap < items) && !deep;
#define SMH_LAUNCH_MAPQ(GRAYV, LOOPV, SETSV, TILESV, GRID) \
	hipLaunchKernelGGL((k_map_brq_pass<GRAYV, LOOPV, SETSV, TILESV>), GRID, dim3(g.m_block), lds, s, g, b, flags, qflags, RB, fixed_start_y, use_anchor_start, nbands, items)
#define SMH_LAUNCH_MAPQ_LUMA(LOOPV, SETSV, TILESV, GRID) \
	hipLaunchKernelGGL((k_map_brq_pass_luma<LOOPV, SETSV, TILESV>), GRID, dim3(g.m_block), lds, s, g, b, flags, qflags, RB, fixed_start_y, use_anchor_start, nbands, items)
	if (grayscale == 2) {
		if (cap && cap < items) SMH_LAUNCH_MAPQ_LUMA(true, 2, false, dim3(cap));
		else if (deep) SMH_LAUNCH_MAPQ_LUMA(false, 3, false, dim3(nbands, n));
		else if (tiles) SMH_LAUNCH_MAPQ_LUMA(false, 2, true, dim3(nbands, n));
		else SMH_LAUNCH_MAPQ_LUMA(false, 2, false, dim3(nbands, n));
	} else if (cap && cap < items) {
		if (grayscale) SMH_LAUNCH_MAPQ(true, true, 2, false, dim3(cap)); else SMH_LAUNCH_MAPQ(false, true, 2, false, dim3(cap));
	} else if (deep) {
		if (grayscale) SMH_LAUNCH_MAPQ(true, false, 3, false, dim3(nbands, n)); else SMH_LAUNCH_MAPQ(false, false, 3, false, dim3(nbands, n));
	} else if (tiles) {
		if (grayscale) SMH_LAUNCH_MAPQ(true, false, 2, true, dim3(nbands, n)); else SMH_LAUNCH_MAPQ(false, false, 2, true, dim3(nbands, n));
	} else {
		if (grayscale) SMH_LAUNCH_MAPQ(true, false, 2, false, dim3(nbands, n)); else SMH_LAUNCH_MAPQ(false, false, 2, false, dim3(nbands, n));
	}
#undef SMH_LAUNCH_MAPQ_LUMA
#undef SMH_LAUNCH_MAPQ
	return hipGetLastError();
}

template <int NR>
__global__ void __launch_bounds__(1024) k_pattern_copy(Geom g, Buffers b, uint32_t RB, uint32_t band_major) {
	uint32_t f = blockIdx.y, band = blockIdx.x;
	if (band_major) {
		const uint32_t id = blockIdx.y * gridDim.x + blockIdx.x;
		band = id / gridDim.y; f = id - band * gridDim.y;
	}
	const uint32_t q = threadIdx.x;
	const int r0 = (int)(band * RB), r1 = min(r0 + (int)RB, (int)g.rh);
	if (q >= g.m_quads) return;
	const uint8_t *fp = b.frames + (size_t)f * g.frame_bytes + ((size_t)g.ry * g.W + g.m_ax) * 4 + (size_t)q * 16;
	uint8_t *up = b.ui + (size_t)f * g.ui_stride + (size_t)q * 16;
	const int qy0 = (int)(g.qy - g.ry);
	const int qq = (int)q - (int)((g.q_ax - g.m_ax) >> 2);
	const bool in_q = qq >= 0 && (uint32_t)qq < g.q_quads;
	uint8_t *op = b.ocr + (size_t)f * g.ocr_stride + (size_t)(in_q ? qq : 0) * 4;
	uint8_t *sp = b.scales + (size_t)f * g.ocr_stride + (size_t)(in_q ? qq : 0) * 4;
	const size_t row_bytes = (size_t)g.W * 4;
	for (int r = r0; r < r1; r += NR) {
		uint4 v[NR];
#pragma unroll
		for (int k = 0; k < NR; ++k) v[k] = *(const uint4 *)(fp + (size_t)min(r + k, r1 - 1) * row_bytes);
#pragma unroll
		for (int k = 0; k < NR; ++k) {
			const int row = r + k;
			if (row >= r1) break;
			*(uint4 *)(up + (size_t)row * g.ui_pitch) = v[k];
			const uint32_t m = v[k].x ^ v[k].y ^ v[k].z ^ v[k].w;
			const int qrow = row - qy0;
			if (in_q && qrow >= 0 && qrow < (int)g.qh) {
				*(uint32_t *)(op + (size_t)qrow * g.ocr_pitch) = ~m;
				*(uint32_t *)(sp + (size_t)qrow * g.ocr_pitch) = m + 1u;
			}
		}
	}
}

hipError_t launch_pattern_copy(const Geom &g, const Buffers &b, uint32_t n, uint32_t rows_in_flight, hipStream_t s) {
	const uint32_t RB = band_rows_for(g.rh, n, MAPQ_RB_MAX);
	const dim3 grid((g.rh + RB - 1) / RB, n), block(g.m_block);
	const uint32_t bm = g_map_band_major.load(std::memory_order_relaxed) == 2u ? 0u : 1u;
	switch (rows_in_flight) {
	case 0: case 4: hipLaunchKernelGGL(k_pattern_copy<4>, grid, block, 0, s, g, b, RB, bm); break;
	case 8: hipLaunchKernelGGL(k_pattern_copy<8>, grid, block, 0, s, g, b, RB, bm); break;
	case 12: hipLaunchKernelGGL(k_pattern_copy<12>, grid, block, 0, s, g, b, RB, bm); break;
	default: return hipErrorInvalidValue;
	}
	return hipGetLastError();
}

void map_band_rows(uint32_t rh, uint32_t n, int fused, uint32_t *rows, int *tiles) {
	const uint32_t RB = band_rows_for(rh, n, fused ? MAPQ_RB_MAX : MAP_RB_MAX, true, fused == 2);
	if (rows) *rows = RB;
	if (tiles) *tiles = (RB & 7u) == 0u ? 1 : 0;
}

hipError_t launch_brq_pass(const Geom &g, const Buffers &b, uint32_t n, uint32_t flags, uint32_t fixed_start_y, int use_anchor_start, hipStream_t s) {
	const dim3 grid((g.qh + BRQ_RB - 1) / BRQ_RB, n);
	hipLaunchKernelGGL(k_brq_pass, grid, dim3(g.q_block), 0, s, g, b, flags, fixed_start_y, use_anchor_start);
	return hipGetLastError();
// ... 4 lines not shown
```

Before: 614,600.

## Defer OCR image materialization by storing compact keep-bitmask in brq pass

In the lazy luma UI path with tiled map/brq pass, the kernel now writes a packed 4-bit-per-quad OCR keep mask instead of full byte OCR output. The full OCR bytes are reconstructed on demand by a new expand kernel only when a consumer (device_ptrs, debug view, feed/render with OCR source) asks for them. This cuts per-frame OCR write bandwidth in the hot pass, at the cost of extra state tracking, a mutex, and a later expand launch when OCR is actually read.

New measurement: 618,100 (median of 6 runs). Within noise of the previous version (+0.6%).

```diff
diff --git a/include/smh_vision_hip_debug.h b/include/smh_vision_hip_debug.h
--- a/include/smh_vision_hip_debug.h
+++ b/include/smh_vision_hip_debug.h
@@ -33,6 +33,8 @@
 SMHV_API int smhv_debug_batch_mask_state(smhv_batch *b, uint32_t *stale_frames, int *eager);
 SMHV_API int smhv_debug_batch_ui_state(smhv_batch *b, uint32_t *stale_frames, int *eager);
 SMHV_API int smhv_debug_batch_materialize_ui(smhv_batch *b, void *stream);
+SMHV_API int smhv_debug_batch_ocr_state(smhv_batch *b, uint32_t *stale_frames, int *eager);
+SMHV_API int smhv_debug_batch_materialize_ocr(smhv_batch *b, void *stream);
 SMHV_API int smhv_debug_mask_expand(smhv_batch *b, uint32_t n, void *stream);
 SMHV_API int smhv_debug_ingest_feed(smhv_ingest *q, uint32_t n, uint32_t *counter);
 SMHV_API int smhv_debug_ingest_feed_pixels(smhv_ingest *q, uint32_t n, uint32_t *counter, uint32_t pixels);
diff --git a/squad-mortar-helper_amd/_lib.py b/squad-mortar-helper_amd/_lib.py
--- a/squad-mortar-helper_amd/_lib.py
+++ b/squad-mortar-helper_amd/_lib.py
@@ -223,6 +223,8 @@
     "smhv_debug_batch_mask_state": (C.c_int, [C.c_void_p, C.POINTER(C.c_uint32), C.POINTER(C.c_int)]),
     "smhv_debug_batch_ui_state": (C.c_int, [C.c_void_p, C.POINTER(C.c_uint32), C.POINTER(C.c_int)]),
     "smhv_debug_batch_materialize_ui": (C.c_int, [C.c_void_p, C.c_void_p]),
+    "smhv_debug_batch_ocr_state": (C.c_int, [C.c_void_p, C.POINTER(C.c_uint32), C.POINTER(C.c_int)]),
+    "smhv_debug_batch_materialize_ocr": (C.c_int, [C.c_void_p, C.c_void_p]),
     "smhv_debug_mask_expand": (C.c_int, [C.c_void_p, C.c_uint32, C.c_void_p]),
     "smhv_debug_marker_table": (C.c_int, [C.c_void_p, C.c_void_p]),
     "smhv_ingest_create": (C.c_int, [C.c_void_p, C.c_uint32, C.c_uint32, C.c_uint32, C.c_uint32, C.POINTER(C.c_void_p)]),
diff --git a/squad-mortar-helper_amd/batch.py b/squad-mortar-helper_amd/batch.py
--- a/squad-mortar-helper_amd/batch.py
+++ b/squad-mortar-helper_amd/batch.py
@@ -48,6 +48,8 @@
             self._ptrs["mask"] = self._batch._mask_ptr()
         if key == "ui" and self._ptrs["ui"] is None:
             self._ptrs["ui"] = self._batch._ui_ptr()
+        if key == "ocr" and self._ptrs["ocr"] is None:
+            self._ptrs["ocr"] = self._batch._ocr_ptr()
         return self._ptrs[key]
 
     def __iter__(self):
@@ -119,7 +121,7 @@
     def device_ptrs(self):
         p = [C.c_void_p() for _ in range(6)]
         args = [C.byref(x) for x in p]
-        args[1] = args[2] = None
+        args[1] = args[2] = args[3] = None
         L.check(self._lib.smhv_batch_device_ptrs(self._b, *args))
         return _DevicePtrs(self, dict(zip(_PTR_KEYS, [x.value for x in p])))
 
@@ -132,6 +134,19 @@
         u = C.c_void_p()
         L.check(self._lib.smhv_batch_device_ptrs(self._b, None, C.byref(u), None, None, None, None))
         return u.value
+
+    def _ocr_ptr(self):
+        o = C.c_void_p()
+        L.check(self._lib.smhv_batch_device_ptrs(self._b, None, None, None, C.byref(o), None, None))
+        return o.value
+
+    def ocr_state(self):
+        stale, eager = C.c_uint32(0), C.c_int(0)
+        L.check(self._lib.smhv_debug_batch_ocr_state(self._b, C.byref(stale), C.byref(eager)))
+        return int(stale.value), bool(eager.value)
+
+    def materialize_ocr(self, stream=0):
+        L.check(self._lib.smhv_debug_batch_materialize_ocr(self._b, C.c_void_p(stream)))
 
     def ui_state(self):
         stale, eager = C.c_uint32(0), C.c_int(0)
diff --git a/squad-mortar-helper_amd/csrc/smh_feed.inc b/squad-mortar-helper_amd/csrc/smh_feed.inc
--- a/squad-mortar-helper_amd/csrc/smh_feed.inc
+++ b/squad-mortar-helper_amd/csrc/smh_feed.inc
@@ -187,6 +187,10 @@
 		rc = batch_materialize_mask(b, (hipStream_t)stream);
 		if (rc) return rc;
 	}
+	if (map_source == (uint32_t)SMHV_VIEW_OCR_INPUT) {
+		rc = batch_materialize_ocr(b, (hipStream_t)stream);
+		if (rc) return rc;
+	}
 	rc = batch_materialize_ui(b, (hipStream_t)stream);
 	if (rc) return rc;
 	return feed_enqueue(f, v, b->d_results + first, first, n, flags, (hipStream_t)stream);
diff --git a/squad-mortar-helper_amd/csrc/smh_kernels.h b/squad-mortar-helper_amd/csrc/smh_kernels.h
--- a/squad-mortar-helper_amd/csrc/smh_kernels.h
+++ b/squad-mortar-helper_amd/csrc/smh_kernels.h
@@ -313,10 +313,15 @@
 hipError_t launch_lsd_service(const Geom &g, const SvcParams &p, uint32_t workgroups, uint32_t waves, uint32_t lds_bytes, hipStream_t s);
 
 enum : uint32_t { MAP_UI = 1u, MAP_MASK = 2u, MAP_BYTES = 4u, MAP_PRIO = 0x100u, MAP_BAND_MAJOR = 0x200u };
-enum : uint32_t { BRQ_OCR = 1u, BRQ_SCALES = 2u };
+enum : uint32_t { BRQ_OCR = 1u, BRQ_SCALES = 2u, BRQ_OCR_KEEP = 4u };
 
 enum : uint32_t { UI_FORM_RGBA = 0u, UI_FORM_LUMA = 1u, UI_FORM_KEEP = 2u };
-hipError_t launch_button(const Geom &g, const Buffers &b, uint32_t n, int force_open, hipStream_t s, uint8_t *ui_form = nullptr, uint32_t ui_luma = UI_FORM_KEEP);
+enum : uint32_t { OCR_FORM_BYTES = 0u, OCR_FORM_BITS = 1u, OCR_FORM_KEEP = 2u };
+__host__ __device__ inline uint32_t ocr_keep_pitch(const Geom &g) { return (uint32_t)(g.ocr_pitch >> 3) + 4u; }
+__host__ __device__ inline uint64_t ocr_keep_stride(const Geom &g) { return (uint64_t)ocr_keep_pitch(g) * g.qh; }
+hipError_t launch_button(const Geom &g, const Buffers &b, uint32_t n, int force_open, hipStream_t s, uint8_t *ui_form = nullptr, uint32_t ui_luma = UI_FORM_KEEP,
+                         uint8_t *ocr_form = nullptr, uint32_t ocr_keep = OCR_FORM_KEEP);
+hipError_t launch_ocr_expand(const Geom &g, const uint8_t *d_luma, const uint8_t *d_keep, uint8_t *d_ocr, uint8_t *ocr_form, uint32_t n, hipStream_t s);
 hipError_t launch_ui_expand(const Geom &g, const uint8_t *d_luma, uint8_t *d_ui, uint8_t *ui_form, uint32_t n, hipStream_t s);
 hipError_t launch_map_pass(const Geom &g, const Buffers &b, uint32_t n, uint32_t flags, int grayscale, hipStream_t s, bool tiles_wanted = false, bool overlapped = false);
 struct LaunchTuning {
@@ -329,6 +334,7 @@
 };
 uint32_t map_brq_lds_bytes(const Geom &g);
 uint32_t lsd_tile_lds_bytes(const Geom &g, uint32_t tile_limit);
+bool map_brq_pass_tiles(const Geom &g, bool have_tiled, uint32_t n, const LaunchTuning *tune);
 hipError_t launch_map_brq_pass(const Geom &g, const Buffers &b, uint32_t n, uint32_t flags, uint32_t qflags, int grayscale, uint32_t fixed_start_y, int use_anchor_start, hipStream_t s,
                                const LaunchTuning *tune = nullptr);
 hipError_t launch_pattern_copy(const Geom &g, const Buffers &b, uint32_t n, uint32_t rows_in_flight, hipStream_t s);
diff --git a/squad-mortar-helper_amd/csrc/smh_misc.hip b/squad-mortar-helper_amd/csrc/smh_misc.hip
--- a/squad-mortar-helper_amd/csrc/smh_misc.hip
+++ b/squad-mortar-helper_amd/csrc/smh_misc.hip
@@ -408,6 +408,35 @@
 	return e;
 }
 
+__global__ void __launch_bounds__(256) k_ocr_expand(const uint8_t *__restrict__ luma, const uint8_t *__restrict__ keep, uint8_t *__restrict__ ocr, const uint8_t *__restrict__ form,
+                                                    Geom g) {
+	const uint32_t f = blockIdx.y;
+	if (form[f] != OCR_FORM_BITS) return;
+	const uint32_t i = blockIdx.x * 256u + threadIdx.x;
+	if (i >= g.q_quads * g.qh) return;
+	const uint32_t row = i / g.q_quads, quad = i - row * g.q_quads;
+	const uint32_t qy0 = g.qy - g.ry, off_q = (g.q_ax - g.m_ax) >> 2;
+	const uint32_t l4 = *(const uint32_t *)(luma + (size_t)f * (g.ui_stride >> 2) + (size_t)(qy0 + row) * (g.ui_pitch >> 2) + (size_t)(off_q + quad) * 4u);
+	const uint32_t kq = quad + (off_q & 7u);
+	const uint32_t kw = *(const uint32_t *)(keep + (size_t)f * ocr_keep_stride(g) + (size_t)row * ocr_keep_pitch(g) + (size_t)(kq >> 3) * 4u);
+	const uint32_t nib = (kw >> (4u * (kq & 7u))) & 15u;
+	const uint32_t bytes = (((nib * 0x00204081u) & 0x01010101u) * 0xFFu);
+	*(uint32_t *)(ocr + (size_t)f * g.ocr_stride + (size_t)row * g.ocr_pitch + (size_t)quad * 4u) = ~(l4 & bytes);
+}
+hipError_t launch_ocr_expand(const Geom &g, const uint8_t *d_luma, const uint8_t *d_keep, uint8_t *d_ocr, uint8_t *ocr_form, uint32_t n, hipStream_t s) {
+	if ((g.ocr_pitch & 7u) || (g.ui_pitch & 15u) || n == 0 || (uint64_t)g.q_quads * g.qh > 0xFFFFFF00ull) return hipErrorInvalidValue;
+	const uint32_t quads = g.q_quads * g.qh;
+	hipError_t e = hipSuccess;
+	for (uint32_t done = 0; done < n && e == hipSuccess; done += 65535u) {
+		const uint32_t k = std::min(n - done, 65535u);
+		hipLaunchKernelGGL(k_ocr_expand, dim3((quads + 255u) / 256u, k), dim3(256), 0, s, d_luma + (size_t)done * (g.ui_stride >> 2), d_keep + (size_t)done * ocr_keep_stride(g),
+		                   d_ocr + (size_t)done * g.ocr_stride, (const uint8_t *)ocr_form + done, g);
+		e = hipGetLastError();
+	}
+	if (e == hipSuccess) e = hipMemsetAsync(ocr_form, 0, n, s);
+	return e;
+}
+
 hipError_t launch_debug_view(const Geom &g, const Buffers &b, uint32_t frame, int which, int isolated, uint8_t *d_rgba, hipStream_t s) {
 	const bool brq = which == SMHV_VIEW_OCR_INPUT || which == SMHV_VIEW_FIND_SCALES_INPUT || which == SMHV_VIEW_CROPPED_BRQ;
 	const uint32_t npx = brq ? g.qw * g.qh : g.rw * g.rh;
diff --git a/squad-mortar-helper_amd/csrc/smh_runtime.cpp b/squad-mortar-helper_amd/csrc/smh_runtime.cpp
--- a/squad-mortar-helper_amd/csrc/smh_runtime.cpp
+++ b/squad-mortar-helper_amd/csrc/smh_runtime.cpp
@@ -205,6 +205,11 @@
 	uint32_t ui_stale = 0;
 	bool ui_eager = false;
 	hipEvent_t ev_ui = nullptr;
+	uint8_t *d_ocr_keep = nullptr, *d_ocr_form = nullptr;
+	std::mutex ocr_mu;
+	uint32_t ocr_stale = 0;
+	bool ocr_eager = false;
+	hipEvent_t ev_ocr = nullptr;
 	smhv_render_prim *h_prims = nullptr, *d_prims = nullptr;
 	hipEvent_t ev_prims = nullptr;
 	smhv_label_result *d_labels = nullptr;
@@ -540,6 +545,8 @@
 	ALLOC0(b->d_tiled, tiled_stride_w(g) * 4 * n);
 	ALLOC0(b->d_occ, occ_stride(g) * n);
 	ALLOC0(b->d_ocr, g.ocr_stride * n);
+	ALLOC0(b->d_ocr_keep, ocr_keep_stride(g) * n);
+	ALLOC0(b->d_ocr_form, n);
 	ALLOC0(b->d_scales, g.ocr_stride * n);
 	ALLOC0(b->d_aux, sizeof(FrameAux) * n);
 	ALLOC0(b->d_results, sizeof(smhv_frame_result) * (n + 3));
@@ -556,6 +563,7 @@
 		if (e == hipSuccess) e = hipEventCreateWithFlags(&b->ev_map_done, hipEventDisableTiming);
 		if (e == hipSuccess) e = hipEventCreateWithFlags(&b->ev_mask, hipEventDisableTiming);
 		if (e == hipSuccess) e = hipEventCreateWithFlags(&b->ev_ui, hipEventDisableTiming);
+		if (e == hipSuccess) e = hipEventCreateWithFlags(&b->ev_ocr, hipEventDisableTiming);
 		if (max_frames > 1 && !lsd_rows_only(b->g)) {
 			if (e == hipSuccess) e = create_stream(&b->lsd_fork.s1, nullptr);
 			if (e == hipSuccess) e = create_stream(&b->lsd_fork.s2, nullptr);
@@ -573,7 +581,7 @@
 	if (!b) return;
 	if (b->ctx) (void)hipSetDevice(b->ctx->device);
 	(void)hipDeviceSynchronize();
-	void *ptrs[] = {b->d_ui, b->d_ui_luma, b->d_ui_form, b->d_mask, b->d_bits, b->d_tiled, b->d_occ, b->d_ocr, b->d_scales, b->d_aux, b->d_results, b->d_anchors, b->d_bars, b->d_farm,
+	void *ptrs[] = {b->d_ui, b->d_ui_luma, b->d_ui_form, b->d_mask, b->d_bits, b->d_tiled, b->d_occ, b->d_ocr, b->d_ocr_keep, b->d_ocr_form, b->d_scales, b->d_aux, b->d_results, b->d_anchors, b->d_bars, b->d_farm,
 	                b->d_lsd_ctl, b->d_lsd_req, b->d_lsd_cache, b->d_firing, b->d_fire_run, b->d_overlay, b->d_render, b->d_prims, b->d_labels,
 	                b->d_label_cull, b->d_label_extra, b->d_probes, b->d_dbg_items, b->d_dbg_pool, b->d_dbg_stage};
 	for (void *p : ptrs)
@@ -609,6 +617,7 @@
 	if (b->ev_map_done) (void)hipEventDestroy(b->ev_map_done);
 	if (b->ev_mask) (void)hipEventDestroy(b->ev_mask);
 	if (b->ev_ui) (void)hipEventDestroy(b->ev_ui);
+	if (b->ev_ocr) (void)hipEventDestroy(b->ev_ocr);
 	for (auto e : b->ev_probe) if (e) (void)hipEventDestroy(e);
 	if (b->lsd_fork.s1) (void)hipStreamDestroy(b->lsd_fork.s1);
 	if (b->lsd_fork.s2) (void)hipStreamDestroy(b->lsd_fork.s2);
@@ -817,6 +826,16 @@
 	return SMHV_OK;
 }
 
+static int batch_materialize_ocr(smhv_batch *b, hipStream_t stream) {
+	std::lock_guard<std::mutex> lk(b->ocr_mu);
+	if (b->ocr_stale) {
+		HIPCHK(launch_ocr_expand(b->g, b->d_ui_luma, b->d_ocr_keep, b->d_ocr, b->d_ocr_form, std::min(b->ocr_stale, b->max_frames), stream));
+		HIPCHK(hipEventRecord(b->ev_ocr, stream));
+		b->ocr_stale = 0;
+	} else HIPCHK(hipStreamWaitEvent(stream, b->ev_ocr, 0));
+	return SMHV_OK;
+}
+
 struct SvcPublish { SvcCtl *ctl; unsigned long long *ring; SvcSlot *slots; uint32_t slot, seq, ring_log2; const uint32_t *cull_tab; bool have_cull; hipStream_t s_pro; hipEvent_t ev_pro;
                     bool *published; };
 static int batch_run_impl(smhv_batch *b, const void *d_frames, uint32_t n, uint32_t stages, int grayscale, uint32_t max_gap,
@@ -880,8 +899,21 @@
 		if (ui_lazy) { b->ui_stale = std::max(b->ui_stale, n); bf.ui = b->d_ui_luma; }
 	}
 	const int pass_gray = ui_lazy ? 2 : (grayscale ? 1 : 0);
+	const bool ocr_stage = (stages & SMHV_STAGE_OCR) != 0u;
+	bool ocr_lazy = false, ocr_settle = false;
+	{
+		std::lock_guard<std::mutex> lk(b->ocr_mu);
+		ocr_lazy = ui_lazy && ocr_stage && !b->ocr_eager && map_brq_pass_tiles(g, b->d_tiled != nullptr, n, &b->tune);
+		if (ocr_lazy) { b->ocr_stale = std::max(b->ocr_stale, n); bf.ocr = b->d_ocr_keep; }
+		ocr_settle = ui_lazy && !ocr_lazy && b->ocr_stale != 0u;
+	}
+	if (ocr_settle) {
+		int rc = batch_materialize_ocr(b, s);
+		if (rc) return rc;
+	}
 	STAGE_BEGIN(0, sb);
-	HIPCHK(launch_button(g, bf, n, 0, sb, b->d_ui_form, ui_stage ? (ui_lazy ? UI_FORM_LUMA : UI_FORM_RGBA) : UI_FORM_KEEP));
+	HIPCHK(launch_button(g, bf, n, 0, sb, b->d_ui_form, ui_stage ? (ui_lazy ? UI_FORM_LUMA : UI_FORM_RGBA) : UI_FORM_KEEP, b->d_ocr_form,
+	                     ocr_stage ? (ocr_lazy ? OCR_FORM_BITS : OCR_FORM_BYTES) : OCR_FORM_KEEP));
 	STAGE_END(0, sb);
 	if (sb != s) {
 		HIPCHK(hipEventRecord(svc->ev_pro, sb));
@@ -890,7 +922,7 @@
 	uint32_t mflags = 0, qflags = 0;
 	if (stages & SMHV_STAGE_MARKERS) mflags |= MAP_MASK;
 	if (stages & SMHV_STAGE_UI_MAP) mflags |= MAP_UI;
-	if (stages & SMHV_STAGE_OCR) qflags |= BRQ_OCR;
+	if (stages & SMHV_STAGE_OCR) qflags |= ocr_lazy ? (BRQ_OCR | BRQ_OCR_KEEP) : BRQ_OCR;
 	if (scales) qflags |= BRQ_SCALES;
 	if (b->probe) HIPCHK(hipEventRecord(b->ev_probe[0], s));
 	STAGE_BEGIN(1, s);
@@ -1033,7 +1065,16 @@
 		HIPCHK(wait_stream(b->ctx->s_main));
 		*mask = b->d_mask;
 	}
-	if (ocr) *ocr = b->d_ocr;
+	if (ocr) {
+		CTX_OPEN(b->ctx);
+		HIPCHK(hipSetDevice(b->ctx->device));
+		{ std::lock_guard<std::mutex> lk(b->ocr_mu); b->ocr_eager = true; }
+		HIPCHK(hipDeviceSynchronize());
+		int rc = batch_materialize_ocr(b, b->ctx->s_main);
+		if (rc) return rc;
+		HIPCHK(wait_stream(b->ctx->s_main));
+		*ocr = b->d_ocr;
+	}
 	if (scales) *scales = b->d_scales;
 	if (bits) *bits = b->d_bits;
 	return SMHV_OK;
@@ -1110,6 +1151,8 @@
 	}
 	case SMHV_VIEW_OCR_INPUT: {
 		std::lock_guard<std::mutex> lk(b->ctx->mu);
+		int rc = batch_materialize_ocr(b, b->ctx->s_main);
+		if (rc) return rc;
 		return copy_image_d2h(b->ctx, 2, out, b->d_ocr + frame * g.ocr_stride, g.ocr_pitch, g.q_xoff, g.qw, g.qh, b->ctx->s_main);
 	}
 	case SMHV_VIEW_FIND_SCALES_INPUT: {
@@ -2646,6 +2689,21 @@
 	return SMHV_OK;
 }
 
+extern "C" SMHV_API int smhv_debug_batch_ocr_state(smhv_batch *b, uint32_t *stale_frames, int *eager) {
+	if (!b) return fail(SMHV_E_INVALID, "null batch");
+	std::lock_guard<std::mutex> lk(b->ocr_mu);
+	if (stale_frames) *stale_frames = b->ocr_stale;
+	if (eager) *eager = b->ocr_eager ? 1 : 0;
+	return SMHV_OK;
+}
+
+extern "C" SMHV_API int smhv_debug_batch_materialize_ocr(smhv_batch *b, void *stream) {
+	if (!b) return fail(SMHV_E_INVALID, "null batch");
+	CTX_OPEN(b->ctx);
+	HIPCHK(hipSetDevice(b->ctx->device));
+	return batch_materialize_ocr(b, (hipStream_t)stream);
+}
+
 extern "C" SMHV_API int smhv_debug_batch_materialize_ui(smhv_batch *b, void *stream) {
 	if (!b) return fail(SMHV_E_INVALID, "null batch");
 	CTX_OPEN(b->ctx);
@@ -3150,6 +3208,10 @@
 	hipStream_t s = (hipStream_t)stream;
 	if (layers->map_source == (uint32_t)SMHV_VIEW_LSD_INPUT) {
 		rc = batch_materialize_mask(b, s);
+		if (rc) return rc;
+	}
+	if (layers->map_source == (uint32_t)SMHV_VIEW_OCR_INPUT) {
+		rc = batch_materialize_ocr(b, s);
 		if (rc) return rc;
 	}
 	rc = batch_materialize_ui(b, s);
diff --git a/squad-mortar-helper_amd/csrc/smh_stream.hip b/squad-mortar-helper_amd/csrc/smh_stream.hip
--- a/squad-mortar-helper_amd/csrc/smh_stream.hip
+++ b/squad-mortar-helper_amd/csrc/smh_stream.hip
@@ -28,7 +28,7 @@
 	return occ;
 }
 
-__global__ void __launch_bounds__(256) k_button(Geom g, Buffers b, int force_open, uint8_t *ui_form, uint32_t ui_luma) {
+__global__ void __launch_bounds__(256) k_button(Geom g, Buffers b, int force_open, uint8_t *ui_form, uint32_t ui_luma, uint8_t *ocr_form, uint32_t ocr_keep) {
 	const uint32_t f = blockIdx.x;
 	const uint8_t *fp = b.frames + (size_t)f * g.frame_bytes;
 	__shared__ uint32_t s_cnt;
@@ -65,6 +65,7 @@
 		a.y_min = 0xFFFFFFFFu; a.y_max = 0; a.w_min = 0xFFFFFFFFu; a.w_max = 0; a.tiles = 0;
 		b.aux[f] = a;
 		if (ui_form && ui_luma != UI_FORM_KEEP && a.open) ui_form[f] = (uint8_t)ui_luma;
+		if (ocr_form && ocr_keep != OCR_FORM_KEEP && a.open) ocr_form[f] = (uint8_t)ocr_keep;
 	}
 }
 
@@ -274,6 +275,9 @@
 		if (an.n == 0 || start_y > g.qh) do_scales = false;
 	}
 	const bool do_ocr = (qflags & BRQ_OCR) != 0;
+	constexpr bool KEEPF = GRAY == 2 && TILES;
+	bool ocr_bits = false;
+	if constexpr (KEEPF) ocr_bits = (qflags & BRQ_OCR_KEEP) != 0;
 	const uint32_t q = threadIdx.x, lane = q & 63u, wave = q >> 6;
 	const uint32_t nwave = blockDim.x >> 6, gwave = wave;
 	const int r0 = live ? (int)(band * RB) : 0;
@@ -303,6 +307,7 @@
 	const uint8_t *fp = fbase + (size_t)q * 16;
 	uint8_t *uibase = b.ui + (size_t)f * (GRAY == 2 ? g.ui_stride >> 2 : g.ui_stride);
 	uint8_t *op = b.ocr + (size_t)f * g.ocr_stride;
+	if constexpr (KEEPF) op = b.ocr + (size_t)f * (ocr_bits ? ocr_keep_stride(g) : g.ocr_stride);
 	uint8_t *sp = b.scales + (size_t)f * g.ocr_stride;
 	const uint32_t qoff = (uint32_t)(in_q ? qq : 0) * 4u;
 	const size_t row_bytes = (size_t)g.W * 4;
@@ -362,7 +367,8 @@
 					enib |= (e ? 1u : 0u) << c;
 				}
 				const bool nb_row = (uint32_t)qrow + SMH_OCR_DILATE_RADIUS <= g.qh;
-				if (nb_row) wrows |= (wnib & qw_) << (4 * k);
+				if constexpr (KEEPF) wrows |= (wnib & qv) << (4 * k);
+				else if (nb_row) wrows |= (wnib & qw_) << (4 * k);
 				if (out_row) erows |= (enib & qv) << (4 * k);
 			}
 			if (out_row) {
@@ -387,7 +393,9 @@
 				}
 				if (q_row && in_q) {
 					const uint32_t l4 = lum[0] | (lum[1] << 8) | (lum[2] << 16) | (lum[3] << 24);
-					if (do_ocr) SMH_ST32(qoff, ~(l4 & nib_to_bytes(wnib & qv)), op + (size_t)qrow * g.ocr_pitch);
+					if constexpr (KEEPF) {
+						if (do_ocr && !ocr_bits) SMH_ST32(qoff, ~(l4 & nib_to_bytes(wnib & qv)), op + (size_t)qrow * g.ocr_pitch);
+					} else if (do_ocr) SMH_ST32(qoff, ~(l4 & nib_to_bytes(wnib & qv)), op + (size_t)qrow * g.ocr_pitch);
 					if (do_scales && (uint32_t)qrow >= start_y) {
 						const uint32_t nz = ((((l4 & 0x7F7F7F7Fu) + 0x7F7F7F7Fu) | l4) >> 7) & 0x01010101u;
 						SMH_ST32(qoff, ones_to_bytes(nz), sp + (size_t)qrow * g.ocr_pitch);
@@ -498,7 +506,12 @@
 	uint64_t V[4];
 #pragma unroll
 	for (int c = 0; c < 4; ++c) {
-		const uint64_t w = get_w(c);
+		uint64_t w = get_w(c);
+		if constexpr (KEEPF) {
+			const int nb_hi = qy0 + (int)g.qh - (int)SMH_OCR_DILATE_RADIUS - base;
+			const uint64_t nb_rows = nb_hi >= 63 ? ~0ull : nb_hi < 0 ? 0ull : ((2ull << nb_hi) - 1ull);
+			w = ((qw_ >> c) & 1u) ? (w & nb_rows) : 0ull;
+		}
 		V[c] = w | (w << 1) | (w << 2) | (w << 3) | (w >> 1) | (w >> 2) | (w >> 3);
 	}
 	__shared__ uint64_t s_edge_first[16], s_edge_last[16], s_first[16][4], s_last[16][4];
@@ -590,6 +603,42 @@
 		if (lane == 63) r = wave + 1 < nwave ? s_first[gwave + 1][c] : 0ull;
 		X[c] = l; X[4 + c] = V[c]; X[8 + c] = r;
 	}
+	if constexpr (KEEPF) {
+		if (ocr_bits) {
+			const uint64_t out_rows = ((1ull << (qr1 - qr0)) - 1ull) << (qr0 + qy0 - base);
+			uint64_t K[4];
+#pragma unroll
+			for (int c = 0; c < 4; ++c) {
+				uint64_t d = 0;
+#pragma unroll
+				for (int k = -3; k <= 3; ++k) d |= X[4 + c + k];
+				K[c] = (get_e(c) & d) | (get_w(c) & out_rows);
+			}
+			const uint32_t offq = (g.q_ax - g.m_ax) >> 2;
+			const bool writer = (lane & 7u) == 0u && (q >> 3) >= (offq >> 3) && q < offq + g.q_quads;
+			const uint32_t kpitch = ocr_keep_pitch(g);
+			uint8_t *kp = op + (writer ? ((q >> 3) - (offq >> 3)) * 4u : 0u);
+			if (!__any((K[0] | K[1] | K[2] | K[3]) != 0ull)) {
+				if (writer)
+					for (int qrow = qr0; qrow < qr1; ++qrow) *(uint32_t *)(kp + (size_t)qrow * kpitch) = 0u;
+				return;
+			}
+#pragma unroll
+			for (int half = 0; half < 2; ++half) {
+				const uint32_t k0 = (uint32_t)(K[0] >> (32 * half)), k1 = (uint32_t)(K[1] >> (32 * half)), k2 = (uint32_t)(K[2] >> (32 * half)), k3 = (uint32_t)(K[3] >> (32 * half));
+				const int row_lo = max(qr0 + qy0, base + 32 * half), row_hi = min(qr1 + qy0, base + 32 * half + 32);
+				for (int row = row_lo; row < row_hi; ++row) {
+					const uint32_t bit = (uint32_t)(row - base) & 31u;
+					uint32_t v = ((k0 >> bit) & 1u) | (((k1 >> bit) & 1u) << 1) | (((k2 >> bit) & 1u) << 2) | (((k3 >> bit) & 1u) << 3);
+					v |= SMH_DPP(v, 0x101) << 4;
+					v |= SMH_DPP(v, 0x102) << 8;
+					v |= SMH_DPP(v, 0x104) << 16;
+					if (writer) *(uint32_t *)(kp + (size_t)(row - qy0) * kpitch) = v;
+				}
+			}
+			return;
+		}
+	}
 #pragma unroll
 	for (int c = 0; c < 4; ++c) {
 		uint64_t d = 0;
@@ -656,8 +705,8 @@
 	}
 }
 
-hipError_t launch_button(const Geom &g, const Buffers &b, uint32_t n, int force_open, hipStream_t s, uint8_t *ui_form, uint32_t ui_luma) {
-	hipLaunchKernelGGL(k_button, dim3(n), dim3(256), 0, s, g, b, force_open, ui_form, ui_luma);
+hipError_t launch_button(const Geom &g, const Buffers &b, uint32_t n, int force_open, hipStream_t s, uint8_t *ui_form, uint32_t ui_luma, uint8_t *ocr_form, uint32_t ocr_keep) {
+	hipLaunchKernelGGL(k_button, dim3(n), dim3(256), 0, s, g, b, force_open, ui_form, ui_luma, ocr_form, ocr_keep);
 	return hipGetLastError();
 }
 
@@ -690,6 +739,15 @@
 	return v;
 }
 uint32_t map_brq_lds_bytes(const Geom &g) { return map_brq_static_lds() + (g.m_block / 64u) * 640u; }
+
+bool map_brq_pass_tiles(const Geom &g, bool have_tiled, uint32_t n, const LaunchTuning *tune) {
+	const uint32_t cap = tune ? tune->map_grid_cap : 0u;
+	const uint32_t RB0 = band_rows_for(g.rh, n, MAPQ_RB_MAX, false);
+	if (!have_tiled || (tune && tune->map_deep) || (cap && cap < ((g.rh + RB0 - 1) / RB0) * n)) return false;
+	const uint32_t RB = band_rows_for(g.rh, n, MAPQ_RB_MAX, true, tune && tune->map_overlapped);
+	if (cap && cap < ((g.rh + RB - 1) / RB) * n) return false;
+	return (RB & 7u) == 0u;
+}
 
 hipError_t launch_map_brq_pass(const Geom &g, const Buffers &b, uint32_t n, uint32_t flags, uint32_t qflags, int grayscale, uint32_t fixed_start_y, int use_anchor_start, hipStream_t s,
                                const LaunchTuning *tune) {
@@ -722,6 +780,7 @@
 	const uint32_t cap = tune ? tune->map_grid_cap : 0u;
 	const bool deep = tune && tune->map_deep && !(cap && cap < items);
 	const bool tiles = !no_tiles && (RB & 7u) == 0u && !(cap && cap < items) && !deep;
+	if ((qflags & BRQ_OCR_KEEP) && !(grayscale == 2 && tiles)) return hipErrorInvalidValue;
 #define SMH_LAUNCH_MAPQ(GRAYV, LOOPV, SETSV, TILESV, GRID) \
 	hipLaunchKernelGGL((k_map_brq_pass<GRAYV, LOOPV, SETSV, TILESV>), GRID, dim3(g.m_block), lds, s, g, b, flags, qflags, RB, fixed_start_y, use_anchor_start, nbands, items)
 #define SMH_LAUNCH_MAPQ_LUMA(LOOPV, SETSV, TILESV, GRID) \
```
